# tenpy/cyten

Measured on AMD Instinct MI355X. Metric: block-sparse tdot+SVD GFLOP/s (fp64), higher is better.
Workload: dtype f64

## Files before the change

### cyten_amd/csrc/jacobi_engine.hip

```cpp
#include "jacobi_engine.h"

#include <algorithm>
#include <cmath>
#include <cstdlib>

namespace cyb {
constexpr double kPredictQuad = 16.0;
namespace {

typedef double d4 __attribute__((ext_vector_type(4)));
typedef double d2 __attribute__((ext_vector_type(2)));
#define GLOBAL_AS __attribute__((address_space(1)))
typedef const GLOBAL_AS d2* gc2;
typedef const GLOBAL_AS d2* gcp2;
typedef GLOBAL_AS double* gp;

constexpr int GS = JP + 2;
constexpr int QS = JP + 16;
constexpr int GK = 64;
constexpr int XS = GK + 2;
constexpr int NT = 256;
constexpr int NPAIR = JP / 2;
static_assert(JP == 32, "the wave tiling below assumes 32 x 32 pair problems");

__device__ __forceinline__ double wave_max(double v)
{
#pragma unroll
    for (int o = 32; o > 0; o >>= 1) v = fmax(v, __shfl_xor(v, o));
    return v;
}

__device__ __forceinline__ double block_max(double v, double* red, int tid)
{
    v = wave_max(v);
    __syncthreads();
    if ((tid & 63) == 0) red[tid >> 6] = v;
    __syncthreads();
    return fmax(fmax(red[0], red[1]), fmax(red[2], red[3]));
}

__device__ __forceinline__ double gram_offmax(const double* Gs, double* red, int tid)
{
    double m = 0.0;
#pragma unroll
    for (int e = tid; e < JP * JP; e += NT) {
        const int i = e / JP, j = e % JP;
        if (i < j) {
            const double den = Gs[i * GS + i] * Gs[j * GS + j];
            if (den > 0.0) m = fmax(m, fabs(Gs[i * GS + j]) * rsqrt(den));
        }
    }
    return block_max(m, red, tid);
}

__host__ __device__ __forceinline__ void circle_pair(int n, int r, int k, int& p, int& q)
{
    const int m = n - 1;
    if (k == 0) {
        p = m;
        q = r;
    } else {
        p = r + k;
        if (p >= m) p -= m;
        q = r - k;
        if (q < 0) q += m;
    }
}

__device__ __forceinline__ double fast_rsqrt(double x)
{
    double r = __builtin_amdgcn_rsq(x);
    r = r * (1.5 - 0.5 * x * r * r);
    r = r * (1.5 - 0.5 * x * r * r);
    return r;
}

__device__ __forceinline__ void jacobi_rot(double a, double d, double b, double& c, double& s)
{
    const double delta = d - a;
    const double h2 = delta * delta + 4.0 * b * b;
    c = 1.0;
    s = 0.0;
    if (fabs(b) > 1e-300 && h2 > 1e-300) {
        const double rh = fast_rsqrt(h2);
        const double c2 = 0.5 + 0.5 * fabs(delta) * rh;
        const double rc = fast_rsqrt(c2);
        c = c2 * rc;
        const double sg = ((delta >= 0.0) == (b >= 0.0)) ? 1.0 : -1.0;
        s = sg * fabs(b) * rh * rc;
    }
}

__device__ __forceinline__ int xrow(int i, int P, int Q) { return (i < JB) ? P * JB + i : Q * JB + (i - JB); }

struct JScratch {
    double* gpart;
    double* qout[2];
    int32_t* zout[2];
    int32_t* flag[2];
    unsigned int* cnt;
};

__device__ __forceinline__ void update_role(const JMat* __restrict__ mats, const JWork* __restrict__ work, int round,
                                            int pi, int unit, int U, const JScratch& sc, int buf, bool do_w, bool do_j,
                                            double* smem, int* zflag);

__global__ void __launch_bounds__(NT, 2)
jacobi_gram_kernel(const JMat* __restrict__ mats, const JWork* __restrict__ work, int round, int G, int max_inner,
                   unsigned long long* __restrict__ offmax_bits, JScratch sc, int buf, int n_gram, int prev_round, int UJ)
{
    constexpr int STAGE = 2 * JP * XS > 4 * JP * GS ? 2 * JP * XS : 4 * JP * GS;
    __shared__ __attribute__((aligned(16))) double smem[2 * JP * GS + JP * QS + STAGE + 8];
    __shared__ int perm[JP];
    __shared__ int zrow[JP];
    __shared__ int s_any_null, s_last;
    __shared__ unsigned short sched[(JP - 1) * NPAIR];
    double* Gs = smem;
    double* G2 = Gs + JP * GS;
    double* Qs = G2 + JP * GS;
    double* Xc = Qs + JP * QS;
    double* red = Xc + STAGE;

    const int tid = threadIdx.x;
    const int lane = tid & 63, wave = tid >> 6;
    if ((int)blockIdx.x >= n_gram) {
        const int b = (int)blockIdx.x - n_gram;
        update_role(mats, work, prev_round, b / UJ, b % UJ, UJ, sc, buf ^ 1, false, true, smem, zrow);
        return;
    }
    const int pi = blockIdx.x / G, part = blockIdx.x % G;

    const JWork wk = work[pi];
    const JMat mt = mats[wk.mat];
    if (round >= mt.nb - 1) return;
    int P, Q;
    circle_pair(mt.nb, round, wk.slot, P, Q);
    if (P > Q) {
        const int t = P;
        P = Q;
        Q = t;
    }

    {
        gp W = (gp)mt.W;
        const int ld = mt.lenp;
        d4 acc[2][2];
#pragma unroll
        for (int i = 0; i < 2; ++i)
#pragma unroll
            for (int j = 0; j < 2; ++j) acc[i][j] = d4{0.0, 0.0, 0.0, 0.0};
        const int r = lane & 15, g2 = 2 * (lane >> 4);
        gcp2 s0 = (gcp2)(W + (int64_t)xrow(r, P, Q) * ld + g2);
        gcp2 s1 = (gcp2)(W + (int64_t)xrow(r + 16, P, Q) * ld + g2);
        const int nchunk_all = ld / 8;
        const int c_begin = (int)((int64_t)part * nchunk_all / G), c_end = (int)((int64_t)(part + 1) * nchunk_all / G);
        constexpr int UN = 8;
        d2 x0[UN], x1[UN], n0[UN], n1[UN];
        auto load = [&](d2 (&a0)[UN], d2 (&a1)[UN], int c0) {
#pragma unroll
            for (int u = 0; u < UN; ++u) {
                const int c = min(c0 + 4 * u, c_end - 1);
                a0[u] = s0[c * 4];
                a1[u] = s1[c * 4];
            }
        };
        if (c_begin + wave < c_end) load(x0, x1, c_begin + wave);
        for (int c0 = c_begin + wave; c0 < c_end; c0 += 4 * UN) {
            const bool more = c0 + 4 * UN < c_end;
            if (more) load(n0, n1, c0 + 4 * UN);
#pragma unroll
            for (int u = 0; u < UN; ++u) {
                if (c0 + 4 * u < c_end) {
                    acc[0][0] = __builtin_amdgcn_mfma_f64_16x16x4f64(x0[u].x, x0[u].x, acc[0][0], 0, 0, 0);
                    acc[0][1] = __builtin_amdgcn_mfma_f64_16x16x4f64(x0[u].x, x1[u].x, acc[0][1], 0, 0, 0);
                    acc[1][1] = __builtin_amdgcn_mfma_f64_16x16x4f64(x1[u].x, x1[u].x, acc[1][1], 0, 0, 0);
                    acc[0][0] = __builtin_amdgcn_mfma_f64_16x16x4f64(x0[u].y, x0[u].y, acc[0][0], 0, 0, 0);
                    acc[0][1] = __builtin_amdgcn_mfma_f64_16x16x4f64(x0[u].y, x1[u].y, acc[0][1], 0, 0, 0);
                    acc[1][1] = __builtin_amdgcn_mfma_f64_16x16x4f64(x1[u].y, x1[u].y, acc[1][1], 0, 0, 0);
                }
            }
            if (more) {
#pragma unroll
                for (int u = 0; u < UN; ++u) {
                    x0[u] = n0[u];
                    x1[u] = n1[u];
                }
            }
        }
        double* wpart = Xc + wave * (JP * GS);
#pragma unroll
        for (int i = 0; i < 2; ++i)
#pragma unroll
            for (int j = 0; j < 2; ++j)
#pragma unroll
                for (int r = 0; r < 4; ++r) {
                    if (i == 1 && j == 0)
                        wpart[(16 + (lane & 15)) * GS + (lane >> 4) + 4 * r] = acc[0][1][r];
                    else
                        wpart[(i * 16 + (lane >> 4) + 4 * r) * GS + j * 16 + (lane & 15)] = acc[i][j][r];
                }
    }
    __syncthreads();
    if (G == 1) {
        for (int e = tid; e < JP * JP; e += NT) {
            const int i = e / JP, j = e % JP;
            double s = 0.0;
#pragma unroll
            for (int w = 0; w < 4; ++w) s += Xc[w * (JP * GS) + i * GS + j];
            Gs[i * GS + j] = s;
        }
        __syncthreads();
    } else {
        GLOBAL_AS double* mine = (GLOBAL_AS double*)(sc.gpart + ((size_t)pi * G + part) * (JP * JP));
        for (int e = tid; e < JP * JP; e += NT) {
            const int i = e / JP, j = e % JP;
            double s = 0.0;
#pragma unroll
            for (int w = 0; w < 4; ++w) s += Xc[w * (JP * GS) + i * GS + j];
            __hip_atomic_store((double*)(mine + e), s, __ATOMIC_RELAXED, __HIP_MEMORY_SCOPE_AGENT);
        }
        asm volatile("s_waitcnt vmcnt(0)" ::: "memory");
        __syncthreads();
        if (tid == 0) {
            const unsigned int old = __hip_atomic_fetch_add(sc.cnt + pi, 1u, __ATOMIC_RELAXED, __HIP_MEMORY_SCOPE_AGENT);
            s_last = (old == (unsigned int)(G - 1)) ? 1 : 0;
            if (s_last) __hip_atomic_store(sc.cnt + pi, 0u, __ATOMIC_RELAXED, __HIP_MEMORY_SCOPE_AGENT);
        }
        __syncthreads();
        if (!s_last) return;
        const GLOBAL_AS double* all = (const GLOBAL_AS double*)(sc.gpart + (size_t)pi * G * (JP * JP));
        for (int e = tid; e < JP * JP; e += NT) {
            const int i = e / JP, j = e % JP;
            double s = 0.0;
            for (int g = 0; g < G; ++g)
                s += __hip_atomic_load((double*)(all + (size_t)g * (JP * JP) + i * JP + j), __ATOMIC_RELAXED, __HIP_MEMORY_SCOPE_AGENT);
            Gs[i * GS + j] = s;
        }
        __syncthreads();
    }
    if (tid == 0) s_any_null = 0;
    __syncthreads();
    if (tid < JP) {
        const double thr2 = mt.thr2;
        const double g = Gs[tid * GS + tid];
        const int z = (g > 0.0 && g <= thr2) ? 1 : 0;
        zrow[tid] = z;
        perm[tid] = tid;
        if (z) s_any_null = 1;
    }
    __syncthreads();
    const bool any_null = s_any_null != 0;
    if (any_null) {
        for (int e = tid; e < JP * JP; e += NT) {
            const int i = e / JP, j = e % JP;
            if (zrow[i] || zrow[j]) Gs[i * GS + j] = 0.0;
        }
        __syncthreads();
    }
    double off = gram_offmax(Gs, red, tid);
    if (tid == 0) {
        atomicMax(offmax_bits + wk.mat, (unsigned long long)__double_as_longlong(off));
        sc.flag[buf][pi] = (off <= mt.tol && !any_null) ? 0 : 1;
    }
    if (off <= mt.tol && !any_null) return;

    for (int e = tid; e < JP * QS; e += NT) Qs[e] = ((e / QS) == (e % QS)) ? 1.0 : 0.0;
    for (int e = tid; e < (JP - 1) * NPAIR; e += NT) {
        int p, q;
        circle_pair(JP, e / NPAIR, e % NPAIR, p, q);
        sched[e] = (unsigned short)(p | (q << 8));
    }
    __syncthreads();
    double* Ga = Gs;
    double* Gb = G2;
    for (int sweep = 0; sweep < (off <= mt.tol ? 0 : max_inner); ++sweep) {
        for (int r = 0; r < JP - 1; ++r) {
            const int pr = tid >> 4, pc = tid & 15;
            const unsigned int sr = sched[r * NPAIR + pr], scl = sched[r * NPAIR + pc];
            const int i = sr & 255, j = sr >> 8, k = scl & 255, l = scl >> 8;
            double c2, s2;
            jacobi_rot(Ga[k * GS + k], Ga[l * GS + l], Ga[k * GS + l], c2, s2);
            const int srcl = (lane & 48) | pr;
            const double c1 = __shfl(c2, srcl), s1 = __shfl(s2, srcl);
            {
                const double gik = Ga[i * GS + k], gil = Ga[i * GS + l];
                const double gjk = Ga[j * GS + k], gjl = Ga[j * GS + l];
                const double hik = c1 * gik - s1 * gjk, hil = c1 * gil - s1 * gjl;
                const double hjk = s1 * gik + c1 * gjk, hjl = s1 * gil + c1 * gjl;
                double nik = c2 * hik - s2 * hil, nil = s2 * hik + c2 * hil;
                double njk = c2 * hjk - s2 * hjl, njl = s2 * hjk + c2 * hjl;
                if (pr == pc) {
                    nil = 0.0;
                    njk = 0.0;
                }
                Gb[i * GS + k] = nik;
                Gb[i * GS + l] = nil;
                Gb[j * GS + k] = njk;
                Gb[j * GS + l] = njl;
            }
#pragma unroll
            for (int t = 0; t < 2; ++t) {
                const int row = (tid >> 4) + 16 * t;
                const double qk = Qs[row * QS + k], ql = Qs[row * QS + l];
                Qs[row * QS + k] = c2 * qk - s2 * ql;
                Qs[row * QS + l] = s2 * qk + c2 * ql;
            }
            __syncthreads();
            double* tsw = Ga;
            Ga = Gb;
            Gb = tsw;
        }
        if (sweep + 1 < max_inner) {
            const double off_in = gram_offmax(Ga, red, tid);
            if (off_in <= 0.25 * mt.tol) break;
        }
    }
    __syncthreads();
    if (off > mt.tol && tid < JP) {
        auto key = [&](int i) { return xrow(i, P, Q) < mt.nv ? Ga[i * GS + i] : -1.0e300; };
        const double g = key(tid);
        int rk = 0;
        for (int j = 0; j < JP; ++j) {
            const double gj = key(j);
            rk += (gj > g || (gj == g && j < tid)) ? 1 : 0;
        }
        perm[rk] = tid;
    }
    __syncthreads();
    GLOBAL_AS double* qo = (GLOBAL_AS double*)(sc.qout[buf] + (size_t)pi * (JP * JP));
    for (int e = tid; e < JP * JP; e += NT) {
        const int k = e / JP, r = e % JP;
        qo[e] = Qs[k * QS + perm[r]];
    }
    if (tid < JP) sc.zout[buf][(size_t)pi * JP + tid] = zrow[perm[tid]];
}

__device__ __forceinline__ void update_role(const JMat* __restrict__ mats, const JWork* __restrict__ work, int round,
                                            int pi, int unit, int U, const JScratch& sc, int buf, bool do_w, bool do_j,
                                            double* smem, int* zflag)
{
    double* Qs = smem;
    const int tid = threadIdx.x;
    const int lane = tid & 63, wave = tid >> 6;
    const JWork wk = work[pi];
    const JMat mt = mats[wk.mat];
    if (round >= mt.nb - 1) return;
    if (sc.flag[buf][pi] == 0) return;
    int P, Q;
    circle_pair(mt.nb, round, wk.slot, P, Q);
    if (P > Q) {
        const int t = P;
        P = Q;
        Q = t;
    }
    const int cw = do_w ? mt.lenp / 64 : 0, cj = (do_j && mt.J) ? mt.nvp / 64 : 0;
    const int ct = cw + cj;
    const int c_begin = (int)((int64_t)unit * ct / U), c_end = (int)((int64_t)(unit + 1) * ct / U);
    if (c_begin >= c_end) return;
    const int n = lane & 15, kq = lane >> 4;
    auto chunk_ptr = [&](int c, int k) -> gp {
        const bool in_w = c < cw;
        gp base = (gp)(in_w ? mt.W : mt.J);
        const int ld = in_w ? mt.lenp : mt.nvp;
        const int cc = in_w ? c : c - cw;
        return base + (int64_t)xrow(k, P, Q) * ld + cc * 64 + wave * 16 + n;
    };
    double xb[JP / 4], xn[JP / 4];
#pragma unroll
    for (int kk = 0; kk < JP / 4; ++kk) xb[kk] = *chunk_ptr(c_begin, 4 * kk + kq);
    const GLOBAL_AS double* qo = (const GLOBAL_AS double*)(sc.qout[buf] + (size_t)pi * (JP * JP));
    for (int e = tid; e < JP * JP; e += NT) Qs[(e / JP) * QS + (e % JP)] = qo[e];
    if (tid < JP) zflag[tid] = sc.zout[buf][(size_t)pi * JP + tid];
    __syncthreads();
    const double* ap0 = Qs + (lane >> 4) * QS + (lane & 15);
    const double* ap1 = ap0 + 16;
    int zr[2][4];
#pragma unroll
    for (int i = 0; i < 2; ++i)
#pragma unroll
        for (int r = 0; r < 4; ++r) zr[i][r] = zflag[i * 16 + (lane >> 4) + 4 * r];
    for (int c = c_begin; c < c_end; ++c) {
        if (c + 1 < c_end) {
#pragma unroll
            for (int kk = 0; kk < JP / 4; ++kk) xn[kk] = *chunk_ptr(c + 1, 4 * kk + kq);
        }
        d4 acc[2] = {d4{0.0, 0.0, 0.0, 0.0}, d4{0.0, 0.0, 0.0, 0.0}};
#pragma unroll
        for (int kk = 0; kk < JP / 4; ++kk) {
            const double a0 = ap0[kk * 4 * QS], a1 = ap1[kk * 4 * QS];
            acc[0] = __builtin_amdgcn_mfma_f64_16x16x4f64(a0, xb[kk], acc[0], 0, 0, 0);
            acc[1] = __builtin_amdgcn_mfma_f64_16x16x4f64(a1, xb[kk], acc[1], 0, 0, 0);
        }
        const bool zero_null = c < cw;
#pragma unroll
        for (int i = 0; i < 2; ++i)
#pragma unroll
            for (int r = 0; r < 4; ++r) {
                const int row = i * 16 + (lane >> 4) + 4 * r;
                const double val = (zero_null && zr[i][r]) ? 0.0 : acc[i][r];
                *chunk_ptr(c, row) = val;
            }
#pragma unroll
        for (int kk = 0; kk < JP / 4; ++kk) xb[kk] = xn[kk];
    }
}

__global__ void __launch_bounds__(NT, 3)
jacobi_update_kernel(const JMat* __restrict__ mats, const JWork* __restrict__ work, int round, int U, JScratch sc, int buf,
                     int do_w, int do_j)
{
    __shared__ __attribute__((aligned(16))) double smem[JP * QS];
    __shared__ int zflag[JP];
    update_role(mats, work, round, blockIdx.x / U, blockIdx.x % U, U, sc, buf, do_w != 0, do_j != 0, smem, zflag);
}


struct RPair {
    double* W;
    double* J;
    double tol, thr2;
    int32_t nvp, lenp, nb, nv;
    int32_t mat, slot;
    int32_t pad[2];
};
static_assert(sizeof(RPair) == 64, "RPair is read as one 64-byte descriptor");

struct RScratch {
    double* gpart;
    unsigned int* cnt;
    unsigned int* err;
    int np;
    unsigned long long* stamps;
};

typedef unsigned int u32x4 __attribute__((ext_vector_type(4)));
union Q16 {
    u32x4 u;
    d2 d;
};

constexpr int VS = JP + 2;
constexpr int ROUND_LDS_DOUBLES = 2 * JP * GS + 2 * JP * VS + JP * QS + 4 * JP * GS + 8;
constexpr size_t ROUND_LDS_BYTES = 88 * 1024;
static_assert(ROUND_LDS_DOUBLES * 8 + 1024 <= ROUND_LDS_BYTES, "LDS carve-up of the fused round kernel");
constexpr int RGMAX = 8;
constexpr int RPRE = 6;

__device__ __forceinline__ int ring_next(int p)
{
    if (p == 0) return 0;
    if (p == 1) return 2;
    if (p & 1) return p - 2;
    return p == JP - 2 ? JP - 1 : p + 2;
}

__device__ __forceinline__ void jacobi_rot_bf(double a, double d, double b, double& c, double& s, double thr2 = 0.0)
{
    const double delta = d - a;
    const double b2 = b + b;
    double h2 = fma(b2, b2, delta * delta);
    const bool ok = (fabs(b) > 1e-300) & (h2 > 1e-300) & (b * b > thr2 * a * d);
    h2 = ok ? h2 : 1.0;
    double r = __builtin_amdgcn_rsq(h2);
    double g = h2 * r, h = 0.5 * r;
    double e = fma(-g, h, 0.5);
    g = fma(g, e, g);
    h = fma(h, e, h);
    e = fma(-g, h, 0.5);
    h = fma(h, e, h);
    const double c2 = fma(fabs(delta), h, 0.5);
    double r2 = __builtin_amdgcn_rsq(c2);
    double gc = c2 * r2, hc = 0.5 * r2;
    double ec = fma(-gc, hc, 0.5);
    gc = fma(gc, ec, gc);
    hc = fma(hc, ec, hc);
    ec = fma(-gc, hc, 0.5);
    gc = fma(gc, ec, gc);
    hc = fma(hc, ec, hc);
    const double sabs = (fabs(b) * h) * (4.0 * hc);
    const bool pos = (delta >= 0.0) == (b >= 0.0);
    c = ok ? gc : 1.0;
    s = ok ? (pos ? sabs : -sabs) : 0.0;
}

__global__ void __launch_bounds__(NT, 1)
jacobi_round_kernel(const RPair* __restrict__ pairs, int round, int G, int max_inner,
                    unsigned long long* __restrict__ offmax_bits, RScratch sc)
{
    extern __shared__ __attribute__((aligned(16))) double rsm[];
    double* Gs = rsm;
    double* G2 = Gs + JP * GS;
    double* Va = G2 + JP * GS;
    double* Vb = Va + JP * VS;
    double* Qs = Vb + JP * VS;
    double* Xc = Qs + JP * QS;
    double* red = Xc + 4 * JP * GS;
    int* ibase = reinterpret_cast<int*>(red + 8);
    int* perm = ibase;
    int* zrow = ibase + JP;
    int* zout = ibase + 2 * JP;
    int* flags = ibase + 3 * JP;

    const int tid = threadIdx.x;
    const int lane = tid & 63, wave = tid >> 6;
    const int pi = blockIdx.x / G, part = blockIdx.x % G;
#define ROUND_STAMP(k)                                                                              \
    do {                                                                                            \
        if (sc.stamps && tid == 0) sc.stamps[(size_t)blockIdx.x * 8 + (k)] = wall_clock64();        \
    } while (0)
    ROUND_STAMP(0);
    const RPair mt = pairs[pi];
    if (round >= mt.nb - 1) return;
    int P, Q;
    circle_pair(mt.nb, round, mt.slot, P, Q);
    if (P > Q) {
        const int t = P;
        P = Q;
        Q = t;
    }
    const int cw = mt.lenp / 64, cj = mt.J ? mt.nvp / 64 : 0;
    const int w_begin = (int)((int64_t)part * cw / G), w_end = (int)((int64_t)(part + 1) * cw / G);
    const int j_begin = (int)((int64_t)part * cj / G), j_end = (int)((int64_t)(part + 1) * cj / G);
    const int nW = w_end - w_begin, nJ = j_end - j_begin;
    const int ct = nW + nJ;
    const int un = lane & 15, ukq = lane >> 4;
    auto chunk_ptr = [&](int c, int k) -> gp {
        const bool in_w = c < nW;
        gp base = (gp)(in_w ? mt.W : mt.J);
        const int ld = in_w ? mt.lenp : mt.nvp;
        const int cc = in_w ? w_begin + c : j_begin + (c - nW);
        return base + (int64_t)xrow(k, P, Q) * ld + cc * 64 + wave * 16 + un;
    };

    double xpre[RPRE][JP / 4];
    {
        gp W = (gp)mt.W;
        const int ld = mt.lenp;
        d4 acc00 = d4{0.0, 0.0, 0.0, 0.0}, acc01 = acc00, acc11 = acc00;
        const int r = lane & 15, g2 = 2 * (lane >> 4);
        gcp2 s0 = (gcp2)(W + (int64_t)xrow(r, P, Q) * ld + g2);
        gcp2 s1 = (gcp2)(W + (int64_t)xrow(r + 16, P, Q) * ld + g2);
        const int c_begin = 8 * w_begin, c_end = 8 * w_end;
        constexpr int UN = 8;
        d2 x0[UN], x1[UN], n0[UN], n1[UN];
        auto load = [&](d2 (&a0)[UN], d2 (&a1)[UN], int c0) {
#pragma unroll
            for (int u = 0; u < UN; ++u) {
                const int c = min(c0 + 4 * u, c_end - 1);
                a0[u] = s0[c * 4];
                a1[u] = s1[c * 4];
            }
        };
        if (c_begin + wave < c_end) load(x0, x1, c_begin + wave);
#pragma unroll
        for (int c = 0; c < RPRE; ++c) {
            if (c < ct) {
#pragma unroll
                for (int kk = 0; kk < JP / 4; ++kk) xpre[c][kk] = *chunk_ptr(c, 4 * kk + ukq);
            }
        }
        for (int c0 = c_begin + wave; c0 < c_end; c0 += 4 * UN) {
            const bool more = c0 + 4 * UN < c_end;
            if (more) load(n0, n1, c0 + 4 * UN);
#pragma unroll
            for (int u = 0; u < UN; ++u) {
                if (c0 + 4 * u < c_end) {
                    acc00 = __builtin_amdgcn_mfma_f64_16x16x4f64(x0[u].x, x0[u].x, acc00, 0, 0, 0);
                    acc01 = __builtin_amdgcn_mfma_f64_16x16x4f64(x0[u].x, x1[u].x, acc01, 0, 0, 0);
                    acc11 = __builtin_amdgcn_mfma_f64_16x16x4f64(x1[u].x, x1[u].x, acc11, 0, 0, 0);
                    acc00 = __builtin_amdgcn_mfma_f64_16x16x4f64(x0[u].y, x0[u].y, acc00, 0, 0, 0);
                    acc01 = __builtin_amdgcn_mfma_f64_16x16x4f64(x0[u].y, x1[u].y, acc01, 0, 0, 0);
                    acc11 = __builtin_amdgcn_mfma_f64_16x16x4f64(x1[u].y, x1[u].y, acc11, 0, 0, 0);
                }
            }
            if (more) {
#pragma unroll
                for (int u = 0; u < UN; ++u) {
                    x0[u] = n0[u];
                    x1[u] = n1[u];
                }
            }
        }
        double* wpart = Xc + wave * (JP * GS);
#pragma unroll
        for (int q = 0; q < 4; ++q) {
            const int rr = (lane >> 4) + 4 * q, cc = lane & 15;
            wpart[rr * GS + cc] = acc00[q];
            wpart[rr * GS + 16 + cc] = acc01[q];
            wpart[(16 + cc) * GS + rr] = acc01[q];
            wpart[(16 + rr) * GS + 16 + cc] = acc11[q];
        }
    }
    __syncthreads();
    ROUND_STAMP(1);
    {
        const int gi = tid >> 3, gj = 4 * (tid & 7);
        d2 lo = d2{0.0, 0.0}, hi = d2{0.0, 0.0};
#pragma unroll
        for (int w = 0; w < 4; ++w) {
            const double* src = Xc + w * (JP * GS) + gi * GS + gj;
            lo.x += src[0];
            lo.y += src[1];
            hi.x += src[2];
            hi.y += src[3];
        }
        if (G > 1) {
            const unsigned int pbytes = JP * JP * 8;
            __amdgpu_buffer_rsrc_t rs_all = __builtin_amdgcn_make_buffer_rsrc(sc.gpart + (size_t)pi * G * (JP * JP), 0, pbytes * G, 0x00020000);
            Q16 a, b;
            a.d = lo;
            b.d = hi;
            const unsigned int off = (unsigned int)part * pbytes + (unsigned int)tid * 32u;
            __builtin_amdgcn_raw_buffer_store_b128(a.u, rs_all, off, 0, 16);
            __builtin_amdgcn_raw_buffer_store_b128(b.u, rs_all, off + 16u, 0, 16);
            asm volatile("s_waitcnt vmcnt(0)" ::: "memory");
            __syncthreads();
            if (tid == 0) {
                unsigned int* ticket = sc.cnt + (size_t)round * sc.np + pi;
                __hip_atomic_fetch_add(ticket, 1u, __ATOMIC_RELAXED, __HIP_MEMORY_SCOPE_AGENT);
                int ok = 1;
                const unsigned long long t0 = wall_clock64();
                while (__hip_atomic_load(ticket, __ATOMIC_RELAXED, __HIP_MEMORY_SCOPE_AGENT) < (unsigned int)G) {
                    __builtin_amdgcn_s_sleep(1);
                    if (wall_clock64() - t0 > 100000000ull) {
                        ok = 0;
                        __hip_atomic_store(sc.err, 1u, __ATOMIC_RELAXED, __HIP_MEMORY_SCOPE_AGENT);
                        break;
                    }
                }
                flags[1] = ok;
            }
            __syncthreads();
            if (!flags[1]) return;
            Q16 pa[RGMAX], pb[RGMAX];
#pragma unroll
            for (int g = 0; g < RGMAX; ++g) {
                if (g < G) {
                    pa[g].u = __builtin_amdgcn_raw_buffer_load_b128(rs_all, (unsigned int)g * pbytes + (unsigned int)tid * 32u, 0, 16);
                    pb[g].u = __builtin_amdgcn_raw_buffer_load_b128(rs_all, (unsigned int)g * pbytes + (unsigned int)tid * 32u + 16u, 0, 16);
                }
            }
            lo = d2{0.0, 0.0};
            hi = d2{0.0, 0.0};
#pragma unroll
            for (int g = 0; g < RGMAX; ++g) {
                if (g < G) {
                    lo += pa[g].d;
                    hi += pb[g].d;
                }
            }
        }
        double* dst = Gs + gi * GS + gj;
        dst[0] = lo.x;
        dst[1] = lo.y;
        dst[2] = hi.x;
        dst[3] = hi.y;
    }
    __syncthreads();
    ROUND_STAMP(2);
    if (tid == 0) flags[0] = 0;
    __syncthreads();
    if (tid < JP) {
        const double g = Gs[tid * GS + tid];
        const int z = (g > 0.0 && g <= mt.thr2) ? 1 : 0;
        zrow[tid] = z;
        perm[tid] = tid;
        if (z) flags[0] = 1;
    }
    __syncthreads();
    const bool any_null = flags[0] != 0;
    if (any_null) {
        for (int e = tid; e < JP * JP; e += NT) {
            const int i = e / JP, j = e % JP;
            if (zrow[i] || zrow[j]) Gs[i * GS + j] = 0.0;
        }
        __syncthreads();
    }
    const double off = gram_offmax(Gs, red, tid);
    if (part == 0 && tid == 0) atomicMax(offmax_bits + mt.mat, (unsigned long long)__double_as_longlong(off));
    if (off <= mt.tol && !any_null) return;

    ROUND_STAMP(3);
    for (int e = tid; e < JP * VS; e += NT) Va[e] = ((e / VS) == (e % VS)) ? 1.0 : 0.0;
    __syncthreads();
    double* Ga = Gs;
    double* Gb = G2;
    double* Vc = Va;
    double* Vn = Vb;
    {
        const int pr = tid >> 4, pc = tid & 15;
        const int r0 = 2 * pr, c0 = 2 * pc;
        const int dr0 = ring_next(r0), dr1 = ring_next(r0 + 1), dc0 = ring_next(c0), dc1 = ring_next(c0 + 1);
        for (int sweep = 0; sweep < (off <= mt.tol ? 0 : max_inner); ++sweep) {
            for (int r = 0; r < JP - 1; ++r) {
                const d2 g0 = *reinterpret_cast<const d2*>(Ga + r0 * GS + c0);
                const d2 g1 = *reinterpret_cast<const d2*>(Ga + (r0 + 1) * GS + c0);
                const d2 ac = *reinterpret_cast<const d2*>(Ga + c0 * GS + c0);
                const double dc = Ga[(c0 + 1) * GS + c0 + 1];
                const d2 v0 = *reinterpret_cast<const d2*>(Vc + r0 * VS + c0);
                const d2 v1 = *reinterpret_cast<const d2*>(Vc + (r0 + 1) * VS + c0);
                double c1, s1, c2, s2;
                jacobi_rot_bf(ac.x, dc, ac.y, c2, s2);
                const int rsrc = (lane & 48) | pr;
                c1 = __shfl(c2, rsrc);
                s1 = __shfl(s2, rsrc);
                const double hik = c1 * g0.x - s1 * g1.x, hil = c1 * g0.y - s1 * g1.y;
                const double hjk = s1 * g0.x + c1 * g1.x, hjl = s1 * g0.y + c1 * g1.y;
                double nik = c2 * hik - s2 * hil, nil = s2 * hik + c2 * hil;
                double njk = c2 * hjk - s2 * hjl, njl = s2 * hjk + c2 * hjl;
                if (pr == pc) {
                    nil = 0.0;
                    njk = 0.0;
                }
                Gb[dr0 * GS + dc0] = nik;
                Gb[dr0 * GS + dc1] = nil;
                Gb[dr1 * GS + dc0] = njk;
                Gb[dr1 * GS + dc1] = njl;
                Vn[r0 * VS + dc0] = c2 * v0.x - s2 * v0.y;
                Vn[r0 * VS + dc1] = s2 * v0.x + c2 * v0.y;
                Vn[(r0 + 1) * VS + dc0] = c2 * v1.x - s2 * v1.y;
                Vn[(r0 + 1) * VS + dc1] = s2 * v1.x + c2 * v1.y;
                __syncthreads();
                double* t = Ga;
                Ga = Gb;
                Gb = t;
                t = Vc;
                Vc = Vn;
                Vn = t;
            }
            if (sweep + 1 < max_inner) {
                const double off_in = gram_offmax(Ga, red, tid);
                if (off_in <= 0.25 * mt.tol) break;
            }
        }
    }
    __syncthreads();
    ROUND_STAMP(4);
    if (off > mt.tol && tid < JP) {
        auto key = [&](int i) { return xrow(i, P, Q) < mt.nv ? Ga[i * GS + i] : -1.0e300; };
        const double g = key(tid);
        int rk = 0;
        for (int j = 0; j < JP; ++j) {
            const double gj = key(j);
            rk += (gj > g || (gj == g && j < tid)) ? 1 : 0;
        }
        perm[rk] = tid;
    }
    __syncthreads();
    for (int e = tid; e < JP * JP; e += NT) {
        const int k = e / JP, m = e % JP;
        Qs[k * QS + m] = Vc[k * VS + perm[m]];
    }
    if (tid < JP) zout[tid] = zrow[perm[tid]];
    __syncthreads();
    ROUND_STAMP(5);
    if (ct <= 0) return;
    const double* ap0 = Qs + (lane >> 4) * QS + (lane & 15);
    const double* ap1 = ap0 + 16;
    double a0[JP / 4], a1[JP / 4];
#pragma unroll
    for (int kk = 0; kk < JP / 4; ++kk) {
        a0[kk] = ap0[kk * 4 * QS];
        a1[kk] = ap1[kk * 4 * QS];
    }
    int zr[2][4];
#pragma unroll
    for (int i = 0; i < 2; ++i)
#pragma unroll
        for (int q = 0; q < 4; ++q) zr[i][q] = zout[i * 16 + (lane >> 4) + 4 * q];
    auto apply = [&](int c, const double (&xb)[JP / 4]) {
        d4 acc[2] = {d4{0.0, 0.0, 0.0, 0.0}, d4{0.0, 0.0, 0.0, 0.0}};
#pragma unroll
        for (int kk = 0; kk < JP / 4; ++kk) {
            acc[0] = __builtin_amdgcn_mfma_f64_16x16x4f64(a0[kk], xb[kk], acc[0], 0, 0, 0);
            acc[1] = __builtin_amdgcn_mfma_f64_16x16x4f64(a1[kk], xb[kk], acc[1], 0, 0, 0);
        }
        const bool zero_null = c < nW;
#pragma unroll
        for (int i = 0; i < 2; ++i)
#pragma unroll
            for (int q = 0; q < 4; ++q) {
                const int row = i * 16 + (lane >> 4) + 4 * q;
                *chunk_ptr(c, row) = (zero_null && zr[i][q]) ? 0.0 : acc[i][q];
            }
    };
#pragma unroll
    for (int c = 0; c < RPRE; ++c)
        if (c < ct) apply(c, xpre[c]);
    if (ct > RPRE) {
        double xb[JP / 4], xn[JP / 4];
#pragma unroll
        for (int kk = 0; kk < JP / 4; ++kk) xb[kk] = *chunk_ptr(RPRE, 4 * kk + ukq);
        for (int c = RPRE; c < ct; ++c) {
            if (c + 1 < ct) {
#pragma unroll
                for (int kk = 0; kk < JP / 4; ++kk) xn[kk] = *chunk_ptr(c + 1, 4 * kk + ukq);
            }
            apply(c, xb);
#pragma unroll
            for (int kk = 0; kk < JP / 4; ++kk) xb[kk] = xn[kk];
        }
    }
    __syncthreads();
    ROUND_STAMP(6);
#undef ROUND_STAMP
}


constexpr int CJ = JP / 2;
constexpr int CS = CJ + 1;
__device__ __forceinline__ void hermitian_pivot_solve(const double* Gs, double* work, double* rot, double* Vout, double* Gdiag, int sweeps,
                                                      int lane, double thr2 = 0.0, bool cross = false)
{
    auto pair_of = [cross](int r, int k, int& p, int& q) {
        if (cross) {
            p = k;
            q = CJ / 2 + ((k + r) & (CJ / 2 - 1));
        } else
            circle_pair(CJ, r, k, p, q);
    };
    const int n_steps = cross ? CJ / 2 : CJ - 1;
    double* Hr = work;
    double* Hi = Hr + CJ * CS;
    double* Ur = Hi + CJ * CS;
    double* Ui = Ur + CJ * CS;
    for (int e = lane; e < CJ * CJ; e += 64) {
        const int a = e / CJ, b = e % CJ;
        Hr[a * CS + b] = 0.5 * (Gs[(2 * a) * GS + 2 * b] + Gs[(2 * a + 1) * GS + 2 * b + 1]);
        Hi[a * CS + b] = a == b ? 0.0 : 0.5 * (Gs[(2 * a + 1) * GS + 2 * b] - Gs[(2 * a) * GS + 2 * b + 1]);
        Ur[a * CS + b] = a == b ? 1.0 : 0.0;
        Ui[a * CS + b] = 0.0;
    }
    __builtin_amdgcn_fence(__ATOMIC_RELEASE, "wavefront");
    __builtin_amdgcn_wave_barrier();
    for (int sw = 0; sw < sweeps; ++sw)
        for (int r = 0; r < n_steps; ++r) {
            if (lane < CJ / 2) {
                int p, q;
                pair_of(r, lane, p, q);
                const double gr = Hr[p * CS + q], gi = Hi[p * CS + q];
                const double ab = sqrt(gr * gr + gi * gi);
                double c = 1.0, sn = 0.0, pr = 1.0, pi = 0.0;
                if (ab > 1e-300) {
                    jacobi_rot_bf(Hr[p * CS + p], Hr[q * CS + q], ab, c, sn, thr2);
                    pr = gr / ab;
                    pi = gi / ab;
                }
                rot[lane * 4 + 0] = c;
                rot[lane * 4 + 1] = sn;
                rot[lane * 4 + 2] = pr;
                rot[lane * 4 + 3] = pi;
            }
            __builtin_amdgcn_fence(__ATOMIC_RELEASE, "wavefront");
            __builtin_amdgcn_wave_barrier();
            for (int e = lane; e < (CJ / 2) * CJ; e += 64) {
                const int k = e / CJ, col = e % CJ;
                int p, q;
                pair_of(r, k, p, q);
                const double c = rot[k * 4], sn = rot[k * 4 + 1], fr = rot[k * 4 + 2], fi = rot[k * 4 + 3];
                const double pr_ = Hr[p * CS + col], pi_ = Hi[p * CS + col], qr_ = Hr[q * CS + col], qi_ = Hi[q * CS + col];
                const double tr = fr * qr_ - fi * qi_, ti = fr * qi_ + fi * qr_;
                Hr[p * CS + col] = c * pr_ - sn * tr;
                Hi[p * CS + col] = c * pi_ - sn * ti;
                Hr[q * CS + col] = sn * pr_ + c * tr;
                Hi[q * CS + col] = sn * pi_ + c * ti;
            }
            __builtin_amdgcn_fence(__ATOMIC_RELEASE, "wavefront");
            __builtin_amdgcn_wave_barrier();
            for (int e = lane; e < (CJ / 2) * CJ * 2; e += 64) {
                const int which = e / ((CJ / 2) * CJ), f = e % ((CJ / 2) * CJ);
                const int k = f / CJ, row = f % CJ;
                int p, q;
                pair_of(r, k, p, q);
                double* Xr = which ? Ur : Hr;
                double* Xi = which ? Ui : Hi;
                const double c = rot[k * 4], sn = rot[k * 4 + 1], fr = rot[k * 4 + 2], fi = -rot[k * 4 + 3];
                const double pr_ = Xr[row * CS + p], pi_ = Xi[row * CS + p], qr_ = Xr[row * CS + q], qi_ = Xi[row * CS + q];
                const double tr = fr * qr_ - fi * qi_, ti = fr * qi_ + fi * qr_;
                Xr[row * CS + p] = c * pr_ - sn * tr;
                Xi[row * CS + p] = c * pi_ - sn * ti;
                Xr[row * CS + q] = sn * pr_ + c * tr;
                Xi[row * CS + q] = sn * pi_ + c * ti;
            }
            __builtin_amdgcn_fence(__ATOMIC_RELEASE, "wavefront");
            __builtin_amdgcn_wave_barrier();
        }
    for (int e = lane; e < CJ * CJ; e += 64) {
        const int a = e / CJ, b = e % CJ;
        const double x = Ur[a * CS + b], y = Ui[a * CS + b];
        Vout[(2 * a) * VS + 2 * b] = x;
        Vout[(2 * a) * VS + 2 * b + 1] = -y;
        Vout[(2 * a + 1) * VS + 2 * b] = y;
        Vout[(2 * a + 1) * VS + 2 * b + 1] = x;
    }
    if (lane < CJ) {
        const double lam = Hr[lane * CS + lane];
        Gdiag[(2 * lane) * GS + 2 * lane] = lam;
        Gdiag[(2 * lane + 1) * GS + 2 * lane + 1] = lam;
    }
}

struct SScratch {
    double* gpart;
    unsigned int* ticket;
    unsigned int* ready;
    unsigned int* err;
    const int2* wgmap;
    const int2* wgent;
    unsigned long long* stamps;
    int stamp_round;
    int n_sweeps, n_mats;
    unsigned int* arrive;
    int* nsw;
    unsigned int* readyJ;
    int defer_j;
    int cross_every, cross_min_nb;
};
constexpr int SW_MAX_ENT = 64;

constexpr int SW_UN = 8;
constexpr int SW_PRE = 6;
constexpr int SWEEP_XREG = (4 * JP * GS > JP * GS + 2 * JP * VS) ? 4 * JP * GS : JP * GS + 2 * JP * VS;
constexpr int SWEEP_LDS_DOUBLES = JP * GS + SWEEP_XREG + 2 * JP * QS + 8;
constexpr size_t SWEEP_LDS_BYTES = 88 * 1024;
static_assert((size_t)SWEEP_LDS_DOUBLES * 8 + 1024 <= SWEEP_LDS_BYTES, "LDS request of the sweep kernel");
constexpr int SWEEP_WG_PER_CU = 1;

typedef unsigned int u32x2 __attribute__((ext_vector_type(2)));
union Q8 {
    u32x2 u;
    double d;
};

template <int SLEEP = 1>
__device__ __forceinline__ bool spin_until(const unsigned int* word, unsigned int target, unsigned int* err)
{
    const unsigned long long t0 = wall_clock64();
    unsigned int it = 0;
    while (__hip_atomic_load(word, __ATOMIC_RELAXED, __HIP_MEMORY_SCOPE_AGENT) < target) {
        __builtin_amdgcn_s_sleep(SLEEP);
        if ((++it & 63u) == 0u) {
            if (__hip_atomic_load(err, __ATOMIC_RELAXED, __HIP_MEMORY_SCOPE_AGENT) != 0u) return false;
            if (wall_clock64() - t0 > 100000000ull) {
                __hip_atomic_store(err, 1u, __ATOMIC_RELAXED, __HIP_MEMORY_SCOPE_AGENT);
                return false;
            }
        }
    }
    return true;
}

__device__ __forceinline__ void sweep_update_j(const __amdgpu_buffer_rsrc_t rsJ, const double* Qm, int P, int Q, int nvp, int j_begin,
                                               int nJ, int wave, int lane)
{
    const int un = lane & 15, ukq = lane >> 4;
    const double* ap0 = Qm + (lane >> 4) * QS + (lane & 15);
    const double* ap1 = ap0 + 16;
    double a0[JP / 4], a1[JP / 4];
#pragma unroll
    for (int kk = 0; kk < JP / 4; ++kk) {
        a0[kk] = ap0[kk * 4 * QS];
        a1[kk] = ap1[kk * 4 * QS];
    }
    auto off_of = [&](int c, int k) { return (unsigned int)(((int64_t)xrow(k, P, Q) * nvp + (j_begin + c) * 64 + wave * 16 + un) * 8); };
    auto load = [&](double (&x)[JP / 4], int c) {
#pragma unroll
        for (int kk = 0; kk < JP / 4; ++kk) {
            Q8 q;
            q.u = __builtin_amdgcn_raw_buffer_load_b64(rsJ, off_of(c, 4 * kk + ukq), 0, 16);
            x[kk] = q.d;
        }
    };
    double xb[JP / 4], xn[JP / 4];
    if (nJ > 0) load(xb, 0);
    for (int c = 0; c < nJ; ++c) {
        if (c + 1 < nJ) load(xn, c + 1);
        d4 acc[2] = {d4{0.0, 0.0, 0.0, 0.0}, d4{0.0, 0.0, 0.0, 0.0}};
#pragma unroll
        for (int kk = 0; kk < JP / 4; ++kk) {
            acc[0] = __builtin_amdgcn_mfma_f64_16x16x4f64(a0[kk], xb[kk], acc[0], 0, 0, 0);
            acc[1] = __builtin_amdgcn_mfma_f64_16x16x4f64(a1[kk], xb[kk], acc[1], 0, 0, 0);
        }
#pragma unroll
        for (int i = 0; i < 2; ++i)
#pragma unroll
            for (int q = 0; q < 4; ++q) {
                Q8 v;
                v.d = acc[i][q];
                __builtin_amdgcn_raw_buffer_store_b64(v.u, rsJ, off_of(c, i * 16 + (lane >> 4) + 4 * q), 0, 16);
            }
#pragma unroll
        for (int kk = 0; kk < JP / 4; ++kk) xb[kk] = xn[kk];
    }
}

template <bool CPLX>
__global__ void __launch_bounds__(NT, 1)
jacobi_sweep_kernel(const RPair* __restrict__ pairs, int max_inner, unsigned long long* __restrict__ offmax_bits, SScratch sc)
{
    extern __shared__ __attribute__((aligned(16))) double rsm[];
    double* Gs = rsm;
    double* G2 = Gs + JP * GS;
    double* Va = G2 + JP * GS;
    double* Vb = Va + JP * VS;
    double* Xc = G2;
    double* Qs0 = G2 + SWEEP_XREG;
    double* Qs1 = Qs0 + JP * QS;
    double* red = Qs1 + JP * QS;
    int* ibase = reinterpret_cast<int*>(red + 8);
    int* perm = ibase;
    int* zrow = ibase + JP;
    int* zout = ibase + 2 * JP;
    int* flags = ibase + 3 * JP;
    int* edone = flags + 4;

    const int tid = threadIdx.x;
    const int lane = tid & 63, wave = tid >> 6;
    const int2 went = sc.wgent ? sc.wgent[blockIdx.x] : make_int2((int)blockIdx.x, (int)blockIdx.x + 1);
    int max_rounds = 0;
    for (int e = went.x; e < went.y; ++e) max_rounds = max(max_rounds, pairs[sc.wgmap[e].x].nb - 1);
    const int n_sw = sc.n_sweeps;
    const bool one_entry = went.y - went.x == 1;
    int pendP = -1, pendQ = -1, pend_ground = 0;
    if (n_sw > 1) {
        if (tid < SW_MAX_ENT) edone[tid] = 0;
        __syncthreads();
    }
    for (int sw = 0; sw < n_sw; ++sw) {
    for (int round = 0; round < max_rounds; ++round)
    for (int ent = went.x; ent < went.y; ++ent) {
    const int2 wm = sc.wgmap[ent];
    const int pi = wm.x, part = wm.y;
    const RPair mt = pairs[pi];
    if (round >= mt.nb - 1) continue;
    if (n_sw > 1 && edone[ent - went.x]) continue;
    const int ground = sw * (mt.nb - 1) + round;
    const int G = mt.pad[0];
    unsigned int* ready = sc.ready + mt.pad[1];
    unsigned int* readyJ = sc.readyJ + mt.pad[1];
    unsigned int* ticket = sc.ticket + pi;
    double* Qs = (ground & 1) ? Qs1 : Qs0;
    const unsigned int pbytes = JP * JP * 8;
    const __amdgpu_buffer_rsrc_t rsW = __builtin_amdgcn_make_buffer_rsrc(mt.W, 0, (int)((size_t)mt.nvp * mt.lenp * 8), 0x00020000);
    const __amdgpu_buffer_rsrc_t rsJ =
        __builtin_amdgcn_make_buffer_rsrc(mt.J ? mt.J : mt.W, 0, mt.J ? (int)((size_t)mt.nvp * mt.nvp * 8) : 0, 0x00020000);
    const int cw = mt.lenp / 64, cj = mt.J ? mt.nvp / 64 : 0;
    const int w_begin = (int)((int64_t)part * cw / G), w_end = (int)((int64_t)(part + 1) * cw / G);
    const int j_begin = (int)((int64_t)part * cj / G), j_end = (int)((int64_t)(part + 1) * cj / G);
    const int nW = w_end - w_begin, nJ = j_end - j_begin;
    const bool defer = sc.defer_j && one_entry && G > 1 && nJ > 0 && round < mt.nb - 2;
    const int ct = defer ? nW : nW + nJ;
    const int pre_limit = (sc.defer_j && G > 1) ? min(ct, nW) : ct;
    const int un = lane & 15, ukq = lane >> 4;
#define SWEEP_STAMP(k)                                                                                            \
    do {                                                                                                          \
        if (sc.stamps && tid == 0 && round == sc.stamp_round) sc.stamps[(size_t)blockIdx.x * 8 + (k)] = wall_clock64(); \
    } while (0)

    {
        int P, Q;
        circle_pair(mt.nb, round, mt.slot, P, Q);
        if (P > Q) {
            const int t = P;
            P = Q;
            Q = t;
        }
        SWEEP_STAMP(0);
        __syncthreads();
        if (ground > 0) {
            if (tid == 0) {
                bool ok = spin_until(ready + (size_t)P * G + part, (unsigned int)ground, sc.err);
                ok = ok && spin_until(ready + (size_t)Q * G + part, (unsigned int)ground, sc.err);
                flags[1] = ok ? 1 : 0;
            }
            __syncthreads();
            if (!flags[1]) return;
        }
        SWEEP_STAMP(1);
        auto chunk_off = [&](int c, int k, bool& in_w) -> unsigned int {
            in_w = c < nW;
            const int ld = in_w ? mt.lenp : mt.nvp;
            const int cc = in_w ? w_begin + c : j_begin + (c - nW);
            return (unsigned int)(((int64_t)xrow(k, P, Q) * ld + cc * 64 + wave * 16 + un) * 8);
        };
        auto chunk_load = [&](int c, int k) -> double {
            bool in_w;
            const unsigned int off = chunk_off(c, k, in_w);
            Q8 q;
            q.u = in_w ? __builtin_amdgcn_raw_buffer_load_b64(rsW, off, 0, 16) : __builtin_amdgcn_raw_buffer_load_b64(rsJ, off, 0, 16);
            return q.d;
        };
        double xpre[SW_PRE][JP / 4];
        {
            const int ld = mt.lenp;
            d4 acc00 = d4{0.0, 0.0, 0.0, 0.0}, acc01 = acc00, acc11 = acc00;
            const int r = lane & 15, g2 = 2 * (lane >> 4);
            const unsigned int o0 = (unsigned int)(((int64_t)xrow(r, P, Q) * ld + g2) * 8);
            const unsigned int o1 = (unsigned int)(((int64_t)xrow(r + 16, P, Q) * ld + g2) * 8);
            const int c_begin = 8 * w_begin, c_end = 8 * w_end;
            constexpr int UN = SW_UN;
            d2 x0[UN], x1[UN], n0[UN], n1[UN];
            auto load = [&](d2 (&a0)[UN], d2 (&a1)[UN], int c0) {
#pragma unroll
                for (int u = 0; u < UN; ++u) {
                    const int c = min(c0 + 4 * u, c_end - 1);
                    Q16 qa, qb;
                    qa.u = __builtin_amdgcn_raw_buffer_load_b128(rsW, o0 + (unsigned int)c * 64u, 0, 16);
                    qb.u = __builtin_amdgcn_raw_buffer_load_b128(rsW, o1 + (unsigned int)c * 64u, 0, 16);
                    a0[u] = qa.d;
                    a1[u] = qb.d;
                }
            };
            if (c_begin + wave < c_end) load(x0, x1, c_begin + wave);
#pragma unroll
            for (int c = 0; c < SW_PRE; ++c) {
                if (c < pre_limit) {
#pragma unroll
                    for (int kk = 0; kk < JP / 4; ++kk) xpre[c][kk] = chunk_load(c, 4 * kk + ukq);
                }
            }
            for (int c0 = c_begin + wave; c0 < c_end; c0 += 4 * UN) {
                const bool more = c0 + 4 * UN < c_end;
                if (more) load(n0, n1, c0 + 4 * UN);
#pragma unroll
                for (int u = 0; u < UN; ++u) {
                    if (c0 + 4 * u < c_end) {
                        acc00 = __builtin_amdgcn_mfma_f64_16x16x4f64(x0[u].x, x0[u].x, acc00, 0, 0, 0);
                        acc01 = __builtin_amdgcn_mfma_f64_16x16x4f64(x0[u].x, x1[u].x, acc01, 0, 0, 0);
                        acc11 = __builtin_amdgcn_mfma_f64_16x16x4f64(x1[u].x, x1[u].x, acc11, 0, 0, 0);
                        acc00 = __builtin_amdgcn_mfma_f64_16x16x4f64(x0[u].y, x0[u].y, acc00, 0, 0, 0);
                        acc01 = __builtin_amdgcn_mfma_f64_16x16x4f64(x0[u].y, x1[u].y, acc01, 0, 0, 0);
                        acc11 = __builtin_amdgcn_mfma_f64_16x16x4f64(x1[u].y, x1[u].y, acc11, 0, 0, 0);
                    }
                }
                if (more) {
#pragma unroll
                    for (int u = 0; u < UN; ++u) {
                        x0[u] = n0[u];
                        x1[u] = n1[u];
                    }
                }
            }
            double* wpart = Xc + wave * (JP * GS);
#pragma unroll
            for (int q = 0; q < 4; ++q) {
                const int rr = (lane >> 4) + 4 * q, cc = lane & 15;
                wpart[rr * GS + cc] = acc00[q];
                wpart[rr * GS + 16 + cc] = acc01[q];
                wpart[(16 + cc) * GS + rr] = acc01[q];
                wpart[(16 + rr) * GS + 16 + cc] = acc11[q];
            }
        }
        __syncthreads();
        SWEEP_STAMP(2);
        {
            const int gi = tid >> 3, gj = 4 * (tid & 7);
            d2 lo = d2{0.0, 0.0}, hi = d2{0.0, 0.0};
#pragma unroll
            for (int w = 0; w < 4; ++w) {
                const double* src = Xc + w * (JP * GS) + gi * GS + gj;
                lo.x += src[0];
                lo.y += src[1];
                hi.x += src[2];
                hi.y += src[3];
            }
            if (G > 1) {
                const __amdgpu_buffer_rsrc_t rs_all = __builtin_amdgcn_make_buffer_rsrc(
                    sc.gpart + ((size_t)pi * 2 + (size_t)(ground & 1)) * RGMAX * (JP * JP), 0, (int)(pbytes * G), 0x00020000);
                Q16 a, b;
                a.d = lo;
                b.d = hi;
                const unsigned int off = (unsigned int)part * pbytes + (unsigned int)tid * 32u;
                __builtin_amdgcn_raw_buffer_store_b128(a.u, rs_all, off, 0, 16);
                __builtin_amdgcn_raw_buffer_store_b128(b.u, rs_all, off + 16u, 0, 16);
                asm volatile("s_waitcnt vmcnt(0)" ::: "memory");
                __syncthreads();
                if (tid == 0) __hip_atomic_fetch_add(ticket, 1u, __ATOMIC_RELAXED, __HIP_MEMORY_SCOPE_AGENT);
                if (pendP >= 0) {
                    if (tid == 0) {
                        bool ok = spin_until(readyJ + (size_t)pendP * G + part, (unsigned int)pend_ground, sc.err);
                        ok = ok && spin_until(readyJ + (size_t)pendQ * G + part, (unsigned int)pend_ground, sc.err);
                        flags[1] = ok ? 1 : 0;
                    }
                    __syncthreads();
                    if (!flags[1]) return;
                    sweep_update_j(rsJ, (pend_ground & 1) ? Qs1 : Qs0, pendP, pendQ, mt.nvp, j_begin, nJ, wave, lane);
                    asm volatile("s_waitcnt vmcnt(0)" ::: "memory");
                    __syncthreads();
                    if (tid == 0) {
                        __hip_atomic_store(readyJ + (size_t)pendP * G + part, (unsigned int)(pend_ground + 1), __ATOMIC_RELAXED, __HIP_MEMORY_SCOPE_AGENT);
                        __hip_atomic_store(readyJ + (size_t)pendQ * G + part, (unsigned int)(pend_ground + 1), __ATOMIC_RELAXED, __HIP_MEMORY_SCOPE_AGENT);
                    }
                    pendP = -1;
                }
                if (tid == 0) flags[1] = spin_until(ticket, (unsigned int)G * (unsigned int)(ground + 1), sc.err) ? 1 : 0;
                __syncthreads();
                if (!flags[1]) return;
                lo = d2{0.0, 0.0};
                hi = d2{0.0, 0.0};
                for (int g0 = 0; g0 < G; g0 += 4) {
                    Q16 pa[4], pb[4];
#pragma unroll
                    for (int g = 0; g < 4; ++g) {
                        if (g0 + g < G) {
                            pa[g].u = __builtin_amdgcn_raw_buffer_load_b128(rs_all, (unsigned int)(g0 + g) * pbytes + (unsigned int)tid * 32u, 0, 16);
                            pb[g].u = __builtin_amdgcn_raw_buffer_load_b128(rs_all, (unsigned int)(g0 + g) * pbytes + (unsigned int)tid * 32u + 16u, 0, 16);
                        }
                    }
#pragma unroll
                    for (int g = 0; g < 4; ++g) {
                        if (g0 + g < G) {
                            lo += pa[g].d;
                            hi += pb[g].d;
                        }
                    }
                }
            }
            double* dst = Gs + gi * GS + gj;
            dst[0] = lo.x;
            dst[1] = lo.y;
            dst[2] = hi.x;
            dst[3] = hi.y;
        }
        __syncthreads();
        SWEEP_STAMP(3);
        if (tid == 0) flags[0] = 0;
        __syncthreads();
        if (tid < JP) {
            double g = Gs[tid * GS + tid];
            if constexpr (CPLX) g = fmax(g, Gs[(tid ^ 1) * GS + (tid ^ 1)]);
            const int z = (g > 0.0 && g <= mt.thr2) ? 1 : 0;
            zrow[tid] = z;
            perm[tid] = tid;
            if (z) flags[0] = 1;
        }
        __syncthreads();
        const bool any_null = flags[0] != 0;
        if (any_null) {
            for (int e = tid; e < JP * JP; e += NT) {
                const int i = e / JP, j = e % JP;
                if (zrow[i] || zrow[j]) Gs[i * GS + j] = 0.0;
            }
            __syncthreads();
        }
        const double off = gram_offmax(Gs, red, tid);
        if (part == 0 && tid == 0) atomicMax(offmax_bits + (size_t)sw * sc.n_mats + mt.mat, (unsigned long long)__double_as_longlong(off));
        const bool skip = off <= mt.tol && !any_null;
        if (!skip) {
            double* Ga = Gs;
            double* Gb = G2;
            double* Vc = Va;
            double* Vn = Vb;
            bool pos_is_interleaved = false;
            const int cross_k = sc.cross_every > 0 ? sc.cross_every : max(4, (mt.nb + 2) / 4);
            const bool cross = sc.cross_every != 0 && !any_null && mt.nb >= sc.cross_min_nb && (round % cross_k) != 0;
            if constexpr (CPLX) {
                if (tid < 64) hermitian_pivot_solve(Gs, G2, Vb, Va, Gs, max_inner, tid, 0.25 * mt.tol * mt.tol, cross);
                __syncthreads();
            } else {
            auto cpos = [](int i) { return i < JB ? 2 * i : 2 * (i - JB) + 1; };
            pos_is_interleaved = cross;
            if (cross) {
                for (int e = tid; e < JP * JP; e += NT) {
                    const int i = e / JP, j = e % JP;
                    Gb[cpos(i) * GS + cpos(j)] = Ga[i * GS + j];
                }
                for (int e = tid; e < JP * VS; e += NT) Va[e] = (cpos(e / VS) == (e % VS)) ? 1.0 : 0.0;
                double* t = Ga;
                Ga = Gb;
                Gb = t;
            } else
                for (int e = tid; e < JP * VS; e += NT) Va[e] = ((e / VS) == (e % VS)) ? 1.0 : 0.0;
            __syncthreads();
            {
                const int pr = tid >> 4, pc = tid & 15;
                const int r0 = 2 * pr, c0 = 2 * pc;
                const int dr0 = cross ? r0 : ring_next(r0), dr1 = cross ? ((r0 + 3) & (JP - 1)) : ring_next(r0 + 1);
                const int dc0 = cross ? c0 : ring_next(c0), dc1 = cross ? ((c0 + 3) & (JP - 1)) : ring_next(c0 + 1);
                const int n_steps = cross ? JB : JP - 1;
                for (int sweep = 0; sweep < (off <= mt.tol ? 0 : max_inner); ++sweep) {
                    for (int r = 0; r < n_steps; ++r) {
                        const d2 g0 = *reinterpret_cast<const d2*>(Ga + r0 * GS + c0);
                        const d2 g1 = *reinterpret_cast<const d2*>(Ga + (r0 + 1) * GS + c0);
                        const d2 ac = *reinterpret_cast<const d2*>(Ga + c0 * GS + c0);
                        const double dc = Ga[(c0 + 1) * GS + c0 + 1];
                        const d2 v0 = *reinterpret_cast<const d2*>(Vc + r0 * VS + c0);
                        const d2 v1 = *reinterpret_cast<const d2*>(Vc + (r0 + 1) * VS + c0);
                        double c1, s1, c2, s2;
                        jacobi_rot_bf(ac.x, dc, ac.y, c2, s2, 0.25 * mt.tol * mt.tol);
                        const int rsrc = (lane & 48) | pr;
                        c1 = __shfl(c2, rsrc);
                        s1 = __shfl(s2, rsrc);
                        const double hik = c1 * g0.x - s1 * g1.x, hil = c1 * g0.y - s1 * g1.y;
                        const double hjk = s1 * g0.x + c1 * g1.x, hjl = s1 * g0.y + c1 * g1.y;
                        double nik = c2 * hik - s2 * hil, nil = s2 * hik + c2 * hil;
                        double njk = c2 * hjk - s2 * hjl, njl = s2 * hjk + c2 * hjl;
                        if (pr == pc) {
                            nil = 0.0;
                            njk = 0.0;
                        }
                        Gb[dr0 * GS + dc0] = nik;
                        Gb[dr0 * GS + dc1] = nil;
                        Gb[dr1 * GS + dc0] = njk;
                        Gb[dr1 * GS + dc1] = njl;
                        Vn[r0 * VS + dc0] = c2 * v0.x - s2 * v0.y;
                        Vn[r0 * VS + dc1] = s2 * v0.x + c2 * v0.y;
                        Vn[(r0 + 1) * VS + dc0] = c2 * v1.x - s2 * v1.y;
                        Vn[(r0 + 1) * VS + dc1] = s2 * v1.x + c2 * v1.y;
                        __syncthreads();
                        double* t = Ga;
                        Ga = Gb;
                        Gb = t;
                        t = Vc;
                        Vc = Vn;
                        Vn = t;
                    }
                    if (sweep + 1 < max_inner) {
                        const double off_in = gram_offmax(Ga, red, tid);
                        if (off_in <= 0.25 * mt.tol) break;
                    }
                }
            }
            }
            __syncthreads();
            SWEEP_STAMP(4);
            if (off > mt.tol && tid < 64) {
                const int li = lane & (JP - 1);
                const int li_idx = pos_is_interleaved ? ((li & 1) ? JB + (li >> 1) : (li >> 1)) : li;
                const double g = xrow(li_idx, P, Q) < mt.nv ? Ga[li * GS + li] : -1.0e300;
                const int glo = __double2loint(g), ghi = __double2hiint(g);
                int rk = 0;
#pragma unroll
                for (int j = 0; j < JP; ++j) {
                    const double gj = __hiloint2double(__builtin_amdgcn_readlane(ghi, j), __builtin_amdgcn_readlane(glo, j));
                    rk += (gj > g || (gj == g && j < li)) ? 1 : 0;
                }
                if (lane < JP) perm[rk] = lane;
            }
            __syncthreads();
            for (int e = tid; e < JP * JP; e += NT) {
                const int k = e / JP, m = e % JP;
                Qs[k * QS + m] = Vc[k * VS + perm[m]];
            }
            if (tid < JP) {
                const int pp = perm[tid];
                zout[tid] = zrow[pos_is_interleaved ? ((pp & 1) ? JB + (pp >> 1) : (pp >> 1)) : pp];
            }
            __syncthreads();
            SWEEP_STAMP(5);
            if (ct > nW) {
                if (tid == 0) {
                    bool ok = spin_until(readyJ + (size_t)P * G + part, (unsigned int)ground, sc.err);
                    ok = ok && spin_until(readyJ + (size_t)Q * G + part, (unsigned int)ground, sc.err);
                    flags[1] = ok ? 1 : 0;
                }
                __syncthreads();
                if (!flags[1]) return;
#pragma unroll
                for (int c = 0; c < SW_PRE; ++c) {
                    if (c >= pre_limit && c < ct) {
#pragma unroll
                        for (int kk = 0; kk < JP / 4; ++kk) xpre[c][kk] = chunk_load(c, 4 * kk + ukq);
                    }
                }
            }
            if (ct > 0) {
                const double* ap0 = Qs + (lane >> 4) * QS + (lane & 15);
                const double* ap1 = ap0 + 16;
                double a0[JP / 4], a1[JP / 4];
#pragma unroll
                for (int kk = 0; kk < JP / 4; ++kk) {
                    a0[kk] = ap0[kk * 4 * QS];
                    a1[kk] = ap1[kk * 4 * QS];
                }
                int zr[2][4];
#pragma unroll
                for (int i = 0; i < 2; ++i)
#pragma unroll
                    for (int q = 0; q < 4; ++q) zr[i][q] = zout[i * 16 + (lane >> 4) + 4 * q];
                auto apply = [&](int c, const double (&xb)[JP / 4]) {
                    d4 acc[2] = {d4{0.0, 0.0, 0.0, 0.0}, d4{0.0, 0.0, 0.0, 0.0}};
#pragma unroll
                    for (int kk = 0; kk < JP / 4; ++kk) {
                        acc[0] = __builtin_amdgcn_mfma_f64_16x16x4f64(a0[kk], xb[kk], acc[0], 0, 0, 0);
                        acc[1] = __builtin_amdgcn_mfma_f64_16x16x4f64(a1[kk], xb[kk], acc[1], 0, 0, 0);
                    }
                    const bool zero_null = c < nW;
#pragma unroll
                    for (int i = 0; i < 2; ++i)
#pragma unroll
                        for (int q = 0; q < 4; ++q) {
                            const int row = i * 16 + (lane >> 4) + 4 * q;
                            bool in_w;
                            const unsigned int o = chunk_off(c, row, in_w);
                            Q8 v;
                            v.d = (zero_null && zr[i][q]) ? 0.0 : acc[i][q];
                            if (in_w) __builtin_amdgcn_raw_buffer_store_b64(v.u, rsW, o, 0, 16);
                            else __builtin_amdgcn_raw_buffer_store_b64(v.u, rsJ, o, 0, 16);
                        }
                };
#pragma unroll
                for (int c = 0; c < SW_PRE; ++c)
                    if (c < ct) apply(c, xpre[c]);
                if (ct > SW_PRE) {
                    double xb[JP / 4], xn[JP / 4];
#pragma unroll
                    for (int kk = 0; kk < JP / 4; ++kk) xb[kk] = chunk_load(SW_PRE, 4 * kk + ukq);
                    for (int c = SW_PRE; c < ct; ++c) {
                        if (c + 1 < ct) {
#pragma unroll
                            for (int kk = 0; kk < JP / 4; ++kk) xn[kk] = chunk_load(c + 1, 4 * kk + ukq);
                        }
                        apply(c, xb);
#pragma unroll
                        for (int kk = 0; kk < JP / 4; ++kk) xb[kk] = xn[kk];
                    }
                }
            }
        }
        if (defer && !skip) {
            pendP = P;
            pendQ = Q;
            pend_ground = ground;
        }
        asm volatile("s_waitcnt vmcnt(0)" ::: "memory");
        __syncthreads();
        if (tid == 0) {
            if (skip && nJ > 0) {
                (void)spin_until(readyJ + (size_t)P * G + part, (unsigned int)ground, sc.err);
                (void)spin_until(readyJ + (size_t)Q * G + part, (unsigned int)ground, sc.err);
            }
            __hip_atomic_store(ready + (size_t)P * G + part, (unsigned int)(ground + 1), __ATOMIC_RELAXED, __HIP_MEMORY_SCOPE_AGENT);
            __hip_atomic_store(ready + (size_t)Q * G + part, (unsigned int)(ground + 1), __ATOMIC_RELAXED, __HIP_MEMORY_SCOPE_AGENT);
            if (!(defer && !skip)) {
                __hip_atomic_store(readyJ + (size_t)P * G + part, (unsigned int)(ground + 1), __ATOMIC_RELAXED, __HIP_MEMORY_SCOPE_AGENT);
                __hip_atomic_store(readyJ + (size_t)Q * G + part, (unsigned int)(ground + 1), __ATOMIC_RELAXED, __HIP_MEMORY_SCOPE_AGENT);
            }
            if (n_sw > 1 && round == mt.nb - 2) __hip_atomic_fetch_add(sc.arrive + mt.mat, 1u, __ATOMIC_RELAXED, __HIP_MEMORY_SCOPE_AGENT);
        }
        SWEEP_STAMP(6);
    }
    }
    if (n_sw == 1) break;
    __syncthreads();
    if (tid == 0) {
        int all = 1, ok = 1;
        for (int ent = went.x; ent < went.y && ok; ++ent) {
            if (edone[ent - went.x]) continue;
            const int2 wm = sc.wgmap[ent];
            const RPair mt = pairs[wm.x];
            const unsigned int entries = (unsigned int)(mt.nb / 2) * (unsigned int)mt.pad[0];
            if (!spin_until<32>(sc.arrive + mt.mat, entries * (unsigned int)(sw + 1), sc.err)) {
                ok = 0;
                break;
            }
            const double off = __longlong_as_double((long long)__hip_atomic_load(offmax_bits + (size_t)sw * sc.n_mats + mt.mat, __ATOMIC_RELAXED, __HIP_MEMORY_SCOPE_AGENT));
            const double prev = sw ? __longlong_as_double((long long)__hip_atomic_load(offmax_bits + (size_t)(sw - 1) * sc.n_mats + mt.mat,
                                                                                      __ATOMIC_RELAXED, __HIP_MEMORY_SCOPE_AGENT))
                                   : 1e300;
            const bool stagnated = sw + 1 >= 6 && off <= 64.0 * mt.tol && off >= 0.5 * prev;
            const bool predicted = off <= 0.1 * sqrt(mt.tol) && prev < 1.0 && off <= prev * sqrt(prev) && off <= kPredictQuad * prev * prev;
            if (off <= mt.tol || stagnated || predicted) {
                edone[ent - went.x] = 1;
                if (mt.slot == 0 && wm.y == 0) sc.nsw[mt.mat] = sw + 1;
            } else all = 0;
        }
        flags[1] = ok;
        flags[2] = all;
    }
    __syncthreads();
    if (!flags[1] || flags[2]) return;
    }
#undef SWEEP_STAMP
}

}

int jacobi_orthogonalise(cyb_ctx_t ctx, const std::vector<JMat>& h_mats, int max_sweeps,
                         std::vector<int32_t>& sweeps_out, bool cplx)
{
    const int n = (int)h_mats.size();
    sweeps_out.assign((size_t)n, 0);
    if (n == 0) return CYB_OK;
    hipStream_t st = ctx->stream;

    std::vector<int> active;
    for (int i = 0; i < n; ++i) {
        if (h_mats[(size_t)i].nv <= 1) sweeps_out[(size_t)i] = 0;
        else active.push_back(i);
    }
    static const bool one_launch_ok = getenv("CYB_JACOBI_PERSWEEP") == nullptr && getenv("CYB_JACOBI_TRACE") == nullptr &&
                                      getenv("CYB_JACOBI_STAMPS") == nullptr && getenv("CYB_JACOBI_NOPREDICT") == nullptr;
    static const bool one_launch_all = getenv("CYB_JACOBI_ONELAUNCH") != nullptr;
    int nb_max_all = 0;
    for (int i = 0; i < n; ++i) nb_max_all = std::max(nb_max_all, h_mats[(size_t)i].nb);
    const int n_sw_dev = (one_launch_ok && (one_launch_all || nb_max_all <= 16)) ? max_sweeps : 1;
    const size_t w_off = (size_t)n * (size_t)n_sw_dev;
    const size_t b_off = (sizeof(unsigned long long) * w_off + 2 * sizeof(unsigned int) * (size_t)n + 15) / 16 * 16;
    std::vector<unsigned long long> h_off(b_off / 8 + 2);
    bool one_launch_done = false;
    std::vector<int> cached_order, cached_G;
    uint64_t cached_at = 0;
    void* cached_img = nullptr;
    size_t cached_map_off = 0;
    std::vector<double> prev_off((size_t)n, 1e300);
    int status = CYB_OK;
    for (int sweep = 1; sweep <= max_sweeps && !active.empty(); ++sweep) {
        std::vector<int> order = active;
        std::stable_sort(order.begin(), order.end(),
                         [&](int a, int b) { return h_mats[(size_t)a].nb > h_mats[(size_t)b].nb; });
        std::vector<JWork> wl;
        int max_nb = 0;
        for (int m : order) {
            const int nb = h_mats[(size_t)m].nb;
            max_nb = std::max(max_nb, nb);
            for (int k = 0; k < nb / 2; ++k) wl.push_back(JWork{m, k});
        }
        const JMat* d_mats = nullptr;
        void* d_wl = nullptr;
        static const bool legacy = getenv("CYB_JACOBI_LEGACY") != nullptr;
        static const int fused_max = getenv("CYB_JACOBI_FUSED_MAX") ? atoi(getenv("CYB_JACOBI_FUSED_MAX")) : 64;
        static const int inner_env = getenv("CYB_JACOBI_INNER") ? atoi(getenv("CYB_JACOBI_INNER")) : 0;
        const int max_inner = inner_env > 0 ? inner_env : (max_nb <= 8 ? 3 : 1);
        constexpr int kGmax = RGMAX;
        const size_t np = wl.size();
        const size_t b_cnt = (sizeof(unsigned int) * np * (size_t)std::max(max_nb - 1, 1) + 15) / 16 * 16;
        const size_t b_gpart = sizeof(double) * np * kGmax * JP * JP, b_q = sizeof(double) * np * JP * JP;
        const size_t b_z = sizeof(int32_t) * np * JP, b_f = (sizeof(int32_t) * np + 15) / 16 * 16, b_c = (sizeof(unsigned int) * np + 15) / 16 * 16;
        size_t n_ready = 0;
        for (int m : order) n_ready += (size_t)h_mats[(size_t)m].nb * RGMAX;
        const size_t b_ready = (sizeof(unsigned int) * (2 * n_ready + np) + 15) / 16 * 16;
        void* wsp = nullptr;
        status = ctx->workspace(b_off + 16 + b_cnt + b_ready + 2 * b_gpart + 2 * (b_q + b_z + b_f) + b_c + 1024, &wsp, 2);
        if (status != CYB_OK) break;
        char* bp = static_cast<char*>(wsp);
        RScratch rs;
        unsigned long long* d_off = reinterpret_cast<unsigned long long*>(bp);
        rs.err = reinterpret_cast<unsigned int*>(bp + b_off);
        rs.cnt = reinterpret_cast<unsigned int*>(bp + b_off + 16);
        unsigned int* d_ready = reinterpret_cast<unsigned int*>(bp + b_off + 16 + b_cnt);
        bp += b_off + 16 + b_cnt + b_ready;
        rs.gpart = reinterpret_cast<double*>(bp);
        bp += 2 * b_gpart;
        rs.np = (int)np;
        rs.stamps = nullptr;
        JScratch sc;
        sc.gpart = rs.gpart;
        for (int h = 0; h < 2; ++h) {
            sc.qout[h] = reinterpret_cast<double*>(bp);
            bp += b_q;
        }
        for (int h = 0; h < 2; ++h) {
            sc.zout[h] = reinterpret_cast<int32_t*>(bp);
            bp += b_z;
        }
        for (int h = 0; h < 2; ++h) {
            sc.flag[h] = reinterpret_cast<int32_t*>(bp);
            bp += b_f;
        }
        sc.cnt = reinterpret_cast<unsigned int*>(bp);
        if (hipMemsetAsync(wsp, 0, b_off + 16 + b_cnt + b_ready, st) != hipSuccess) {
            status = CYB_ERR_HIP;
            break;
        }
        std::vector<RPair> rp(np);
        for (size_t k = 0; k < np; ++k) {
            const JMat& jm = h_mats[(size_t)wl[k].mat];
            RPair& q = rp[k];
            q.W = jm.W;
            q.J = jm.J;
            q.tol = jm.tol;
            q.thr2 = jm.thr2;
            q.nvp = jm.nvp;
            q.lenp = jm.lenp;
            q.nb = jm.nb;
            q.nv = jm.nv;
            q.mat = wl[k].mat;
            q.slot = wl[k].slot;
            q.pad[0] = q.pad[1] = 0;
        }
        void* d_rp = nullptr;
        static const bool want_stamps = getenv("CYB_JACOBI_STAMPS") != nullptr;
        static unsigned long long* d_stamps = nullptr;
        if (want_stamps) {
            if (!d_stamps && hipMalloc(reinterpret_cast<void**>(&d_stamps), sizeof(unsigned long long) * 8 * 2048) != hipSuccess) d_stamps = nullptr;
            rs.stamps = d_stamps;
        }
        static bool attr_set = false;
        if (!attr_set) {
            if (hipFuncSetAttribute(reinterpret_cast<const void*>(jacobi_round_kernel), hipFuncAttributeMaxDynamicSharedMemorySize,
                                    (int)ROUND_LDS_BYTES) != hipSuccess) {
                set_error("jacobi: cannot reserve %zu bytes of LDS for the round kernel", ROUND_LDS_BYTES);
                status = CYB_ERR_HIP;
                break;
            }
            attr_set = true;
        }
        bool any_j = false;
        for (int m : order) any_j = any_j || h_mats[(size_t)m].J != nullptr;
        static const bool defer_j = getenv("CYB_JACOBI_NODEFER") == nullptr;
        static const int g_env = getenv("CYB_JACOBI_G") ? atoi(getenv("CYB_JACOBI_G")) : 0;
        static const int u_max = getenv("CYB_JACOBI_UMAX") ? atoi(getenv("CYB_JACOBI_UMAX")) : 16;
        static const bool no_sweep = getenv("CYB_JACOBI_NOSWEEP") != nullptr;
        bool did_sweep = false;
        bool big_ok = true;
        for (int m : order)
            big_ok = big_ok && (size_t)h_mats[(size_t)m].nvp * (size_t)std::max(h_mats[(size_t)m].lenp, h_mats[(size_t)m].nvp) * 8 < ((size_t)1 << 31);
        const size_t sweep_slots = (size_t)SWEEP_WG_PER_CU * (size_t)ctx->n_cu;
        static const bool no_share = getenv("CYB_JACOBI_NOSHARE") != nullptr;
        if (!legacy && !no_sweep && big_ok && (np <= sweep_slots || !no_share)) {
            std::vector<int> Gm((size_t)n, 1);
            auto chain = [&](int m) {
                const JMat& jm = h_mats[(size_t)m];
                const double per_round = 8.0 + 22.0 * (double)(jm.lenp + ((jm.J || jm.rec_j) ? jm.nvp : 0)) / 2240.0 / (double)Gm[(size_t)m]
                                         + (Gm[(size_t)m] > 1 ? 4.0 : 0.0);
                return per_round * (double)(jm.nb - 1);
            };
            size_t used = np;
            while (true) {
                int best = -1;
                double worst = 0.0;
                for (int m : order) {
                    const JMat& jm = h_mats[(size_t)m];
                    const int cw_ = jm.lenp / 64;
                    if (Gm[(size_t)m] >= RGMAX || Gm[(size_t)m] >= cw_ || used + (size_t)jm.nb / 2 > sweep_slots) continue;
                    const double c = chain(m);
                    if (c > worst) {
                        worst = c;
                        best = m;
                    }
                }
                if (best < 0) break;
                ++Gm[(size_t)best];
                used += (size_t)h_mats[(size_t)best].nb / 2;
            }
            if (g_env > 0)
                for (int m : order) Gm[(size_t)m] = std::max(1, std::min({g_env, RGMAX, h_mats[(size_t)m].lenp / 64}));
            size_t total = 0;
            for (int m : order) total += (size_t)h_mats[(size_t)m].nb / 2 * (size_t)Gm[(size_t)m];
            if (total <= sweep_slots || (!no_share && total == np)) {
                std::vector<int> flag_base((size_t)n, 0);
                int fb = (int)np;
                for (int m : order) {
                    flag_base[(size_t)m] = fb;
                    fb += h_mats[(size_t)m].nb * Gm[(size_t)m];
                }
                std::vector<int2> wgmap;
                for (size_t k = 0; k < np; ++k) {
                    rp[k].pad[0] = Gm[(size_t)wl[k].mat];
                    rp[k].pad[1] = flag_base[(size_t)wl[k].mat];
                    for (int g = 0; g < Gm[(size_t)wl[k].mat]; ++g) wgmap.push_back(make_int2((int)k, g));
                }
                std::vector<int2> wgent;
                if (wgmap.size() > sweep_slots) {
                    std::vector<size_t> ent_before;
                    size_t acc = 0;
                    for (int m : order) {
                        ent_before.push_back(acc);
                        acc += (size_t)h_mats[(size_t)m].nb / 2;
                    }
                    ent_before.push_back(acc);
                    size_t best_i = 0, best_m = 0;
                    double best_cost = 1e300;
                    for (size_t i = 0; i <= order.size(); ++i) {
                        const size_t D = ent_before[i], S = acc - D;
                        if (D > sweep_slots || (S > 0 && D >= sweep_slots)) break;
                        const size_t m = S ? (S + (sweep_slots - D) - 1) / (sweep_slots - D) : 1;
                        const double own = (double)(h_mats[(size_t)order[0]].nb - 1);
                        const double shared = i < order.size() ? (double)m * (double)(h_mats[(size_t)order[i]].nb - 1) : 0.0;
                        const double cost = std::max(own, shared);
                        if (cost < best_cost) {
                            best_cost = cost;
                            best_i = i;
                            best_m = m;
                        }
                    }
                    const size_t D = ent_before[best_i];
                    for (size_t e = 0; e < D; ++e) wgent.push_back(make_int2((int)e, (int)e + 1));
                    for (size_t e = D; e < wgmap.size(); e += best_m)
                        wgent.push_back(make_int2((int)e, (int)std::min(e + best_m, wgmap.size())));
                }
                const size_t n_wg = wgent.empty() ? wgmap.size() : wgent.size();
                std::vector<int> g_now;
                for (int m : order) g_now.push_back(Gm[(size_t)m]);
                const size_t map_off = (sizeof(RPair) * np + 255) / 256 * 256;
                const size_t ent_off = (map_off + sizeof(int2) * wgmap.size() + 255) / 256 * 256;
                if (!(cached_img && order == cached_order && g_now == cached_G && ctx->n_uploads - cached_at < (uint64_t)cyb_ctx_s::kSlots / 2 - 1)) {
                    std::vector<char> img(ent_off + sizeof(int2) * wgent.size());
                    memcpy(img.data(), rp.data(), sizeof(RPair) * np);
                    memcpy(img.data() + map_off, wgmap.data(), sizeof(int2) * wgmap.size());
                    if (!wgent.empty()) memcpy(img.data() + ent_off, wgent.data(), sizeof(int2) * wgent.size());
                    status = ctx->upload(img.data(), img.size(), &cached_img);
                    if (status != CYB_OK) break;
                    cached_order = order;
                    cached_G = g_now;
                    cached_at = ctx->n_uploads;
                    cached_map_off = map_off;
                }
                void* d_rp2 = cached_img;
                void* d_map = static_cast<char*>(cached_img) + cached_map_off;
                static bool attr2_set = false;
                if (!attr2_set) {
                    if (hipFuncSetAttribute(reinterpret_cast<const void*>(jacobi_sweep_kernel<false>), hipFuncAttributeMaxDynamicSharedMemorySize,
                                            (int)SWEEP_LDS_BYTES) != hipSuccess ||
                        hipFuncSetAttribute(reinterpret_cast<const void*>(jacobi_sweep_kernel<true>), hipFuncAttributeMaxDynamicSharedMemorySize,
                                            (int)SWEEP_LDS_BYTES) != hipSuccess) {
                        set_error("jacobi: cannot reserve %zu bytes of LDS for the sweep kernel", SWEEP_LDS_BYTES);
                        status = CYB_ERR_HIP;
                        break;
                    }
                    attr2_set = true;
                }
                SScratch ss;
                ss.gpart = rs.gpart;
                ss.ticket = d_ready;
                ss.ready = d_ready;
                ss.readyJ = d_ready + n_ready;
                static const bool no_defer_j = getenv("CYB_JACOBI_NODEFERJ") != nullptr;
                ss.defer_j = no_defer_j ? 0 : 1;
                static const int cross_env = getenv("CYB_JACOBI_CROSS") ? atoi(getenv("CYB_JACOBI_CROSS")) : -1;
                static const bool cross_small = getenv("CYB_JACOBI_CROSS_SMALL") != nullptr;
                ss.cross_every = (max_inner == 1 || cross_small) ? cross_env : 0;
                static const int cross_min_nb = getenv("CYB_JACOBI_CROSS_MINNB") ? atoi(getenv("CYB_JACOBI_CROSS_MINNB")) : 0;
                ss.cross_min_nb = cross_min_nb;
                ss.err = rs.err;
                ss.wgmap = static_cast<const int2*>(d_map);
                ss.wgent = wgent.empty() ? nullptr : reinterpret_cast<const int2*>(static_cast<char*>(cached_img) + ent_off);
                ss.stamps = wgent.empty() ? rs.stamps : nullptr;
                ss.stamp_round = std::min(3, max_nb - 2);
                size_t max_ent = 1;
                for (const int2& we : wgent) max_ent = std::max(max_ent, (size_t)(we.y - we.x));
                const bool one_launch = n_sw_dev > 1 && sweep == 1 && max_ent <= (size_t)SW_MAX_ENT;
                ss.n_sweeps = one_launch ? n_sw_dev : 1;
                ss.n_mats = n;
                ss.arrive = reinterpret_cast<unsigned int*>(d_off + w_off);
                ss.nsw = reinterpret_cast<int*>(ss.arrive + n);
                one_launch_done = one_launch;
                if (cplx)
                    hipLaunchKernelGGL(jacobi_sweep_kernel<true>, dim3((unsigned)n_wg), dim3(NT), SWEEP_LDS_BYTES, st,
                                       static_cast<const RPair*>(d_rp2), max_inner, d_off, ss);
                else
                    hipLaunchKernelGGL(jacobi_sweep_kernel<false>, dim3((unsigned)n_wg), dim3(NT), SWEEP_LDS_BYTES, st,
                                       static_cast<const RPair*>(d_rp2), max_inner, d_off, ss);
                if (ss.stamps && wgmap.size() <= 2048) {
                    std::vector<unsigned long long> hs(8 * wgmap.size());
                    if (hipMemcpyAsync(hs.data(), rs.stamps, sizeof(unsigned long long) * hs.size(), hipMemcpyDeviceToHost, st) == hipSuccess &&
                        hipStreamSynchronize(st) == hipSuccess) {
                        double acc[6] = {0, 0, 0, 0, 0, 0};
                        int cntw = 0;
                        const int mbig = order.front();
                        for (size_t b = 0; b < wgmap.size(); ++b) {
                            if (wl[(size_t)wgmap[b].x].mat != mbig) continue;
                            for (int k = 0; k < 6; ++k) acc[k] += (double)(hs[8 * b + k + 1] - hs[8 * b + k]) * 0.01;
                            ++cntw;
                        }
                        if (cntw)
                            fprintf(stderr, "[jacobi sweep stamps] sweep %d round %d, largest matrix (G=%d, %d workgroups of %zu): wait %.2f load+gram %.2f "
                                            "exch %.2f defl+eig %.2f sort %.2f upd+publish %.2f us\n",
                                    sweep, ss.stamp_round, Gm[(size_t)mbig], cntw, wgmap.size(), acc[0] / cntw, acc[1] / cntw,
                                    acc[2] / cntw, acc[3] / cntw, acc[4] / cntw, acc[5] / cntw);
                    }
                }
                did_sweep = true;
            }
        }
        if (!did_sweep && cplx) {
            set_error("block-Jacobi on embedded complex rows needs the persistent sweep kernel (list too large for one launch)");
            status = CYB_ERR_UNSUPPORTED;
            break;
        }
        if (!did_sweep) {
        cached_img = nullptr;
        {
            void* d_mats_v = nullptr;
            status = ctx->upload(h_mats.data(), sizeof(JMat) * (size_t)n, &d_mats_v);
            if (status == CYB_OK) status = ctx->upload(wl.data(), sizeof(JWork) * wl.size(), &d_wl);
            if (status == CYB_OK) status = ctx->upload(rp.data(), sizeof(RPair) * np, &d_rp);
            if (status != CYB_OK) break;
            d_mats = static_cast<const JMat*>(d_mats_v);
            if (hipMemsetAsync(sc.cnt, 0, b_c, st) != hipSuccess) {
                status = CYB_ERR_HIP;
                break;
            }
        }
        int pend_round = -1;
        size_t pend_cnt = 0;
        auto flush_pending = [&]() {
            if (pend_round < 0) return;
            const int U = (int)std::min<size_t>(16, std::max<size_t>(1, (size_t)(3 * ctx->n_cu) / pend_cnt));
            hipLaunchKernelGGL(jacobi_update_kernel, dim3((unsigned)(pend_cnt * U)), dim3(NT), 0, st, d_mats,
                               static_cast<const JWork*>(d_wl), pend_round, U, sc, pend_round & 1, 0, 1);
            pend_round = -1;
        };
        for (int r = 0; r < max_nb - 1; ++r) {
            size_t cnt = 0;
            for (int m : order) {
                if (h_mats[(size_t)m].nb - 1 > r) cnt += (size_t)h_mats[(size_t)m].nb / 2;
                else break;
            }
            if (cnt == 0) break;
            const bool fused = !legacy && cnt <= (size_t)fused_max && cnt <= (size_t)ctx->n_cu;
            if (fused) {
                flush_pending();
                int G = (int)std::min<size_t>(kGmax, (size_t)ctx->n_cu / cnt);
                if (g_env > 0 && (size_t)g_env * cnt <= (size_t)ctx->n_cu) G = std::min(g_env, kGmax);
                G = std::max(G, 1);
                hipLaunchKernelGGL(jacobi_round_kernel, dim3((unsigned)(cnt * G)), dim3(NT), ROUND_LDS_BYTES, st,
                                   static_cast<const RPair*>(d_rp), r, G, max_inner, d_off, rs);
                if (rs.stamps && r == max_nb / 2 && cnt * (size_t)G <= 2048) {
                    std::vector<unsigned long long> hs(8 * cnt * G);
                    if (hipMemcpyAsync(hs.data(), rs.stamps, sizeof(unsigned long long) * hs.size(), hipMemcpyDeviceToHost, st) == hipSuccess &&
                        hipStreamSynchronize(st) == hipSuccess) {
                        double acc[6] = {0, 0, 0, 0, 0, 0}, tot = 0, mx = 0;
                        for (size_t b = 0; b < cnt * G; ++b) {
                            for (int k = 0; k < 6; ++k) acc[k] += (double)(hs[8 * b + k + 1] - hs[8 * b + k]) * 0.01;
                            const double t = (double)(hs[8 * b + 6] - hs[8 * b]) * 0.01;
                            tot += t;
                            mx = std::max(mx, t);
                        }
                        const double nb_ = (double)(cnt * G);
                        fprintf(stderr, "[jacobi stamps] sweep %d round %d: %zu pairs x G=%d | gram %.2f exch %.2f defl %.2f eig %.2f sort %.2f upd %.2f | wg mean %.2f max %.2f us\n",
                                sweep, r, cnt, G, acc[0] / nb_, acc[1] / nb_, acc[2] / nb_, acc[3] / nb_, acc[4] / nb_, acc[5] / nb_, tot / nb_, mx);
                    }
                }
                continue;
            }
            const int slots = 2 * ctx->n_cu;
            int G = g_env > 0 ? g_env : ((size_t)2 * cnt <= (size_t)slots ? 2 : 1);
            G = std::min(G, kGmax);
            const int U = (int)std::min<size_t>((size_t)u_max, std::max<size_t>(1, (size_t)(3 * ctx->n_cu) / cnt));
            const int buf = r & 1;
            const int n_gram = (int)(cnt * G);
            int UJ = 1;
            size_t n_jwg = 0;
            if (pend_round >= 0) {
                const long long free_slots = (long long)slots - (long long)n_gram;
                UJ = (int)std::max<long long>(1, std::min<long long>(8, free_slots / (long long)pend_cnt));
                n_jwg = pend_cnt * (size_t)UJ;
            }
            hipLaunchKernelGGL(jacobi_gram_kernel, dim3((unsigned)(n_gram + n_jwg)), dim3(NT), 0, st, d_mats,
                               static_cast<const JWork*>(d_wl), r, G, max_inner, d_off, sc, buf, n_gram, pend_round, UJ);
            const bool defer = defer_j && any_j;
            hipLaunchKernelGGL(jacobi_update_kernel, dim3((unsigned)(cnt * U)), dim3(NT), 0, st, d_mats,
                               static_cast<const JWork*>(d_wl), r, U, sc, buf, 1, defer ? 0 : 1);
            pend_round = defer ? r : -1;
            pend_cnt = cnt;
        }
        flush_pending();
        }
        if (hipGetLastError() != hipSuccess) {
            set_error("jacobi round kernels: launch failed");
            status = CYB_ERR_HIP;
            break;
        }
        unsigned int h_err = 0;
        if (ctx->d2h(h_off.data(), d_off, b_off + 16) != CYB_OK) {
            set_error("jacobi: reading the convergence flags failed: %s", hipGetErrorString(hipGetLastError()));
            status = CYB_ERR_HIP;
            break;
        }
        memcpy(&h_err, reinterpret_cast<const char*>(h_off.data()) + b_off, sizeof(unsigned int));
        if (h_err) {
            set_error("jacobi round kernel: a workgroup waited more than a second for the Gram partials of its pair "
                      "(partner workgroup not resident?)");
            status = CYB_ERR_HIP;
            break;
        }
        std::vector<int> still;
        if (one_launch_done) {
            const int* h_nsw = reinterpret_cast<const int*>(reinterpret_cast<const unsigned int*>(h_off.data() + w_off) + n);
            for (int m : active) {
                if (h_nsw[m] > 0) sweeps_out[(size_t)m] = h_nsw[m];
                else still.push_back(m);
            }
            active.swap(still);
            break;
        }
        static const bool trace = getenv("CYB_JACOBI_TRACE") != nullptr;
        for (int m : active) {
            double off;
            memcpy(&off, &h_off[(size_t)m], sizeof(double));
            if (trace)
                fprintf(stderr, "[jacobi] sweep %2d mat %3d (nv=%d len=%d) off=%.3e tol=%.3e\n", sweep, m,
                        h_mats[(size_t)m].nv, h_mats[(size_t)m].len, off, h_mats[(size_t)m].tol);
            const double tol = h_mats[(size_t)m].tol;
            const bool stagnated = sweep >= 6 && off <= 64.0 * tol && off >= 0.5 * prev_off[(size_t)m];
            static const bool no_predict = getenv("CYB_JACOBI_NOPREDICT") != nullptr;
            const double prev = prev_off[(size_t)m];
            const bool predicted = !no_predict && off <= 0.1 * std::sqrt(tol) && prev < 1.0 && off <= prev * std::sqrt(prev) &&
                                   off <= kPredictQuad * prev * prev;
            if (off <= tol || stagnated || predicted) sweeps_out[(size_t)m] = sweep;
            else still.push_back(m);
            prev_off[(size_t)m] = off;
        }
        active.swap(still);
    }
    if (status != CYB_OK) return status;
    if (!active.empty()) {
        for (int m : active) sweeps_out[(size_t)m] = -1;
        set_error("block-Jacobi did not converge within %d sweeps for %zu matrices", max_sweeps, active.size());
        return CYB_ERR_NOCONV;
    }
    return CYB_OK;
}

}
```

### cyten_amd/csrc/scaling.hip

```cpp
#include "common.h"

#include <algorithm>
#include <cmath>

namespace cyb {
namespace {

#define GLOBAL_AS __attribute__((address_space(1)))
typedef const GLOBAL_AS double* gcp;
typedef GLOBAL_AS double* gp;

struct AmaxDesc {
    const double* A;
    int64_t lda;
    int32_t m, n;
    double* out;
};

__global__ void __launch_bounds__(256) matrix_amax_kernel(const AmaxDesc* __restrict__ descs)
{
    __shared__ double red[4];
    const AmaxDesc d = descs[blockIdx.y];
    gcp A = (gcp)d.A;
    double mx = 0.0;
    bool bad = false;
    if (d.lda == d.n) {
        const int64_t tot = (int64_t)d.m * d.n;
        for (int64_t e = (int64_t)blockIdx.x * 256 + threadIdx.x; e < tot; e += (int64_t)gridDim.x * 256) {
            const double v = A[e];
            bad = bad || !(fabs(v) <= 1.7e308);
            mx = fmax(mx, fabs(v));
        }
    } else {
        for (int r = blockIdx.x; r < d.m; r += gridDim.x) {
            gcp row = A + (int64_t)r * d.lda;
            for (int c = threadIdx.x; c < d.n; c += 256) {
                const double v = row[c];
                bad = bad || !(fabs(v) <= 1.7e308);
                mx = fmax(mx, fabs(v));
            }
        }
    }
    if (bad) mx = __builtin_nan("");
#pragma unroll
    for (int o = 32; o > 0; o >>= 1) {
        const double other = __shfl_xor(mx, o);
        mx = (mx != mx || other != other) ? __builtin_nan("") : fmax(mx, other);
    }
    if ((threadIdx.x & 63) == 0) red[threadIdx.x >> 6] = mx;
    __syncthreads();
    if (threadIdx.x == 0) {
        double r = red[0];
        for (int w = 1; w < 4; ++w) r = (r != r || red[w] != red[w]) ? __builtin_nan("") : fmax(r, red[w]);
        ((gp)d.out)[blockIdx.x] = r;
    }
}

struct ScaleDesc {
    const double* src;
    int64_t lds;
    double* dst;
    int64_t ldd;
    int32_t rows, cols;
    double s;
};

__global__ void __launch_bounds__(256) scale_copy_kernel(const ScaleDesc* __restrict__ descs)
{
    const ScaleDesc d = descs[blockIdx.y];
    gcp src = (gcp)d.src;
    gp dst = (gp)d.dst;
    const int64_t tot = (int64_t)d.rows * d.cols;
    for (int64_t e = (int64_t)blockIdx.x * 256 + threadIdx.x; e < tot; e += (int64_t)gridDim.x * 256) {
        const int64_t r = e / d.cols, c = e % d.cols;
        dst[r * d.ldd + c] = src[r * d.lds + c] * d.s;
    }
}

}

int matrix_amax(cyb_ctx_t ctx, const std::vector<MatRef>& mats, std::vector<double>& amax)
{
    const size_t n = mats.size();
    amax.assign(n, 0.0);
    if (n == 0) return CYB_OK;
    constexpr int kParts = 32;
    void* d_out = nullptr;
    CYB_TRY(ctx->workspace(sizeof(double) * n * kParts, &d_out, 2));
    std::vector<AmaxDesc> ds(n);
    for (size_t i = 0; i < n; ++i)
        ds[i] = AmaxDesc{mats[i].A, mats[i].lda, (int32_t)mats[i].m, (int32_t)mats[i].n, static_cast<double*>(d_out) + i * kParts};
    void* d_ds = nullptr;
    CYB_TRY(ctx->upload(ds.data(), sizeof(AmaxDesc) * n, &d_ds));
    hipLaunchKernelGGL(matrix_amax_kernel, dim3(kParts, (unsigned)n), dim3(256), 0, ctx->stream, static_cast<const AmaxDesc*>(d_ds));
    CYB_HIP(hipGetLastError());
    std::vector<double> parts(n * kParts);
    CYB_TRY(ctx->d2h(parts.data(), d_out, sizeof(double) * parts.size()));
    for (size_t i = 0; i < n; ++i) {
        double r = 0.0;
        for (int p = 0; p < kParts; ++p) {
            const double v = parts[i * kParts + p];
            r = (r != r || v != v) ? std::nan("") : std::max(r, v);
        }
        amax[i] = r;
    }
    return CYB_OK;
}

double range_scale(double amax)
{
    if (!(amax > 0.0) || !(amax <= 1.7e308)) return 1.0;
    if (amax <= 1e90 && amax >= 1e-90) return 1.0;
    int e = 0;
    (void)std::frexp(amax, &e);
    return std::ldexp(1.0, -e);
}

int scale_copy_batched(cyb_ctx_t ctx, const std::vector<ScaleJob>& jobs)
{
    if (jobs.empty()) return CYB_OK;
    std::vector<ScaleDesc> ds(jobs.size());
    for (size_t i = 0; i < jobs.size(); ++i)
        ds[i] = ScaleDesc{jobs[i].src, jobs[i].lds, jobs[i].dst, jobs[i].ldd, (int32_t)jobs[i].rows, (int32_t)jobs[i].cols, jobs[i].s};
    void* d_ds = nullptr;
    CYB_TRY(ctx->upload(ds.data(), sizeof(ScaleDesc) * ds.size(), &d_ds));
    hipLaunchKernelGGL(scale_copy_kernel, dim3(64, (unsigned)ds.size()), dim3(256), 0, ctx->stream, static_cast<const ScaleDesc*>(d_ds));
    CYB_HIP(hipGetLastError());
    return CYB_OK;
}

}
```

### cyten_amd/csrc/svd_jacobi.hip

```cpp
#include "blocked_qr.h"
#include "jacobi_engine.h"

#include <algorithm>
#include <cmath>
#include <cstdlib>

namespace cyb {
namespace {

#define GLOBAL_AS __attribute__((address_space(1)))
typedef GLOBAL_AS double* gp;
typedef const GLOBAL_AS double* gcp;

struct PrepDesc {
    const double* A;
    int64_t lda;
    int32_t m, n;
    double* W;
    double* J;
    int32_t nvp, lenp;
    int32_t transpose;
    int32_t pad;
    const double* shift;
};

__global__ void __launch_bounds__(256) prep_kernel(const PrepDesc* __restrict__ descs)
{
    __shared__ double tile[32][33];
    const PrepDesc d = descs[blockIdx.y];
    gcp A = (gcp)d.A;
    gp W = (gp)d.W;
    const int tx = threadIdx.x & 31, ty = threadIdx.x >> 5;
    const int tiles_n = (d.n + 31) / 32, tiles_m = (d.m + 31) / 32;
    const double shift = d.shift ? *(gcp)d.shift : 0.0;
    for (int t = blockIdx.x; t < tiles_m * tiles_n; t += gridDim.x) {
        const int ti = t / tiles_n, tj = t % tiles_n;
        const int i0 = ti * 32, j0 = tj * 32;
        if (d.transpose) {
#pragma unroll
            for (int r = 0; r < 4; ++r) {
                const int i = i0 + ty + 8 * r, j = j0 + tx;
                tile[ty + 8 * r][tx] = (i < d.m && j < d.n) ? A[(int64_t)i * d.lda + j] : 0.0;
            }
            __syncthreads();
#pragma unroll
            for (int r = 0; r < 4; ++r) {
                const int j = j0 + ty + 8 * r, i = i0 + tx;
                if (j < d.n && i < d.m) W[(int64_t)j * d.lenp + i] = tile[tx][ty + 8 * r];
            }
            __syncthreads();
        } else {
#pragma unroll
            for (int r = 0; r < 4; ++r) {
                const int i = i0 + ty + 8 * r, j = j0 + tx;
                if (i < d.m && j < d.n) {
                    double v = A[(int64_t)i * d.lda + j];
                    if (i == j) v += shift;
                    W[(int64_t)i * d.lenp + j] = v;
                }
            }
        }
    }
    if (d.J) {
        gp J = (gp)d.J;
        for (int i = blockIdx.x * 256 + threadIdx.x; i < d.nvp; i += gridDim.x * 256) J[(int64_t)i * d.nvp + i] = 1.0;
    }
}

struct NormDesc {
    const double* A;
    int64_t lda;
    int32_t m, n;
    double* out;
};
__global__ void __launch_bounds__(256) fro_shift_kernel(const NormDesc* __restrict__ descs)
{
    __shared__ double red[4];
    const NormDesc d = descs[blockIdx.x];
    gcp A = (gcp)d.A;
    double s = 0.0;
    const int64_t tot = (int64_t)d.m * d.n;
    for (int64_t e = threadIdx.x; e < tot; e += 256) {
        const double v = A[(e / d.n) * d.lda + (e % d.n)];
        s += v * v;
    }
#pragma unroll
    for (int o = 32; o > 0; o >>= 1) s += __shfl_xor(s, o);
    if ((threadIdx.x & 63) == 0) red[threadIdx.x >> 6] = s;
    __syncthreads();
    if (threadIdx.x == 0) {
        const double f = sqrt(red[0] + red[1] + red[2] + red[3]);
        *(gp)d.out = (f > 0.0) ? 2.0 * f : 1.0;
    }
}

struct PostDesc {
    const double* W;
    const double* J;
    int32_t nvp, lenp, nv, len;
    int32_t transposed;
    int32_t mode;
    double* sig;
    int32_t* rank;
    double* S;
    double* U;
    int64_t ldu;
    double* Vh;
    int64_t ldvh;
    const double* shift;
    double* scratch;
    int32_t* n_null;
    double null_scale;
    int32_t cplx = 0;
    int32_t pad_ = 0;
    const double* sig_lq = nullptr;
};

__global__ void __launch_bounds__(256) row_norm_kernel(const PostDesc* __restrict__ descs)
{
    const PostDesc d = descs[blockIdx.y];
    gcp W = (gcp)d.W;
    const int lane = threadIdx.x & 63;
    for (int j = blockIdx.x * 4 + (threadIdx.x >> 6); j < d.nv; j += gridDim.x * 4) {
        double s = 0.0;
        for (int c = lane; c < d.len; c += 64) {
            const double v = W[(int64_t)j * d.lenp + c];
            s += v * v;
        }
#pragma unroll
        for (int o = 32; o > 0; o >>= 1) s += __shfl_xor(s, o);
        if (lane == 0) {
            const double o = d.sig_lq ? ((gcp)d.sig_lq)[j] : 0.0;
            ((gp)d.sig)[j] = (o > 0.0 && s > 0.0) ? o : sqrt(s);
        }
    }
}

__global__ void __launch_bounds__(256) rank_kernel(const PostDesc* __restrict__ descs)
{
    constexpr int CH = 2048;
    __shared__ double keys[CH];
    const PostDesc d = descs[blockIdx.y];
    gcp sig = (gcp)d.sig;
    const double shift = d.shift ? *(gcp)d.shift : 0.0;
    const int msk = d.cplx ? ~1 : ~0;
    const int per = (d.nv + (int)gridDim.x * 256 - 1) / ((int)gridDim.x * 256);
    for (int it = 0; it < per; ++it) {
        const int j = (it * (int)gridDim.x + (int)blockIdx.x) * 256 + (int)threadIdx.x;
        const bool mine = j < d.nv;
        const double sj = mine ? sig[j & msk] : 0.0;
        int r = 0;
        for (int k0 = 0; k0 < d.nv; k0 += CH) {
            const int kn = min(CH, d.nv - k0);
            __syncthreads();
            for (int k = threadIdx.x; k < kn; k += 256) keys[k] = sig[(k0 + k) & msk];
            __syncthreads();
            if (mine) {
                if (d.mode == 0) {
                    for (int k = 0; k < kn; ++k) {
                        const double sk = keys[k];
                        r += (sk > sj || (sk == sj && k0 + k < j)) ? 1 : 0;
                    }
                } else {
                    for (int k = 0; k < kn; ++k) {
                        const double sk = keys[k];
                        r += (sk < sj || (sk == sj && k0 + k < j)) ? 1 : 0;
                    }
                }
            }
        }
        if (mine) {
            d.rank[j] = r;
            d.S[r] = (d.mode == 0) ? sj : sj - shift;
        }
    }
}

__global__ void __launch_bounds__(256) write_factors_kernel(const PostDesc* __restrict__ descs)
{
    __shared__ double tile[32][33];
    __shared__ int rk[32];
    __shared__ double sc[32];
    const PostDesc d = descs[blockIdx.y];
    gcp W = (gcp)d.W;
    gcp J = (gcp)d.J;
    const int tx = threadIdx.x & 31, ty = threadIdx.x >> 5;
    double smax = 0.0;
    if (d.mode == 0) smax = ((gcp)d.S)[0];
    const double thresh = fmax(smax * 1e-280, 1e-300);

    const bool col_from_W = (d.mode == 1) || d.transposed;
    gcp csrc = col_from_W ? W : J;
    const int csrc_ld = col_from_W ? d.lenp : d.nvp;
    const int c_rows = col_from_W ? d.len : d.nv;
    gcp rsrc = col_from_W ? J : W;
    const int rsrc_ld = col_from_W ? d.nvp : d.lenp;
    const int r_cols = col_from_W ? d.nv : d.len;

    const int tj = (d.nv + 31) / 32;
    if (d.U) {
        const int ti_n = (c_rows + 31) / 32;
        for (int t = blockIdx.x; t < tj * ti_n; t += gridDim.x) {
            const int j0 = (t / ti_n) * 32, i0 = (t % ti_n) * 32;
            __syncthreads();
            if (threadIdx.x < 32) {
                const int j = j0 + threadIdx.x;
                double s = 1.0;
                int r = 0;
                if (j < d.nv) {
                    r = d.rank[j];
                    if (col_from_W) {
                        const double sj = ((gcp)d.sig)[j];
                        s = (d.mode == 0 && sj <= thresh) ? d.null_scale : 1.0 / sj;
                    }
                }
                rk[threadIdx.x] = r;
                sc[threadIdx.x] = s;
            }
            __syncthreads();
#pragma unroll
            for (int q = 0; q < 4; ++q) {
                const int j = j0 + ty + 8 * q, i = i0 + tx;
                tile[ty + 8 * q][tx] = (j < d.nv && i < c_rows) ? csrc[(int64_t)j * csrc_ld + i] * sc[ty + 8 * q] : 0.0;
            }
            __syncthreads();
#pragma unroll
            for (int q = 0; q < 4; ++q) {
                const int i = i0 + ty + 8 * q, j = j0 + tx;
                if (i < c_rows && j < d.nv) ((gp)d.U)[(int64_t)i * d.ldu + rk[tx]] = tile[tx][ty + 8 * q];
            }
        }
    }
    if (d.mode == 0 && d.Vh) {
        for (int j = blockIdx.x; j < d.nv; j += gridDim.x) {
            const int r = d.rank[j];
            double s = 1.0;
            if (!col_from_W) {
                const double sj = ((gcp)d.sig)[j];
                s = (sj <= thresh) ? d.null_scale : 1.0 / sj;
            }
            for (int c = threadIdx.x; c < r_cols; c += 256)
                ((gp)d.Vh)[(int64_t)r * d.ldvh + c] = rsrc[(int64_t)j * rsrc_ld + c] * s;
        }
    }
    if (d.mode == 0 && blockIdx.x == 0) {
        __syncthreads();
        int cnt = 0;
        for (int j = threadIdx.x; j < d.nv; j += 256) cnt += (((gcp)d.sig)[j] <= thresh) ? 1 : 0;
#pragma unroll
        for (int o = 32; o > 0; o >>= 1) cnt += __shfl_xor(cnt, o);
        if ((threadIdx.x & 63) == 0) rk[threadIdx.x >> 6] = cnt;
        __syncthreads();
        if (threadIdx.x == 0) *d.n_null = rk[0] + rk[1] + rk[2] + rk[3];
    }
}

__global__ void __launch_bounds__(256) complete_null_kernel(const PostDesc* __restrict__ descs)
{
    __shared__ double red[4];
    __shared__ int redi[4];
    __shared__ int s_pick;
    const PostDesc d = descs[blockIdx.x];
    if (d.mode != 0 || *d.n_null == 0) return;
    const int tid = threadIdx.x;
    gp F = (gp)(d.transposed ? d.U : d.Vh);
    if (!F) return;
    const int64_t es = d.transposed ? d.ldu : 1;
    const int64_t vs = d.transposed ? 1 : d.ldvh;
    gp v = (gp)d.scratch;
    gp resid = v + d.lenp;
    const int n_null = *d.n_null;
    const int first_null = d.nv - n_null;
    for (int i = tid; i < d.len; i += 256) {
        double s = 1.0;
        for (int q = 0; q < first_null; ++q) {
            const double f = F[(int64_t)i * es + q * vs];
            s -= f * f;
        }
        resid[i] = s;
    }
    __syncthreads();
    for (int r = first_null; r < d.nv; ++r) {
        double best = -1.0;
        int bi = 0;
        for (int i = tid; i < d.len; i += 256)
            if (resid[i] > best) {
                best = resid[i];
                bi = i;
            }
#pragma unroll
        for (int o = 32; o > 0; o >>= 1) {
            const double ob = __shfl_xor(best, o);
            const int oi = __shfl_xor(bi, o);
            if (ob > best || (ob == best && oi < bi)) {
                best = ob;
                bi = oi;
            }
        }
        if ((tid & 63) == 0) {
            red[tid >> 6] = best;
            redi[tid >> 6] = bi;
        }
        __syncthreads();
        if (tid == 0) {
            int p = 0;
            for (int w = 1; w < 4; ++w)
                if (red[w] > red[p] || (red[w] == red[p] && redi[w] < redi[p])) p = w;
            s_pick = redi[p];
        }
        __syncthreads();
        const int cand = s_pick;
        for (int i = tid; i < d.len; i += 256) v[i] = (i == cand) ? 1.0 : 0.0;
        __syncthreads();
        for (int pass = 0; pass < 2; ++pass) {
            for (int q = 0; q < r; ++q) {
                double s = 0.0;
                for (int i = tid; i < d.len; i += 256) s += F[(int64_t)i * es + q * vs] * v[i];
#pragma unroll
                for (int o = 32; o > 0; o >>= 1) s += __shfl_xor(s, o);
                __syncthreads();
                if ((tid & 63) == 0) red[tid >> 6] = s;
                __syncthreads();
                const double dot = red[0] + red[1] + red[2] + red[3];
                for (int i = tid; i < d.len; i += 256) v[i] -= dot * F[(int64_t)i * es + q * vs];
                __syncthreads();
            }
        }
        double s = 0.0;
        for (int i = tid; i < d.len; i += 256) s += v[i] * v[i];
#pragma unroll
        for (int o = 32; o > 0; o >>= 1) s += __shfl_xor(s, o);
        __syncthreads();
        if ((tid & 63) == 0) red[tid >> 6] = s;
        __syncthreads();
        const double nrm2 = red[0] + red[1] + red[2] + red[3];
        const double inv = (nrm2 > 0.0) ? 1.0 / sqrt(nrm2) : 0.0;
        for (int i = tid; i < d.len; i += 256) {
            const double f = v[i] * inv;
            F[(int64_t)i * es + r * vs] = f;
            resid[i] = (i == cand) ? -1.0 : resid[i] - f * f;
        }
        __syncthreads();
    }
}

inline int round_up(int x, int m) { return (x + m - 1) / m * m; }

struct Layout {
    std::vector<JMat> mats;
    std::vector<PrepDesc> prep;
    std::vector<PostDesc> post;
    size_t bytes = 0;
};

}

static inline int row_blocks(int nv, int nvp)
{
    const int nb = 2 * ((nv + 2 * cyb::JB - 1) / (2 * cyb::JB));
    return std::min(std::max(nb, 4), nvp / cyb::JB);
}

static int run_jacobi(cyb_ctx_t ctx, int mode, int64_t nmat, const cyb_svd_desc* sd, const cyb_eigh_desc* ed,
                      int32_t* info, bool cplx = false)
{
    if (nmat == 0) return CYB_OK;
    hipStream_t st = ctx->stream;
    std::vector<JMat> mats((size_t)nmat);
    std::vector<PrepDesc> prep((size_t)nmat);
    std::vector<PostDesc> post((size_t)nmat);
    std::vector<NormDesc> nd;
    size_t off = 0;
    auto take = [&](size_t bytes) {
        const size_t o = off;
        off += (bytes + 255) / 256 * 256;
        return o;
    };
    struct Offs {
        size_t W, J, sig, rank, shift, scratch, nnull;
    };
    std::vector<Offs> offs((size_t)nmat);
    for (int64_t b = 0; b < nmat; ++b) {
        int m, n;
        if (mode == 0) {
            CYB_REQUIRE(sd[b].m >= 0 && sd[b].n >= 0 && sd[b].m < (1 << 30) && sd[b].n < (1 << 30),
                        "svd block %lld: bad shape", (long long)b);
            m = (int)sd[b].m;
            n = (int)sd[b].n;
            CYB_REQUIRE(m == 0 || n == 0 || (sd[b].A && sd[b].S), "svd block %lld: NULL pointer", (long long)b);
            CYB_REQUIRE(sd[b].lda >= n, "svd block %lld: lda < n", (long long)b);
        } else {
            CYB_REQUIRE(ed[b].n >= 0 && ed[b].n < (1 << 30), "eigh block %lld: bad shape", (long long)b);
            m = n = (int)ed[b].n;
            CYB_REQUIRE(n == 0 || (ed[b].A && ed[b].W), "eigh block %lld: NULL pointer", (long long)b);
            CYB_REQUIRE(ed[b].lda >= n, "eigh block %lld: lda < n", (long long)b);
        }
        const int nv = std::min(m, n), len = std::max(m, n);
        const int nvp = std::max(round_up(nv, 64), 64), lenp = std::max(round_up(len, 64), 64);
        const bool need_J = (mode == 0);
        Offs& o = offs[(size_t)b];
        o.W = take(sizeof(double) * (size_t)nvp * lenp);
        o.J = need_J ? take(sizeof(double) * (size_t)nvp * nvp) : 0;
        o.sig = take(sizeof(double) * (size_t)nvp);
        o.rank = take(sizeof(int32_t) * (size_t)nvp);
        o.shift = take(sizeof(double));
        o.scratch = take(sizeof(double) * (size_t)lenp * 2);
        o.nnull = take(sizeof(int32_t));
        JMat& jm = mats[(size_t)b];
        jm.nvp = nvp;
        jm.lenp = lenp;
        jm.nb = row_blocks(nv, nvp);
        jm.nv = nv;
        jm.len = len;
        jm.rec_j = 0;
        jm.tol = 2.220446049250313e-16 * std::max(16.0, 4.0 * std::sqrt((double)len));
        jm.thr2 = 0.0;
    }
    void* ws = nullptr;
    CYB_TRY(ctx->workspace(off, &ws));
    char* base = static_cast<char*>(ws);
    CYB_HIP(hipMemsetAsync(ws, 0, off, st));
    for (int64_t b = 0; b < nmat; ++b) {
        const Offs& o = offs[(size_t)b];
        JMat& jm = mats[(size_t)b];
        jm.W = reinterpret_cast<double*>(base + o.W);
        jm.J = (mode == 0) ? reinterpret_cast<double*>(base + o.J) : nullptr;
        PrepDesc& p = prep[(size_t)b];
        PostDesc& q = post[(size_t)b];
        if (mode == 0) {
            p.A = sd[b].A;
            p.lda = sd[b].lda;
            p.m = (int)sd[b].m;
            p.n = (int)sd[b].n;
            p.transpose = (sd[b].m >= sd[b].n) ? 1 : 0;
            p.shift = nullptr;
            q.U = sd[b].U;
            q.ldu = sd[b].ldu;
            q.Vh = sd[b].Vh;
            q.ldvh = sd[b].ldvh;
            q.S = sd[b].S;
            q.shift = nullptr;
        } else {
            p.A = ed[b].A;
            p.lda = ed[b].lda;
            p.m = p.n = (int)ed[b].n;
            p.transpose = 0;
            p.shift = reinterpret_cast<double*>(base + o.shift);
            q.U = ed[b].V;
            q.ldu = ed[b].ldv;
            q.Vh = nullptr;
            q.ldvh = 0;
            q.S = ed[b].W;
            q.shift = p.shift;
            nd.push_back(NormDesc{ed[b].A, ed[b].lda, (int)ed[b].n, (int)ed[b].n, reinterpret_cast<double*>(base + o.shift)});
        }
        p.W = jm.W;
        p.J = jm.J;
        p.nvp = jm.nvp;
        p.lenp = jm.lenp;
        p.pad = 0;
        q.W = jm.W;
        q.J = jm.J;
        q.nvp = jm.nvp;
        q.lenp = jm.lenp;
        q.nv = jm.nv;
        q.len = jm.len;
        q.transposed = p.transpose;
        q.mode = mode;
        q.sig = reinterpret_cast<double*>(base + o.sig);
        q.rank = reinterpret_cast<int32_t*>(base + o.rank);
        q.scratch = reinterpret_cast<double*>(base + o.scratch);
        q.n_null = reinterpret_cast<int32_t*>(base + o.nnull);
        q.null_scale = 0.0;
        q.cplx = cplx ? 1 : 0;
    }
    void* d_prep = nullptr;
    CYB_TRY(ctx->upload(prep.data(), sizeof(PrepDesc) * prep.size(), &d_prep));
    if (mode == 1) {
        void* d_nd = nullptr;
        CYB_TRY(ctx->upload(nd.data(), sizeof(NormDesc) * nd.size(), &d_nd));
        hipLaunchKernelGGL(fro_shift_kernel, dim3((unsigned)nmat), dim3(256), 0, st, static_cast<const NormDesc*>(d_nd));
    }
    hipLaunchKernelGGL(prep_kernel, dim3(64, (unsigned)nmat), dim3(256), 0, st, static_cast<const PrepDesc*>(d_prep));
    CYB_HIP(hipGetLastError());
    std::vector<int32_t> sweeps;
    const int jst = jacobi_orthogonalise(ctx, mats, 40, sweeps, cplx);
    if (info)
        for (int64_t b = 0; b < nmat; ++b) info[b] = sweeps[(size_t)b];
    if (jst != CYB_OK && jst != CYB_ERR_NOCONV) return jst;
    void* d_post = nullptr;
    CYB_TRY(ctx->upload(post.data(), sizeof(PostDesc) * post.size(), &d_post));
    const PostDesc* dp = static_cast<const PostDesc*>(d_post);
    hipLaunchKernelGGL(row_norm_kernel, dim3(helper_grid_x((size_t)nmat), (unsigned)nmat), dim3(256), 0, st, dp);
    hipLaunchKernelGGL(rank_kernel, dim3(8, (unsigned)nmat), dim3(256), 0, st, dp);
    hipLaunchKernelGGL(write_factors_kernel, dim3(helper_grid_x((size_t)nmat), (unsigned)nmat), dim3(256), 0, st, dp);
    if (mode == 0) hipLaunchKernelGGL(complete_null_kernel, dim3((unsigned)nmat), dim3(256), 0, st, dp);
    CYB_HIP(hipGetLastError());
    if (info) CYB_HIP(hipStreamSynchronize(st));
    return jst;
}


namespace {

struct RowsDesc {
    double* W;
    const double* sig;
    const int32_t* idx;
    double* buf;
    int32_t kp, k, cnt, pad;
    const int32_t* col;
};
__global__ void __launch_bounds__(256) gather_rows_kernel(const RowsDesc* __restrict__ descs)
{
    const RowsDesc d = descs[blockIdx.y];
    gcp W = (gcp)d.W;
    gp buf = (gp)d.buf;
    const int lane = threadIdx.x & 63;
    for (int c = blockIdx.x * 4 + (threadIdx.x >> 6); c < d.cnt; c += gridDim.x * 4) {
        const int j = d.idx[c];
        const double inv = 1.0 / ((gcp)d.sig)[j];
        for (int i = lane; i < d.k; i += 64) buf[(int64_t)c * d.k + i] = W[(int64_t)j * d.kp + i] * inv;
    }
}
__global__ void __launch_bounds__(256) scatter_rows_kernel(const RowsDesc* __restrict__ descs)
{
    const RowsDesc d = descs[blockIdx.y];
    gp W = (gp)d.W;
    gcp buf = (gcp)d.buf;
    const int lane = threadIdx.x & 63;
    for (int c = blockIdx.x * 4 + (threadIdx.x >> 6); c < d.cnt; c += gridDim.x * 4) {
        const int j = d.idx[c];
        const int cc = d.col ? d.col[c] : c;
        for (int i = lane; i < d.k; i += 64) W[(int64_t)j * d.kp + i] = buf[(int64_t)cc * d.k + i];
    }
}

struct JcqDesc {
    const double* J;
    const int32_t* rank;
    double* Cq;
    int64_t L;
    int32_t kp, k;
};
__global__ void __launch_bounds__(256) j_to_cq_kernel(const JcqDesc* __restrict__ descs)
{
    const JcqDesc d = descs[blockIdx.y];
    gcp J = (gcp)d.J;
    gp Cq = (gp)d.Cq;
    const int lane = threadIdx.x & 63;
    for (int j = blockIdx.x * 4 + (threadIdx.x >> 6); j < d.k; j += gridDim.x * 4) {
        const int r = d.rank[j];
        for (int i = lane; i < d.k; i += 64) Cq[(int64_t)r * d.L + i] = J[(int64_t)j * d.kp + i];
    }
}


struct RowMoveDesc {
    const double* src;
    double* dst;
    const int32_t* idx;
    int64_t lds, ldd;
    int32_t cnt, ncols;
    int32_t mode, pad;
};
__global__ void __launch_bounds__(256) row_move_kernel(const RowMoveDesc* __restrict__ descs)
{
    const RowMoveDesc d = descs[blockIdx.y];
    gcp src = (gcp)d.src;
    gp dst = (gp)d.dst;
    const int lane = threadIdx.x & 63;
    for (int g = blockIdx.x * 4 + (threadIdx.x >> 6); g < d.cnt; g += gridDim.x * 4) {
        const int j = d.idx[g];
        if (d.mode == 0) {
            for (int c = lane; c < d.ncols; c += 64) dst[(int64_t)g * d.ldd + c] = src[(int64_t)j * d.lds + c];
        } else if (d.mode == 1) {
            for (int c = lane; c < d.ncols; c += 64) dst[(int64_t)j * d.ldd + c] = src[(int64_t)g * d.lds + c];
        } else {
            for (int c = lane; c < d.ncols; c += 64) dst[(int64_t)j * d.ldd + c] = 0.0;
        }
    }
}
__global__ void __launch_bounds__(256) j_scatter_kernel(const RowMoveDesc* __restrict__ descs)
{
    const RowMoveDesc d = descs[blockIdx.y];
    gcp src = (gcp)d.src;
    gp dst = (gp)d.dst;
    const int lane = threadIdx.x & 63;
    for (int g = blockIdx.x * 4 + (threadIdx.x >> 6); g < d.cnt; g += gridDim.x * 4) {
        const int j = d.idx[g];
        for (int h = lane; h < d.cnt; h += 64) dst[(int64_t)j * d.ldd + d.idx[h]] = src[(int64_t)g * d.lds + h];
    }
}

struct PairDesc {
    double* W;
    int64_t ld;
    int32_t nv, len;
};
__global__ void __launch_bounds__(256) embed_pairs_kernel(const PairDesc* __restrict__ descs)
{
    const PairDesc d = descs[blockIdx.y];
    gp W = (gp)d.W;
    const int lane = threadIdx.x & 63;
    for (int a = blockIdx.x * 4 + (threadIdx.x >> 6); a < d.nv / 2; a += gridDim.x * 4) {
        gp e = W + (int64_t)(2 * a) * d.ld, o = e + d.ld;
        for (int j = lane; j < d.len / 2; j += 64) {
            const double x = 0.5 * (e[2 * j] + o[2 * j + 1]), y = 0.5 * (o[2 * j] - e[2 * j + 1]);
            e[2 * j] = x;
            e[2 * j + 1] = -y;
            o[2 * j] = y;
            o[2 * j + 1] = x;
        }
    }
}

struct LqDesc {
    double* Wq;
    double* Jc;
    double* Wc;
    double* Cq2;
    double* sig2;
    double* bad;
    double thr2;
    int32_t rp, kp, k, r0;
    int32_t cplx, jrec;
    double* Ws;
    double* G;
    double* dev;
    double* sigo;
    const int32_t* idx;
};
constexpr double JREC_BOUND = 2e-11;
constexpr int JREC_NB = 128;
__global__ void __launch_bounds__(256) lq_pack_kernel(const LqDesc* __restrict__ descs)
{
    const LqDesc d = descs[blockIdx.y];
    gcp Jc = (gcp)d.Jc;
    gp C = (gp)d.Cq2;
    const int lane = threadIdx.x & 63;
    for (int i = blockIdx.x * 4 + (threadIdx.x >> 6); i < d.k; i += gridDim.x * 4) {
        for (int c = lane; c < d.k; c += 64) {
            double v;
            if (i < d.r0) {
                if (c < d.r0 && d.jrec) continue;
                v = c < d.r0 ? Jc[(int64_t)i * d.rp + c] : 0.0;
            } else v = c == i ? 1.0 : 0.0;
            C[(int64_t)i * d.k + c] = v;
        }
    }
}
__global__ void __launch_bounds__(256) lq_rows_kernel(const LqDesc* __restrict__ descs)
{
    const LqDesc d = descs[blockIdx.y];
    gcp Wq = (gcp)d.Wq;
    gp Jc = (gp)d.Jc;
    const int lane = threadIdx.x & 63;
    for (int i = blockIdx.x * 4 + (threadIdx.x >> 6); i < d.r0; i += gridDim.x * 4) {
        double s = 0.0;
        for (int c = lane; c < d.r0; c += 64) {
            const double v = Wq[(int64_t)i * d.rp + c];
            s += v * v;
        }
#pragma unroll
        for (int o = 32; o > 0; o >>= 1) s += __shfl_xor(s, o);
        const double sg = sqrt(s);
        if (lane == 0) {
            ((gp)d.sig2)[i] = sg;
            if (!(sg > 0.0)) *(gp)d.bad = 1.0;
            if (d.jrec && !(sg * sg > d.thr2)) *(gp)d.bad = 1.0;
        }
        const double inv = sg > 0.0 ? 1.0 / sg : 0.0;
        for (int c = lane; c < d.r0; c += 64) Jc[(int64_t)i * d.rp + c] = Wq[(int64_t)i * d.rp + c] * inv;
        if (d.jrec) {
            gp Ws = (gp)d.Ws;
            const double inv2 = inv * inv;
            for (int c = lane; c < d.r0; c += 64) Ws[(int64_t)i * d.r0 + c] = Wq[(int64_t)i * d.rp + c] * inv2;
        }
    }
}
__global__ void __launch_bounds__(256) jrec_check_kernel(const LqDesc* __restrict__ descs)
{
    const LqDesc d = descs[blockIdx.y];
    if (!d.jrec) return;
    gcp G = (gcp)d.G;
    const int lane = threadIdx.x & 63;
    double mx = 0.0;
    bool nan = false;
    for (int i = blockIdx.x * 4 + (threadIdx.x >> 6); i < d.r0; i += gridDim.x * 4) {
        for (int c = i / JREC_NB * JREC_NB + lane; c < d.r0; c += 64) {
            const double v = fabs(G[(int64_t)i * d.r0 + c] - (c == i ? 1.0 : 0.0));
            nan = nan || !(v == v);
            mx = fmax(mx, v);
        }
    }
#pragma unroll
    for (int o = 32; o > 0; o >>= 1) mx = fmax(mx, __shfl_xor(mx, o));
    nan = __any(nan);
    if (lane == 0) {
        if (nan) mx = __builtin_huge_val();
        atomicMax((unsigned long long*)d.dev, (unsigned long long)__double_as_longlong(mx));
        if (!(mx <= JREC_BOUND)) *(gp)d.bad = 1.0;
    }
}
__global__ void __launch_bounds__(256) lq_check_kernel(const LqDesc* __restrict__ descs)
{
    const LqDesc d = descs[blockIdx.y];
    gcp Jc = (gcp)d.Jc;
    const int lane = threadIdx.x & 63;
    const int wid = blockIdx.x * 4 + (threadIdx.x >> 6), nw = gridDim.x * 4;
    for (int i0 = 0; i0 < d.r0; i0 += 64) {
        bool fl = false;
        if (i0 + lane < d.r0) {
            const double sg = ((gcp)d.sig2)[i0 + lane];
            fl = !(sg * sg > d.thr2);
        }
        unsigned long long msk = __ballot(fl);
        while (msk) {
            const int i = i0 + __ffsll((long long)msk) - 1;
            msk &= msk - 1;
            double worst = 0.0;
            for (int j = wid; j < d.r0; j += nw) {
                if (j == i) continue;
                double t = 0.0;
                for (int c = lane; c < d.r0; c += 64) t = fma(Jc[(int64_t)i * d.rp + c], Jc[(int64_t)j * d.rp + c], t);
#pragma unroll
                for (int o = 32; o > 0; o >>= 1) t += __shfl_xor(t, o);
                worst = fmax(worst, fabs(t));
            }
            if (lane == 0 && !(worst <= 1e-12)) *(gp)d.bad = 1.0;
        }
    }
}
__global__ void __launch_bounds__(256) lq_unpack_kernel(const LqDesc* __restrict__ descs)
{
    const LqDesc d = descs[blockIdx.y];
    gcp C = (gcp)d.Cq2;
    gp Wc = (gp)d.Wc;
    const int lane = threadIdx.x & 63;
    for (int i = blockIdx.x * 4 + (threadIdx.x >> 6); i < d.r0; i += gridDim.x * 4) {
        const double sg = ((gcp)d.sig2)[i];
        const double sm = d.cplx ? fmax(sg, ((gcp)d.sig2)[i ^ 1]) : sg;
        double f = sm * sm > d.thr2 ? sg : 0.0;
        double n2 = 0.0;
        for (int c = lane; c < d.k; c += 64) n2 = fma(C[(int64_t)i * d.k + c], C[(int64_t)i * d.k + c], n2);
#pragma unroll
        for (int o = 32; o > 0; o >>= 1) n2 += __shfl_xor(n2, o);
        if (lane == 0) ((gp)d.sigo)[d.idx[i]] = n2 > 0.0 ? f : 0.0;
        f = n2 > 0.0 ? f / sqrt(n2) : 0.0;
        for (int c = lane; c < d.kp; c += 64) Wc[(int64_t)i * d.kp + c] = c < d.k ? f * C[(int64_t)i * d.k + c] : 0.0;
    }
}

static int launch_row_moves(cyb_ctx_t ctx, const std::vector<RowMoveDesc>& v, bool jscatter = false)
{
    if (v.empty()) return CYB_OK;
    void* d = nullptr;
    CYB_TRY(ctx->upload(v.data(), sizeof(RowMoveDesc) * v.size(), &d));
    if (jscatter)
        hipLaunchKernelGGL(j_scatter_kernel, dim3(64, (unsigned)v.size()), dim3(256), 0, ctx->stream, static_cast<const RowMoveDesc*>(d));
    else
        hipLaunchKernelGGL(row_move_kernel, dim3(helper_grid_x(v.size()), (unsigned)v.size()), dim3(256), 0, ctx->stream, static_cast<const RowMoveDesc*>(d));
    CYB_HIP(hipGetLastError());
    return CYB_OK;
}

}

static int run_svd_qr(cyb_ctx_t ctx, int64_t nmat, const cyb_svd_desc* sd, int32_t* info, int flags, int32_t* rank_out)
{
    if (nmat == 0) return CYB_OK;
    const bool cplx = (flags & CYB_SVD_EMBEDDED_COMPLEX) != 0;
    hipStream_t st = ctx->stream;
    auto al = [](size_t b) { return (b + 255) / 256 * 256; };
    struct Lay {
        int m, n, k, L, kp;
        bool tall;
        size_t Ac, aux, W, J, sig, rank, thr, nnull, Cq, Fc, aux2, Cn, idx, Wc, Jc;
        size_t bad, Wq, aux3, Cq2, sig2;
        size_t stop;
        size_t ctl;
        int n_fac = -1;
        size_t sigo;
        size_t dev;
        bool lq = false;
        bool jrec = false;
        int r0 = 0;
        std::vector<int32_t> good0;
    };
    std::vector<Lay> lay((size_t)nmat);
    size_t off = 0;
    size_t sig_begin = off;
    for (int64_t b = 0; b < nmat; ++b) {
        Lay& l = lay[(size_t)b];
        l.m = (int)sd[b].m;
        l.n = (int)sd[b].n;
        l.k = std::min(l.m, l.n);
        l.L = std::max(l.m, l.n);
        l.kp = round_up(l.k, 64);
        l.tall = l.m >= l.n;
        l.sig = off;
        off += sizeof(double) * (size_t)l.kp;
    }
    for (int64_t b = 0; b < nmat; ++b) {
        lay[(size_t)b].thr = off;
        off += sizeof(double);
    }
    for (int64_t b = 0; b < nmat; ++b) {
        lay[(size_t)b].bad = off;
        off += sizeof(double);
    }
    for (int64_t b = 0; b < nmat; ++b) {
        lay[(size_t)b].dev = off;
        off += sizeof(double);
    }
    for (int64_t b = 0; b < nmat; ++b) {
        lay[(size_t)b].ctl = off;
        off += 2 * sizeof(double);
    }
    const size_t sig_bytes = off - sig_begin;
    off = al(off);
    for (int64_t b = 0; b < nmat; ++b) {
        Lay& l = lay[(size_t)b];
        auto take = [&](size_t bytes) {
            const size_t o = off;
            off += al(bytes);
            return o;
        };
        l.Ac = take(sizeof(double) * (size_t)l.L * l.k);
        l.aux = take(bqr_aux_bytes(l.L, l.k, l.L, l.k));
        l.stop = take(sizeof(double) * (size_t)std::max(1, (l.k + cyb::NBK - 1) / cyb::NBK * cyb::bqr_strip_slots(l.L)));
        l.W = take(sizeof(double) * (size_t)l.kp * l.kp);
        l.J = take(sizeof(double) * (size_t)l.kp * l.kp);
        l.rank = take(sizeof(int32_t) * (size_t)l.kp);
        l.nnull = take(sizeof(int32_t));
        l.Cq = take(sizeof(double) * (size_t)l.L * l.k);
        l.Fc = take(sizeof(double) * (size_t)l.k * l.k);
        l.aux2 = take(bqr_aux_bytes(l.k, l.k, l.k, l.k));
        l.Cn = take(sizeof(double) * (size_t)l.k * l.k);
        l.Wc = take(sizeof(double) * (size_t)l.kp * l.kp);
        l.Jc = take(sizeof(double) * (size_t)l.kp * l.kp);
        l.Wq = take(sizeof(double) * (size_t)l.kp * l.kp);
        l.aux3 = take(bqr_aux_bytes(l.k, l.k, l.kp, l.k));
        l.Cq2 = take(sizeof(double) * (size_t)l.k * l.k);
        l.sig2 = take(sizeof(double) * (size_t)l.kp);
        l.sigo = take(sizeof(double) * (size_t)l.kp);
    }
    const size_t idx_begin = off;
    for (int64_t b = 0; b < nmat; ++b) {
        lay[(size_t)b].idx = off;
        off += sizeof(int32_t) * (size_t)lay[(size_t)b].k;
    }
    off = al(off);
    void* ws = nullptr;
    CYB_TRY(ctx->workspace(off, &ws, 0));
    char* base = static_cast<char*>(ws);
    CYB_HIP(hipMemsetAsync(ws, 0, off, st));
    auto dp = [&](size_t o) { return reinterpret_cast<double*>(base + o); };

    std::vector<BqrMat> qm((size_t)nmat);
    std::vector<XposeDesc> x_in, x_r;
    std::vector<EyeDesc> eyeJ;
    std::vector<JMat> jm((size_t)nmat);
    for (int64_t b = 0; b < nmat; ++b) {
        const Lay& l = lay[(size_t)b];
        BqrMat& q = qm[(size_t)b];
        q.Ac = dp(l.Ac);
        q.ld = l.L;
        q.m = l.L;
        q.n = l.k;
        q.k = l.k;
        bqr_carve(q, base + l.aux, l.k);
        q.v_zeroed = 1;
        q.reflect_always = cplx ? 1 : 0;
        q.ctl = dp(l.ctl);
        q.parts = dp(l.stop);
        q.stop_rel2 = ((double)l.L * 2.220446049250313e-16) * ((double)l.L * 2.220446049250313e-16);
        if (l.tall)
            x_in.push_back(XposeDesc{sd[b].A, q.Ac, sd[b].lda, l.L, l.n, l.m, 0, 0, 0, 0});
        else
            x_in.push_back(XposeDesc{sd[b].A, q.Ac, sd[b].lda, l.L, l.m, l.n, 0, 0, 1, 0});
        x_r.push_back(XposeDesc{q.Ac, dp(l.W), l.L, l.kp, l.k, l.k, 1, l.k, 0, 0});
        eyeJ.push_back(EyeDesc{dp(l.J), l.kp, l.kp, l.kp, 0, 0});
        JMat& j = jm[(size_t)b];
        j.W = dp(l.W);
        j.J = dp(l.J);
        j.nvp = l.kp;
        j.lenp = l.kp;
        j.nb = row_blocks(l.k, l.kp);
        j.nv = l.k;
        j.len = l.k;
        j.rec_j = 0;
        j.tol = 2.220446049250313e-16 * std::max(16.0, 4.0 * std::sqrt((double)l.k));
        j.thr2 = 0.0;
    }
    CYB_TRY(xpose_batched(ctx, x_in));
    CYB_TRY(bqr_factor(ctx, qm));
    CYB_TRY(xpose_batched(ctx, x_r));
    CYB_TRY(eye_cols_batched(ctx, eyeJ));
    std::vector<PostDesc> post((size_t)nmat);
    for (int64_t b = 0; b < nmat; ++b) {
        const Lay& l = lay[(size_t)b];
        PostDesc& q = post[(size_t)b];
        q.W = dp(l.W);
        q.J = dp(l.J);
        q.nvp = l.kp;
        q.lenp = l.kp;
        q.nv = l.k;
        q.len = l.k;
        q.transposed = l.tall ? 0 : 1;
        q.mode = 0;
        q.sig = dp(l.sig);
        q.rank = reinterpret_cast<int32_t*>(base + l.rank);
        q.S = sd[b].S;
        q.U = l.tall ? nullptr : sd[b].U;
        q.ldu = sd[b].ldu;
        q.Vh = l.tall ? sd[b].Vh : nullptr;
        q.ldvh = sd[b].ldvh;
        q.shift = nullptr;
        q.scratch = nullptr;
        q.n_null = reinterpret_cast<int32_t*>(base + l.nnull);
        q.null_scale = 1.0;
        q.cplx = cplx ? 1 : 0;
    }
    void* d_post = nullptr;
    const PostDesc* dpost = nullptr;
    std::vector<double> h_sig(sig_bytes / sizeof(double));
    auto sig_of = [&](const Lay& l) { return h_sig.data() + (l.sig - sig_begin) / sizeof(double); };
    CYB_TRY(ctx->upload(post.data(), sizeof(PostDesc) * post.size(), &d_post));
    dpost = static_cast<const PostDesc*>(d_post);
    hipLaunchKernelGGL(row_norm_kernel, dim3(helper_grid_x((size_t)nmat), (unsigned)nmat), dim3(256), 0, st, dpost);
    CYB_HIP(hipGetLastError());
    CYB_TRY(ctx->d2h(h_sig.data(), base + sig_begin, sig_bytes));
    {
        std::vector<int32_t> idx_all;
        std::vector<size_t> idx_off((size_t)nmat, 0);
        for (int64_t b = 0; b < nmat; ++b) {
            Lay& l = lay[(size_t)b];
            const double* sg = sig_of(l);
            const double stopped = h_sig[(l.ctl - sig_begin) / sizeof(double)];
            l.n_fac = stopped != 0.0 ? (int)stopped - 1 : -1;
            double fro2 = 0.0;
            for (int j = 0; j < l.k; ++j) fro2 += sg[j] * sg[j];
            const double sc = (double)l.L * 2.220446049250313e-16;
            const double thr2 = fro2 * sc * sc;
            jm[(size_t)b].thr2 = thr2;
            std::vector<int32_t> nul;
            for (int j = 0; j < l.k; ++j) {
                const double v = cplx ? std::max(sg[j & ~1], sg[std::min(j | 1, l.k - 1)]) : sg[j];
                (v * v > thr2 ? l.good0 : nul).push_back(j);
            }
            l.r0 = (int)l.good0.size();
            idx_off[(size_t)b] = idx_all.size();
            idx_all.insert(idx_all.end(), l.good0.begin(), l.good0.end());
            idx_all.insert(idx_all.end(), nul.begin(), nul.end());
        }
        static const bool no_lq = getenv("CYB_SVD_NOLQ") != nullptr;
        static const bool lq_always = getenv("CYB_SVD_LQ_ALWAYS") != nullptr;
        static const int lq_skip_k = getenv("CYB_SVD_LQ_SKIP_K") ? atoi(getenv("CYB_SVD_LQ_SKIP_K")) : 128;
        static const double lq_skip_ratio = getenv("CYB_SVD_LQ_SKIP_RATIO") ? atof(getenv("CYB_SVD_LQ_SKIP_RATIO")) : 1e4;
        for (int64_t b = 0; b < nmat; ++b) {
            Lay& l = lay[(size_t)b];
            bool skip = false;
            if (!lq_always && l.r0 == l.k && l.k >= lq_skip_k) {
                const double* sg = sig_of(l);
                double lo = 1e300, hi = 0.0;
                for (int j = 0; j < l.k; ++j) {
                    lo = std::min(lo, sg[j]);
                    hi = std::max(hi, sg[j]);
                }
                skip = hi <= lq_skip_ratio * lo;
            }
            l.lq = !no_lq && l.r0 >= 2 && !skip;
        }
        static const bool no_jrec = getenv("CYB_SVD_NOJREC") != nullptr;
        static const double jrec_ratio = getenv("CYB_SVD_JREC_RATIO") ? atof(getenv("CYB_SVD_JREC_RATIO")) : 1e1;
        static const int jrec_min = getenv("CYB_SVD_JREC_MIN") ? atoi(getenv("CYB_SVD_JREC_MIN")) : 256;
        for (int64_t b = 0; b < nmat; ++b) {
            Lay& l = lay[(size_t)b];
            if (!l.lq || no_jrec || cplx || l.r0 < jrec_min) continue;
            const double* sg = sig_of(l);
            double lo = 1e300, hi = 0.0;
            for (int32_t j : l.good0) {
                lo = std::min(lo, sg[j]);
                hi = std::max(hi, sg[j]);
            }
            l.jrec = hi <= jrec_ratio * lo;
        }
        void* d_idx_v = nullptr;
        CYB_TRY(ctx->upload(idx_all.data(), sizeof(int32_t) * idx_all.size(), &d_idx_v));
        CYB_HIP(hipMemcpyAsync(base + idx_begin, d_idx_v, sizeof(int32_t) * idx_all.size(), hipMemcpyDeviceToDevice, st));
    }
    const std::vector<JMat> jm0 = jm;
    std::vector<BqrMat> qm3;
    std::vector<int> qm3_of((size_t)nmat, -1);
    std::vector<int32_t> sweeps;
    auto iterate = [&](bool allow_lq, int& jst) -> int {
        jm = jm0;
        qm3.clear();
        std::fill(qm3_of.begin(), qm3_of.end(), -1);
        std::vector<RowMoveDesc> gat, zer;
        std::vector<EyeDesc> eyeJc;
        std::vector<XposeDesc> x_r2;
        std::vector<LqDesc> lqd;
        std::vector<int> jrec_blocks;
        std::vector<BqrTarget> tg3;
        for (int64_t b = 0; b < nmat; ++b) {
            Lay& l = lay[(size_t)b];
            l.lq = l.lq && allow_lq;
            if (l.r0 == l.k && !l.lq) continue;
            const int32_t* didx = reinterpret_cast<const int32_t*>(base + l.idx);
            const int rp = std::max(round_up(l.r0, 64), 64);
            gat.push_back(RowMoveDesc{dp(l.W), dp(l.Wc), didx, l.kp, l.kp, l.r0, l.kp, 0, 0});
            if (l.r0 < l.k) zer.push_back(RowMoveDesc{nullptr, dp(l.W), didx + l.r0, 0, l.kp, l.k - l.r0, l.kp, 2, 0});
            const bool jrec = l.lq && l.jrec && allow_lq;
            if (!jrec) eyeJc.push_back(EyeDesc{dp(l.Jc), rp, rp, rp, 0, 0});
            JMat& j = jm[(size_t)b];
            j.W = dp(l.Wc);
            j.J = dp(l.Jc);
            j.nvp = rp;
            j.nb = row_blocks(l.r0, rp);
            j.nv = l.r0;
            if (l.lq) {
                BqrMat q;
                q.Ac = dp(l.Wc);
                q.ld = l.kp;
                q.m = l.k;
                q.n = l.r0;
                q.k = l.r0;
                bqr_carve(q, base + l.aux3, l.k);
                q.v_zeroed = allow_lq ? 1 : 0;
                q.reflect_always = cplx ? 1 : 0;
                x_r2.push_back(XposeDesc{dp(l.Wc), dp(l.Wq), l.kp, rp, l.r0, l.r0, 1, l.r0, 0, 0});
                j.W = dp(l.Wq);
                j.lenp = rp;
                j.len = l.r0;
                const double thr2 = j.thr2;
                j.thr2 = 0.0;
                lqd.push_back(LqDesc{dp(l.Wq), dp(l.Jc), dp(l.Wc), dp(l.Cq2), dp(l.sig2), dp(l.bad), thr2, rp, l.kp, l.k, l.r0, cplx ? 1 : 0,
                                     jrec ? 1 : 0, dp(l.Fc), dp(l.Fc), dp(l.dev), dp(l.sigo), didx});
                if (jrec) {
                    j.J = nullptr;
                    j.rec_j = 1;
                    x_r2.push_back(XposeDesc{dp(l.Wc), dp(l.Cn), l.kp, l.r0, l.r0, l.r0, 1, l.r0, 0, 0});
                    jrec_blocks.push_back((int)b);
                }
                tg3.push_back(BqrTarget{(int)qm3.size(), dp(l.Cq2), l.k, l.k});
                qm3_of[(size_t)b] = (int)qm3.size();
                qm3.push_back(q);
            }
        }
        CYB_TRY(launch_row_moves(ctx, gat));
        CYB_TRY(launch_row_moves(ctx, zer));
        CYB_TRY(eye_cols_batched(ctx, eyeJc));
        if (!qm3.empty()) {
            CYB_TRY(bqr_factor(ctx, qm3));
            CYB_TRY(xpose_batched(ctx, x_r2));
        }
        if (cplx) {
            std::vector<PairDesc> prs;
            for (const JMat& j : jm)
                if (j.nv >= 2) prs.push_back(PairDesc{const_cast<double*>(j.W), j.lenp, j.nv & ~1, j.len & ~1});
            if (!prs.empty()) {
                void* d = nullptr;
                CYB_TRY(ctx->upload(prs.data(), sizeof(PairDesc) * prs.size(), &d));
                hipLaunchKernelGGL(embed_pairs_kernel, dim3(64, (unsigned)prs.size()), dim3(256), 0, st, static_cast<const PairDesc*>(d));
                CYB_HIP(hipGetLastError());
            }
        }
        jst = jacobi_orthogonalise(ctx, jm, 40, sweeps, cplx);
        if (jst != CYB_OK && jst != CYB_ERR_NOCONV) return jst;
        if (!qm3.empty()) {
            void* d = nullptr;
            CYB_TRY(ctx->upload(lqd.data(), sizeof(LqDesc) * lqd.size(), &d));
            const LqDesc* dl = static_cast<const LqDesc*>(d);
            hipLaunchKernelGGL(lq_pack_kernel, dim3(64, (unsigned)lqd.size()), dim3(256), 0, st, dl);
            hipLaunchKernelGGL(lq_rows_kernel, dim3(64, (unsigned)lqd.size()), dim3(256), 0, st, dl);
            if (!jrec_blocks.empty()) {
                int64_t tiles = 0;
                for (int b : jrec_blocks) tiles += (int64_t)((lay[(size_t)b].r0 + 127) / 128) * ((lay[(size_t)b].r0 + 127) / 128);
                const int nbc = tiles >= 2 * (int64_t)ctx->n_cu ? 128 : 64;
                GemmBatch g_rec, g_chk;
                for (int b : jrec_blocks) {
                    const Lay& l = lay[(size_t)b];
                    const int64_t r0 = l.r0, k = l.k;
                    for (int64_t c0 = 0; c0 < r0; c0 += nbc)
                        g_rec.add(dp(l.Cq2) + c0, r0, std::min<int64_t>(nbc, r0 - c0), k, dp(l.Fc) + c0, r0, 1, dp(l.Cn) + c0 * r0 + c0, 1, r0,
                                  r0 - c0, 1.0, 0.0);
                    for (int64_t i0 = 0; i0 < r0; i0 += JREC_NB)
                        g_chk.add(dp(l.Fc) + i0 * r0 + i0, std::min<int64_t>(JREC_NB, r0 - i0), r0 - i0, r0, dp(l.Cq2) + i0 * k, k, 1,
                                  dp(l.Cq2) + i0 * k, 1, k, r0, 1.0, 0.0);
                }
                CYB_TRY(g_rec.launch(ctx));
                CYB_TRY(g_chk.launch(ctx));
                CYB_TRY(ctx->upload(lqd.data(), sizeof(LqDesc) * lqd.size(), &d));
                dl = static_cast<const LqDesc*>(d);
                hipLaunchKernelGGL(jrec_check_kernel, dim3(16, (unsigned)lqd.size()), dim3(256), 0, st, dl);
            }
            hipLaunchKernelGGL(lq_check_kernel, dim3(helper_grid_x(lqd.size()), (unsigned)lqd.size()), dim3(256), 0, st, dl);
            CYB_HIP(hipGetLastError());
            CYB_TRY(bqr_apply_q(ctx, qm3, tg3));
            CYB_TRY(ctx->upload(lqd.data(), sizeof(LqDesc) * lqd.size(), &d));
            hipLaunchKernelGGL(lq_unpack_kernel, dim3(64, (unsigned)lqd.size()), dim3(256), 0, st, static_cast<const LqDesc*>(d));
            CYB_HIP(hipGetLastError());
        }
        return CYB_OK;
    };
    int jst = CYB_OK;
    CYB_TRY(iterate(true, jst));
    if (!qm3.empty()) {
        std::vector<double> bad((size_t)nmat * 2, 0.0);
        CYB_TRY(ctx->d2h(bad.data(), base + lay[0].bad, sizeof(double) * (size_t)nmat * 2));
        const std::vector<double> jdev(bad.begin() + nmat, bad.end());
        bad.resize((size_t)nmat);
        static const bool force_redo = getenv("CYB_SVD_LQ_FORCE_REDO") != nullptr;
        static const bool force_jredo = getenv("CYB_SVD_JREC_FORCE_REDO") != nullptr;
        bool redo = jst == CYB_ERR_NOCONV || force_redo;
        for (double v : bad) redo = redo || v != 0.0;
        for (const Lay& l : lay) redo = redo || (force_jredo && l.lq && l.jrec);
        static const bool trace_redo = getenv("CYB_SVD_TRACE_REDO") != nullptr;
        if (trace_redo)
            for (int64_t b = 0; b < nmat; ++b) {
                const Lay& l = lay[(size_t)b];
                const char* route = !l.lq ? "no LQ step" : !l.jrec ? "excluded" : redo ? "recovered then redone" : "recovered";
                fprintf(stderr, "[cyb] svd jrec: block %lld (%d x %d, r0 %d): %s (deviation %.2e, flagged %d)\n", (long long)b, l.m, l.n, l.r0,
                        route, jdev[(size_t)b], (int)(bad[(size_t)b] != 0.0));
            }
        if (redo && trace_redo) {
            int nb = 0;
            for (double v : bad) nb += v != 0.0;
            fprintf(stderr, "[cyb] svd: plain iteration after the LQ one (%d of %lld blocks flagged, noconv %d)\n", nb, (long long)nmat,
                    (int)(jst == CYB_ERR_NOCONV));
        }
        if (redo) CYB_TRY(iterate(false, jst));
    } else if (getenv("CYB_SVD_TRACE_REDO") != nullptr) {
        for (int64_t b = 0; b < nmat; ++b)
            fprintf(stderr, "[cyb] svd jrec: block %lld (%d x %d, r0 %d): no LQ step (deviation %.2e, flagged 0)\n", (long long)b,
                    lay[(size_t)b].m, lay[(size_t)b].n, lay[(size_t)b].r0, 0.0);
    }
    if (info)
        for (int64_t b = 0; b < nmat; ++b) info[b] = sweeps[(size_t)b];
    if (jst != CYB_OK && jst != CYB_ERR_NOCONV) return jst;
    {
        std::vector<RowMoveDesc> sw, sj;
        for (int64_t b = 0; b < nmat; ++b) {
            const Lay& l = lay[(size_t)b];
            if ((l.r0 == l.k && !l.lq) || l.r0 == 0) continue;
            const int32_t* didx = reinterpret_cast<const int32_t*>(base + l.idx);
            const int rp = std::max(round_up(l.r0, 64), 64);
            sw.push_back(RowMoveDesc{dp(l.Wc), dp(l.W), didx, l.kp, l.kp, l.r0, l.kp, 1, 0});
            sj.push_back(RowMoveDesc{dp(l.Jc), dp(l.J), didx, rp, l.kp, l.r0, l.r0, 0, 0});
        }
        CYB_TRY(launch_row_moves(ctx, sw));
        CYB_TRY(launch_row_moves(ctx, sj, true));
    }
    for (int64_t b = 0; b < nmat; ++b) post[(size_t)b].sig_lq = lay[(size_t)b].lq ? dp(lay[(size_t)b].sigo) : nullptr;
    CYB_TRY(ctx->upload(post.data(), sizeof(PostDesc) * post.size(), &d_post));
    dpost = static_cast<const PostDesc*>(d_post);
    hipLaunchKernelGGL(row_norm_kernel, dim3(helper_grid_x((size_t)nmat), (unsigned)nmat), dim3(256), 0, st, dpost);
    CYB_HIP(hipGetLastError());
    CYB_TRY(ctx->d2h(h_sig.data(), base + sig_begin, sig_bytes));
    {
        std::vector<int32_t> idx_all;
        struct Comp {
            int64_t b;
            size_t good_off, null_off;
            int r, q;
        };
        std::vector<Comp> comps;
        for (int64_t b = 0; b < nmat; ++b) {
            const Lay& l = lay[(size_t)b];
            const double* sg = sig_of(l);
            std::vector<int32_t> good, nul;
            for (int j = 0; j < l.k; ++j) {
                const double v = cplx ? std::max(sg[j & ~1], sg[std::min(j | 1, l.k - 1)]) : sg[j];
                (v > 0.0 ? good : nul).push_back(j);
            }
            if (rank_out) rank_out[b] = (int32_t)good.size();
            Comp c{b, idx_all.size(), 0, (int)good.size(), (int)nul.size()};
            idx_all.insert(idx_all.end(), good.begin(), good.end());
            c.null_off = idx_all.size();
            idx_all.insert(idx_all.end(), nul.begin(), nul.end());
            if (nul.empty() || (flags & CYB_SVD_SKIP_NULL_VECTORS)) continue;
            comps.push_back(c);
        }
        if (!comps.empty()) {
            void* d_idx_v = nullptr;
            CYB_TRY(ctx->upload(idx_all.data(), sizeof(int32_t) * idx_all.size(), &d_idx_v));
            CYB_HIP(hipMemcpyAsync(base + idx_begin, d_idx_v, sizeof(int32_t) * idx_all.size(), hipMemcpyDeviceToDevice, st));
            std::vector<RowsDesc> gath, scat;
            std::vector<int32_t> cols_all;
            std::vector<std::pair<size_t, size_t>> lq_scat;
            std::vector<BqrMat> qm2;
            std::vector<BqrTarget> tg2;
            std::vector<EyeDesc> eyes;
            for (const Comp& c : comps) {
                const Lay& l = lay[(size_t)c.b];
                if (l.lq) {
                    const size_t c0 = cols_all.size();
                    int t = 0;
                    size_t g = 0;
                    const int32_t* nulp = idx_all.data() + c.null_off;
                    for (int qn = 0; qn < c.q; ++qn) {
                        const int32_t j = nulp[qn];
                        while (g < l.good0.size() && l.good0[g] < j) ++g;
                        if (g < l.good0.size() && l.good0[g] == j) cols_all.push_back((int32_t)g);
                        else cols_all.push_back((int32_t)(l.r0 + t++));
                    }
                    lq_scat.push_back({scat.size(), c0});
                    scat.push_back(RowsDesc{dp(l.W), dp(l.sig), reinterpret_cast<const int32_t*>(base + l.idx) + c.r, dp(l.Cq2), l.kp,
                                            l.k, c.q, 0, nullptr});
                    continue;
                }
                if (c.r > 0) {
                    gath.push_back(RowsDesc{dp(l.W), dp(l.sig), reinterpret_cast<const int32_t*>(base + l.idx), dp(l.Fc), l.kp, l.k, c.r, 0, nullptr});
                    BqrMat q;
                    q.Ac = dp(l.Fc);
                    q.ld = l.k;
                    q.m = l.k;
                    q.n = c.r;
                    q.k = std::min(l.k, c.r);
                    bqr_carve(q, base + l.aux2, c.q);
                    tg2.push_back(BqrTarget{(int)qm2.size(), dp(l.Cn), l.k, c.q});
                    qm2.push_back(q);
                }
                eyes.push_back(EyeDesc{dp(l.Cn), l.k, l.k, c.q, c.r, 0});
                scat.push_back(RowsDesc{dp(l.W), dp(l.sig), reinterpret_cast<const int32_t*>(base + l.idx) + c.r, dp(l.Cn), l.kp, l.k, c.q, 0, nullptr});
            }
            if (!gath.empty()) {
                void* d = nullptr;
                CYB_TRY(ctx->upload(gath.data(), sizeof(RowsDesc) * gath.size(), &d));
                hipLaunchKernelGGL(gather_rows_kernel, dim3(64, (unsigned)gath.size()), dim3(256), 0, st,
                                   static_cast<const RowsDesc*>(d));
                CYB_HIP(hipGetLastError());
                CYB_TRY(bqr_factor(ctx, qm2));
            }
            CYB_TRY(eye_cols_batched(ctx, eyes));
            if (!tg2.empty()) CYB_TRY(bqr_apply_q(ctx, qm2, tg2));
            void* d = nullptr;
            if (!cols_all.empty()) {
                void* d_cols = nullptr;
                CYB_TRY(ctx->upload(cols_all.data(), sizeof(int32_t) * cols_all.size(), &d_cols));
                for (const auto& pr : lq_scat) scat[pr.first].col = static_cast<const int32_t*>(d_cols) + pr.second;
            }
            CYB_TRY(ctx->upload(scat.data(), sizeof(RowsDesc) * scat.size(), &d));
            hipLaunchKernelGGL(scatter_rows_kernel, dim3(64, (unsigned)scat.size()), dim3(256), 0, st,
                               static_cast<const RowsDesc*>(d));
            CYB_HIP(hipGetLastError());
        }
    }
    CYB_TRY(ctx->upload(post.data(), sizeof(PostDesc) * post.size(), &d_post));
    dpost = static_cast<const PostDesc*>(d_post);
    hipLaunchKernelGGL(rank_kernel, dim3(8, (unsigned)nmat), dim3(256), 0, st, dpost);
    hipLaunchKernelGGL(write_factors_kernel, dim3(helper_grid_x((size_t)nmat), (unsigned)nmat), dim3(256), 0, st, dpost);
    CYB_HIP(hipGetLastError());
    std::vector<JcqDesc> jc;
    std::vector<BqrTarget> tg;
    std::vector<XposeDesc> x_out;
    for (int64_t b = 0; b < nmat; ++b) {
        const Lay& l = lay[(size_t)b];
        jc.push_back(JcqDesc{dp(l.J), reinterpret_cast<const int32_t*>(base + l.rank), dp(l.Cq), l.L, l.kp, l.k});
        tg.push_back(BqrTarget{(int)b, dp(l.Cq), l.L, l.k, l.n_fac >= 0 ? l.n_fac : (l.k + cyb::NBK - 1) / cyb::NBK});
        if (l.tall)
            x_out.push_back(XposeDesc{dp(l.Cq), sd[b].U, l.L, sd[b].ldu, l.m, l.k, 0, 0, 0, 0});
        else
            x_out.push_back(XposeDesc{dp(l.Cq), sd[b].Vh, l.L, sd[b].ldvh, l.k, l.n, 0, 0, 1, 0});
    }
    {
        void* d = nullptr;
        CYB_TRY(ctx->upload(jc.data(), sizeof(JcqDesc) * jc.size(), &d));
        hipLaunchKernelGGL(j_to_cq_kernel, dim3(helper_grid_x((size_t)nmat), (unsigned)nmat), dim3(256), 0, st, static_cast<const JcqDesc*>(d));
        CYB_HIP(hipGetLastError());
    }
    CYB_TRY(bqr_apply_q(ctx, qm, tg));
    CYB_TRY(xpose_batched(ctx, x_out));
    if (info) CYB_HIP(hipStreamSynchronize(st));
    return jst;
}

}

namespace cyb {
bool svd_small_fits(int64_t m, int64_t n);
int svd_small_batched(cyb_ctx_t ctx, const cyb_svd_desc* descs, int64_t n, int32_t* sweeps_out);
int eigh_small_batched(cyb_ctx_t ctx, const cyb_eigh_desc* descs, int64_t n, int32_t* sweeps_out);
}

extern "C" {

static int svd_batched_impl(cyb_ctx_t ctx, const cyb_svd_desc* descs, int64_t n, int32_t* info, int flags = 0,
                            int32_t* rank_out = nullptr)
{
    CYB_REQUIRE(ctx, "cyb_svd_batched_f64: ctx is NULL");
    CYB_REQUIRE(n >= 0 && (n == 0 || descs), "cyb_svd_batched_f64: bad descriptor list");
    std::vector<cyb_svd_desc> nz;
    std::vector<int64_t> idx;
    for (int64_t b = 0; b < n; ++b) {
        if (info) info[b] = 0;
        if (rank_out) rank_out[b] = (int32_t)std::min(descs[b].m, descs[b].n);
        if (descs[b].m > 0 && descs[b].n > 0) {
            CYB_REQUIRE(descs[b].U && descs[b].Vh, "svd block %lld: U / Vh is NULL", (long long)b);
            nz.push_back(descs[b]);
            idx.push_back(b);
        }
    }
    static const bool no_qr = getenv("CYB_SVD_NOQR") != nullptr;
    static const bool no_small = getenv("CYB_SVD_NOSMALL") != nullptr;
    size_t n_fit = 0;
    for (const auto& d : nz) n_fit += cyb::svd_small_fits(d.m, d.n) ? 1 : 0;
    const bool embedded = (flags & CYB_SVD_EMBEDDED_COMPLEX) != 0;
    const bool use_small = !embedded && !no_small && (n_fit == nz.size() || n_fit >= 16);
    std::vector<cyb_svd_desc> tiny, small, large;
    std::vector<int64_t> idx_t, idx_s, idx_l;
    static const bool no_merge = getenv("CYB_SVD_NOMERGE") != nullptr;
    bool any_large = false;
    for (const auto& d : nz) any_large = any_large || (!no_qr && std::min(d.m, d.n) >= 48 && !(use_small && cyb::svd_small_fits(d.m, d.n)));
    (void)any_large;
    const int64_t large_min = embedded ? 1 : no_merge ? 48 : 2;
    for (size_t k = 0; k < nz.size(); ++k) {
        if (use_small && cyb::svd_small_fits(nz[k].m, nz[k].n)) {
            CYB_REQUIRE(nz[k].S, "svd block %lld: S is NULL", (long long)idx[k]);
            tiny.push_back(nz[k]);
            idx_t.push_back(idx[k]);
        } else if (!no_qr && std::min(nz[k].m, nz[k].n) >= large_min) {
            large.push_back(nz[k]);
            idx_l.push_back(idx[k]);
        } else {
            small.push_back(nz[k]);
            idx_s.push_back(idx[k]);
        }
    }
    std::vector<int32_t> inf_t(tiny.size()), inf_s(small.size()), inf_l(large.size());
    const int st_t = cyb::svd_small_batched(ctx, tiny.data(), (int64_t)tiny.size(), inf_t.data());
    if (st_t != CYB_OK && st_t != CYB_ERR_NOCONV) return st_t;
    if (info)
        for (size_t k = 0; k < tiny.size(); ++k) info[idx_t[k]] = inf_t[k];
    if (small.empty() && large.empty()) return st_t;
    std::vector<int32_t> rank_l(large.size());
    const int st_l = cyb::run_svd_qr(ctx, (int64_t)large.size(), large.data(), info ? inf_l.data() : nullptr, flags,
                                     rank_out ? rank_l.data() : nullptr);
    if (rank_out)
        for (size_t k = 0; k < large.size(); ++k) rank_out[idx_l[k]] = rank_l[k];
    if (st_l != CYB_OK && st_l != CYB_ERR_NOCONV) return st_l;
    const int st_s = cyb::run_jacobi(ctx, 0, (int64_t)small.size(), small.data(), nullptr, info ? inf_s.data() : nullptr);
    if (info) {
        for (size_t k = 0; k < small.size(); ++k) info[idx_s[k]] = inf_s[k];
        for (size_t k = 0; k < large.size(); ++k) info[idx_l[k]] = inf_l[k];
    }
    return st_s != CYB_OK ? st_s : (st_l != CYB_OK ? st_l : st_t);
}

static int eigh_batched_impl(cyb_ctx_t ctx, const cyb_eigh_desc* descs, int64_t n, int32_t* info, int flags = 0)
{
    CYB_REQUIRE(ctx, "cyb_eigh_batched_f64: ctx is NULL");
    CYB_REQUIRE(n >= 0 && (n == 0 || descs), "cyb_eigh_batched_f64: bad descriptor list");
    std::vector<cyb_eigh_desc> nz;
    std::vector<int64_t> idx;
    for (int64_t b = 0; b < n; ++b) {
        if (info) info[b] = 0;
        if (descs[b].n > 0) {
            nz.push_back(descs[b]);
            idx.push_back(b);
        }
    }
    std::vector<int32_t> inf(nz.size());
    static const bool no_small = getenv("CYB_SVD_NOSMALL") != nullptr;
    const bool embedded = (flags & CYB_EIGH_EMBEDDED_COMPLEX) != 0;
    bool all_small = !no_small && !nz.empty() && !embedded;
    for (const auto& d : nz) all_small = all_small && d.n <= 64;
    const int st = all_small ? cyb::eigh_small_batched(ctx, nz.data(), (int64_t)nz.size(), inf.data())
                             : cyb::run_jacobi(ctx, 1, (int64_t)nz.size(), nullptr, nz.data(), info ? inf.data() : nullptr, embedded);
    if (info)
        for (size_t k = 0; k < nz.size(); ++k) info[idx[k]] = inf[k];
    return st;
}

static int svd_batched_ranged(cyb_ctx_t ctx, const cyb_svd_desc* descs, int64_t n, int32_t* info, int flags, int32_t* rank)
{
    std::vector<cyb::MatRef> refs;
    std::vector<int64_t> which;
    for (int64_t b = 0; b < n; ++b)
        if (descs[b].m > 0 && descs[b].n > 0 && descs[b].A) {
            refs.push_back(cyb::MatRef{descs[b].A, descs[b].lda, descs[b].m, descs[b].n});
            which.push_back(b);
        }
    std::vector<double> amax;
    CYB_TRY(cyb::matrix_amax(ctx, refs, amax));
    std::vector<cyb_svd_desc> mod;
    std::vector<void*> temps;
    std::vector<cyb::ScaleJob> pre, post;
    for (size_t k = 0; k < refs.size(); ++k) {
        const double sc = cyb::range_scale(amax[k]);
        if (sc == 1.0) continue;
        if (mod.empty()) mod.assign(descs, descs + n);
        cyb_svd_desc& d = mod[(size_t)which[k]];
        void* t = nullptr;
        CYB_HIP(hipMalloc(&t, sizeof(double) * (size_t)d.m * (size_t)d.n));
        temps.push_back(t);
        pre.push_back(cyb::ScaleJob{d.A, d.lda, static_cast<double*>(t), d.n, d.m, d.n, sc});
        d.A = static_cast<const double*>(t);
        d.lda = d.n;
        post.push_back(cyb::ScaleJob{d.S, 1, d.S, 1, std::min(d.m, d.n), 1, 1.0 / sc});
    }
    if (mod.empty()) return svd_batched_impl(ctx, descs, n, info, flags, rank);
    int st = cyb::scale_copy_batched(ctx, pre);
    if (st == CYB_OK) st = svd_batched_impl(ctx, mod.data(), n, info, flags, rank);
    if (st == CYB_OK || st == CYB_ERR_NOCONV) {
        const int st2 = cyb::scale_copy_batched(ctx, post);
        if (st2 != CYB_OK) st = st2;
    }
    (void)hipStreamSynchronize(ctx->stream);
    for (void* t : temps) (void)hipFree(t);
    return st;
}

int cyb_svd_batched_f64(cyb_ctx_t ctx, const cyb_svd_desc* descs, int64_t n, int32_t* info)
{
    CYB_REQUIRE(ctx, "cyb_svd_batched_f64: ctx is NULL");
    CYB_REQUIRE(n >= 0 && (n == 0 || descs), "cyb_svd_batched_f64: bad descriptor list");
    return svd_batched_ranged(ctx, descs, n, info, 0, nullptr);
}

int cyb_svd_batched_ex_f64(cyb_ctx_t ctx, const cyb_svd_desc* descs, int64_t n, int32_t* info, int32_t flags, int32_t* rank)
{
    CYB_REQUIRE(ctx, "cyb_svd_batched_ex_f64: ctx is NULL");
    CYB_REQUIRE(n >= 0 && (n == 0 || descs), "cyb_svd_batched_ex_f64: bad descriptor list");
    CYB_REQUIRE((flags & ~(CYB_SVD_SKIP_NULL_VECTORS | CYB_SVD_EMBEDDED_COMPLEX)) == 0, "cyb_svd_batched_ex_f64: unknown flag bits 0x%x", flags);
    if (flags & CYB_SVD_EMBEDDED_COMPLEX)
        for (int64_t b = 0; b < n; ++b)
            CYB_REQUIRE(descs[b].m % 2 == 0 && descs[b].n % 2 == 0, "svd block %lld: an embedded complex block has even extents", (long long)b);
    const int st = svd_batched_ranged(ctx, descs, n, info, flags, rank);
    if (rank && !info) CYB_HIP(hipStreamSynchronize(ctx->stream));
    return st;
}

static int eigh_batched_ranged(cyb_ctx_t ctx, const cyb_eigh_desc* descs, int64_t n, int32_t* info, int flags)
{
    std::vector<cyb::MatRef> refs;
    std::vector<int64_t> which;
    for (int64_t b = 0; b < n; ++b)
        if (descs[b].n > 0 && descs[b].A) {
            refs.push_back(cyb::MatRef{descs[b].A, descs[b].lda, descs[b].n, descs[b].n});
            which.push_back(b);
        }
    std::vector<double> amax;
    CYB_TRY(cyb::matrix_amax(ctx, refs, amax));
    std::vector<cyb_eigh_desc> mod;
    std::vector<void*> temps;
    std::vector<cyb::ScaleJob> pre, post;
    for (size_t k = 0; k < refs.size(); ++k) {
        const double sc = cyb::range_scale(amax[k]);
        if (sc == 1.0) continue;
        if (mod.empty()) mod.assign(descs, descs + n);
        cyb_eigh_desc& d = mod[(size_t)which[k]];
        void* t = nullptr;
        CYB_HIP(hipMalloc(&t, sizeof(double) * (size_t)d.n * (size_t)d.n));
        temps.push_back(t);
        pre.push_back(cyb::ScaleJob{d.A, d.lda, static_cast<double*>(t), d.n, d.n, d.n, sc});
        d.A = static_cast<const double*>(t);
        d.lda = d.n;
        post.push_back(cyb::ScaleJob{d.W, 1, d.W, 1, d.n, 1, 1.0 / sc});
    }
    if (mod.empty()) return eigh_batched_impl(ctx, descs, n, info, flags);
    int st = cyb::scale_copy_batched(ctx, pre);
    if (st == CYB_OK) st = eigh_batched_impl(ctx, mod.data(), n, info, flags);
    if (st == CYB_OK || st == CYB_ERR_NOCONV) {
        const int st2 = cyb::scale_copy_batched(ctx, post);
        if (st2 != CYB_OK) st = st2;
    }
    (void)hipStreamSynchronize(ctx->stream);
    for (void* t : temps) (void)hipFree(t);
    return st;
}

int cyb_eigh_batched_f64(cyb_ctx_t ctx, const cyb_eigh_desc* descs, int64_t n, int32_t* info)
{
    CYB_REQUIRE(ctx, "cyb_eigh_batched_f64: ctx is NULL");
    CYB_REQUIRE(n >= 0 && (n == 0 || descs), "cyb_eigh_batched_f64: bad descriptor list");
    return eigh_batched_ranged(ctx, descs, n, info, 0);
}

int cyb_eigh_batched_ex_f64(cyb_ctx_t ctx, const cyb_eigh_desc* descs, int64_t n, int32_t* info, int32_t flags)
{
    CYB_REQUIRE(ctx, "cyb_eigh_batched_ex_f64: ctx is NULL");
    CYB_REQUIRE(n >= 0 && (n == 0 || descs), "cyb_eigh_batched_ex_f64: bad descriptor list");
    CYB_REQUIRE((flags & ~CYB_EIGH_EMBEDDED_COMPLEX) == 0, "cyb_eigh_batched_ex_f64: unknown flag bits 0x%x", flags);
    if (flags & CYB_EIGH_EMBEDDED_COMPLEX)
        for (int64_t b = 0; b < n; ++b)
            CYB_REQUIRE(descs[b].n % 2 == 0, "eigh block %lld: an embedded complex block has an even extent", (long long)b);
    return eigh_batched_ranged(ctx, descs, n, info, flags);
}

}
```

### cyten_amd/csrc/truncation.hip

```cpp
#include "common.h"

#include <algorithm>
#include <vector>

namespace {

constexpr int NT = 1024;
constexpr int NMAX = 8192;
constexpr int NBIG = 65536;

struct SDesc {
    const double* S;
    int64_t n, offset;
    double w;
};

struct Opts {
    int64_t chi_max, chi_min;
    double degeneracy_tol, trunc_cut, svd_min;
    int32_t has_svd_min, minimize_error;
};

__device__ __forceinline__ bool key_less(double ka, int ia, double kb, int ib) { return ka < kb || (ka == kb && ia < ib); }

__device__ int block_any(bool v, int* scratch)
{
    const unsigned long long b = __ballot(v);
    __syncthreads();
    if ((threadIdx.x & 63) == 0) scratch[threadIdx.x >> 6] = b != 0;
    __syncthreads();
    int r = 0;
    for (int q = 0; q < NT / 64; ++q) r |= scratch[q];
    return r;
}

template <typename T>
__device__ T block_excl_scan(T v, T* wave_tot, T* total)
{
    const int lane = threadIdx.x & 63, wave = threadIdx.x >> 6;
    T inc = v;
#pragma unroll
    for (int o = 1; o < 64; o <<= 1) {
        const T up = __shfl_up(inc, o);
        if (lane >= o) inc += up;
    }
    __syncthreads();
    if (lane == 63) wave_tot[wave] = inc;
    __syncthreads();
    T base = 0, all = 0;
    for (int w = 0; w < NT / 64; ++w) {
        if (w < wave) base += wave_tot[w];
        all += wave_tot[w];
    }
    if (total) *total = all;
    return base + inc - v;
}

template <bool BIG>
__global__ void __launch_bounds__(NT) truncate_select_kernel(const SDesc* __restrict__ descs, int n_sectors, int n, int n2, Opts o,
                                                             double* __restrict__ s_all,
                                                             int64_t* __restrict__ keep_idx, uint8_t* __restrict__ mask_out,
                                                             double* __restrict__ result,
                                                             double* __restrict__ gkey, int* __restrict__ gidx,
                                                             unsigned char* __restrict__ ggood)
{
    __shared__ double lkey[NMAX];
    __shared__ int lidx[NMAX];
    __shared__ unsigned char lgood[BIG ? 1 : NMAX];
    double* key = BIG ? gkey : lkey;
    int* idx = BIG ? gidx : lidx;
    unsigned char* good = BIG ? ggood : lgood;
    __shared__ int scratch[NT / 64];
    __shared__ double dtot[NT / 64];
    __shared__ int s_cut;
    const int tid = threadIdx.x;
    for (int s = 0; s < n_sectors; ++s) {
        const SDesc d = descs[s];
        for (int64_t e = tid; e < d.n; e += NT) {
            const double v = d.S[e];
            s_all[d.offset + e] = v;
            key[d.offset + e] = d.w * (v * v);
            idx[d.offset + e] = (int)(d.offset + e);
        }
    }
    for (int e = n + tid; e < n2; e += NT) {
        key[e] = __builtin_huge_val();
        idx[e] = e;
    }
    __syncthreads();
    auto cmpx = [&](double* kk, int* ii, int e, int p, bool up) {
        const double ka = kk[e], kb = kk[p];
        const int ia = ii[e], ib = ii[p];
        const bool swap = up ? key_less(kb, ib, ka, ia) : key_less(ka, ia, kb, ib);
        if (swap) {
            kk[e] = kb, kk[p] = ka;
            ii[e] = ib, ii[p] = ia;
        }
    };
    if (!BIG) {
        for (int k = 2; k <= n2; k <<= 1) {
            for (int j = k >> 1; j > 0; j >>= 1) {
                for (int t = tid; t < n2 / 2; t += NT) {
                    const int e = ((t & ~(j - 1)) << 1) | (t & (j - 1));
                    cmpx(key, idx, e, e + j, (e & k) == 0);
                }
                __syncthreads();
            }
        }
    } else {
        auto chunk_steps = [&](int base, int k, int jmax) {
            for (int e = tid; e < NMAX; e += NT) {
                lkey[e] = gkey[base + e];
                lidx[e] = gidx[base + e];
            }
            __syncthreads();
            for (int kk = (jmax == 0 ? 2 : k); kk <= k; kk <<= 1) {
                for (int j = min(kk >> 1, NMAX >> 1); j > 0; j >>= 1) {
                    for (int t = tid; t < NMAX / 2; t += NT) {
                        const int e = ((t & ~(j - 1)) << 1) | (t & (j - 1));
                        cmpx(lkey, lidx, e, e + j, ((base + e) & kk) == 0);
                    }
                    __syncthreads();
                }
            }
            for (int e = tid; e < NMAX; e += NT) {
                gkey[base + e] = lkey[e];
                gidx[base + e] = lidx[e];
            }
            __syncthreads();
        };
        for (int base = 0; base < n2; base += NMAX) chunk_steps(base, NMAX, 0);
        for (int k = 2 * NMAX; k <= n2; k <<= 1) {
            for (int j = k >> 1; j >= NMAX; j >>= 1) {
                for (int t = tid; t < n2 / 2; t += NT) {
                    const int e = ((t & ~(j - 1)) << 1) | (t & (j - 1));
                    cmpx(gkey, gidx, e, e + j, (e & k) == 0);
                }
                __syncthreads();
            }
            for (int base = 0; base < n2; base += NMAX) chunk_steps(base, k, 1);
        }
    }
    for (int e = tid; e < n; e += NT) good[e] = 1;
    __syncthreads();
    auto combine = [&](auto g2) {
        bool any = false;
        for (int e = tid; e < n; e += NT) any |= good[e] && g2(e);
        if (block_any(any, scratch)) {
            for (int e = tid; e < n; e += NT) good[e] = good[e] && g2(e);
        }
        __syncthreads();
    };
    if (o.chi_max >= 0 && o.chi_max < n) combine([&](int e) { return e >= n - (int)o.chi_max; });
    if (o.chi_min > 1) combine([&](int e) { return e < n - (int)o.chi_min + 1; });
    if (o.degeneracy_tol > 0.0)
        combine([&](int e) {
            if (e == 0) return true;
            const double a = s_all[idx[e]], b = s_all[idx[e - 1]];
            return log(a <= 1e-100 ? 1e-100 : a) - log(b <= 1e-100 ? 1e-100 : b) >= o.degeneracy_tol;
        });
    if (o.has_svd_min) combine([&](int e) { return s_all[idx[e]] >= o.svd_min; });
    {
        const int chunk = (n + NT - 1) / NT;
        const int b0 = min(tid * chunk, n), b1 = min(b0 + chunk, n);
        double run = 0.0;
        for (int e = b0; e < b1; ++e) {
            run += key[e];
            key[e] = run;
        }
        const double base = block_excl_scan<double>(run, dtot, nullptr);
        for (int e = b0; e < b1; ++e) key[e] += base;
        __syncthreads();
    }
    {
        const double tc2 = o.trunc_cut * o.trunc_cut;
        combine([&](int e) { return key[e] > tc2; });
    }
    {
        int best = o.minimize_error ? n : -1;
        for (int e = tid; e < n; e += NT)
            if (good[e]) best = o.minimize_error ? min(best, e) : max(best, e);
        for (int off = 32; off > 0; off >>= 1) {
            const int other = __shfl_xor(best, off);
            best = o.minimize_error ? min(best, other) : max(best, other);
        }
        if ((tid & 63) == 0) scratch[tid >> 6] = best;
        __syncthreads();
        if (tid == 0) {
            int b = scratch[0];
            for (int q = 1; q < NT / 64; ++q) b = o.minimize_error ? min(b, scratch[q]) : max(b, scratch[q]);
            s_cut = b;
            const double total = key[n - 1];
            const double err = b > 0 ? key[b - 1] : 0.0;
            result[0] = err;
            result[1] = total - err;
        }
        __syncthreads();
    }
    const int cut = s_cut;
    for (int e = tid; e < n; e += NT) good[idx[e]] = 0;
    __syncthreads();
    for (int e = cut + tid; e < n; e += NT) good[idx[e]] = 1;
    __syncthreads();
    for (int e = tid; e < n; e += NT) mask_out[e] = good[e];
    int64_t* counts = reinterpret_cast<int64_t*>(result + 2);
    for (int s = 0; s < n_sectors; ++s) {
        const SDesc d = descs[s];
        const int ns = (int)d.n, o0 = (int)d.offset;
        const int chunk = (ns + NT - 1) / NT;
        const int b0 = min(tid * chunk, ns), b1 = min(b0 + chunk, ns);
        int cnt = 0;
        for (int e = b0; e < b1; ++e) cnt += good[o0 + e];
        int kept = 0;
        int w = block_excl_scan<int>(cnt, scratch, &kept);
        if (tid == 0) counts[s] = kept;
        for (int e = b0; e < b1; ++e)
            if (good[o0 + e]) keep_idx[o0 + w++] = e;
        __syncthreads();
    }
}

}

extern "C" int cyb_truncate_select_f64(cyb_ctx_t ctx, const cyb_vec_desc* descs, int64_t n_sectors, const cyb_trunc_opts* opts,
                                       int64_t* keep_idx_dev, uint8_t* mask_dev, double* result_dev)
{
    return cyb_truncate_select_weighted_f64(ctx, descs, n_sectors, nullptr, opts, keep_idx_dev, mask_dev, result_dev);
}

extern "C" int cyb_truncate_select_weighted_f64(cyb_ctx_t ctx, const cyb_vec_desc* descs, int64_t n_sectors, const double* sector_weights,
                                                const cyb_trunc_opts* opts, int64_t* keep_idx_dev, uint8_t* mask_dev, double* result_dev)
{
    CYB_REQUIRE(ctx && opts && result_dev, "cyb_truncate_select_f64: NULL argument");
    CYB_REQUIRE(n_sectors >= 0 && (n_sectors == 0 || descs), "cyb_truncate_select_f64: bad sector list");
    std::vector<SDesc> hd((size_t)n_sectors);
    int64_t n = 0;
    for (int64_t s = 0; s < n_sectors; ++s) {
        CYB_REQUIRE(descs[s].n >= 0 && (descs[s].n == 0 || descs[s].x), "cyb_truncate_select_f64: sector %lld is malformed", (long long)s);
        const double w = sector_weights ? sector_weights[s] : 1.0;
        CYB_REQUIRE(w > 0.0 && w < 1e300, "cyb_truncate_select_weighted_f64: weight of sector %lld is not a positive finite number", (long long)s);
        hd[(size_t)s] = SDesc{descs[s].x, descs[s].n, n, w};
        n += descs[s].n;
    }
    CYB_REQUIRE(n >= 1, "cyb_truncate_select_f64: no singular values");
    CYB_REQUIRE(keep_idx_dev && mask_dev, "cyb_truncate_select_f64: NULL output");
    if (n > NBIG) {
        cyb::set_error("cyb_truncate_select_f64: %lld values exceed the %d one workgroup sorts", (long long)n, NBIG);
        return CYB_ERR_UNSUPPORTED;
    }
    CYB_REQUIRE(opts->chi_min >= 1, "cyb_truncate_select_f64: chi_min must be >= 1");
    int n2 = 2;
    while (n2 < n) n2 <<= 1;
    void *d_descs = nullptr, *ws = nullptr;
    CYB_TRY(ctx->upload(hd.data(), sizeof(SDesc) * hd.size(), &d_descs));
    const bool big = n > NMAX;
    if (big) n2 = std::max(n2, 2 * NMAX);
    const size_t off_key = (sizeof(double) * (size_t)n + 255) & ~(size_t)255;
    const size_t off_idx = off_key + sizeof(double) * (size_t)n2, off_good = off_idx + sizeof(int) * (size_t)n2;
    CYB_TRY(ctx->workspace(big ? off_good + (size_t)n2 : sizeof(double) * (size_t)n, &ws, 2));
    Opts o{opts->chi_max, opts->chi_min, opts->degeneracy_tol, opts->trunc_cut, opts->svd_min, opts->has_svd_min,
           opts->minimize_error};
    char* w8 = static_cast<char*>(ws);
    if (big)
        hipLaunchKernelGGL(truncate_select_kernel<true>, dim3(1), dim3(NT), 0, ctx->stream, static_cast<const SDesc*>(d_descs),
                           (int)n_sectors, (int)n, n2, o, static_cast<double*>(ws), keep_idx_dev, mask_dev, result_dev,
                           reinterpret_cast<double*>(w8 + off_key), reinterpret_cast<int*>(w8 + off_idx),
                           reinterpret_cast<unsigned char*>(w8 + off_good));
    else
        hipLaunchKernelGGL(truncate_select_kernel<false>, dim3(1), dim3(NT), 0, ctx->stream, static_cast<const SDesc*>(d_descs),
                           (int)n_sectors, (int)n, n2, o, static_cast<double*>(ws), keep_idx_dev, mask_dev, result_dev,
                           (double*)nullptr, (int*)nullptr, (unsigned char*)nullptr);
    CYB_HIP(hipGetLastError());
    return CYB_OK;
}
```

Baseline: 5469.

## Parallelize amax, rank and truncation sorting; drop J scatter and buffers

Spreads the matrix amax reduction over a number of workgroups proportional to matrix size, with an unrolled load loop. The rank kernel now splits the key comparisons across four waves per 64-element column and uses a wider launch grid. Truncation replaces the single-workgroup bitonic sort with a parallel counting-rank kernel for the small case. The separate J scatter kernel and several buffers are removed by having j_to_cq read through an inverse index map. Finer sweep timing stamps are also added for debugging. The main risks are the extra kernel launches and the reshaped buffer layout.

```diff
diff --git a/cyten_amd/csrc/jacobi_engine.hip b/cyten_amd/csrc/jacobi_engine.hip
--- a/cyten_amd/csrc/jacobi_engine.hip
+++ b/cyten_amd/csrc/jacobi_engine.hip
@@ -1054,7 +1054,7 @@
     const int un = lane & 15, ukq = lane >> 4;
 #define SWEEP_STAMP(k)                                                                                            \
     do {                                                                                                          \
-        if (sc.stamps && tid == 0 && round == sc.stamp_round) sc.stamps[(size_t)blockIdx.x * 8 + (k)] = wall_clock64(); \
+        if (sc.stamps && tid == 0 && round == sc.stamp_round) sc.stamps[(size_t)blockIdx.x * 16 + (k)] = wall_clock64(); \
     } while (0)
 
     {
@@ -1243,8 +1243,10 @@
             }
             __syncthreads();
         }
+        SWEEP_STAMP(8);
         const double off = gram_offmax(Gs, red, tid);
         if (part == 0 && tid == 0) atomicMax(offmax_bits + (size_t)sw * sc.n_mats + mt.mat, (unsigned long long)__double_as_longlong(off));
+        SWEEP_STAMP(9);
         const bool skip = off <= mt.tol && !any_null;
         if (!skip) {
             double* Ga = Gs;
@@ -1272,6 +1274,7 @@
             } else
                 for (int e = tid; e < JP * VS; e += NT) Va[e] = ((e / VS) == (e % VS)) ? 1.0 : 0.0;
             __syncthreads();
+            SWEEP_STAMP(10);
             {
                 const int pr = tid >> 4, pc = tid & 15;
                 const int r0 = 2 * pr, c0 = 2 * pc;
@@ -1338,6 +1341,7 @@
                 if (lane < JP) perm[rk] = lane;
             }
             __syncthreads();
+            SWEEP_STAMP(11);
             for (int e = tid; e < JP * JP; e += NT) {
                 const int k = e / JP, m = e % JP;
                 Qs[k * QS + m] = Vc[k * VS + perm[m]];
@@ -1583,7 +1587,7 @@
         static const bool want_stamps = getenv("CYB_JACOBI_STAMPS") != nullptr;
         static unsigned long long* d_stamps = nullptr;
         if (want_stamps) {
-            if (!d_stamps && hipMalloc(reinterpret_cast<void**>(&d_stamps), sizeof(unsigned long long) * 8 * 2048) != hipSuccess) d_stamps = nullptr;
+            if (!d_stamps && hipMalloc(reinterpret_cast<void**>(&d_stamps), sizeof(unsigned long long) * 16 * 2048) != hipSuccess) d_stamps = nullptr;
             rs.stamps = d_stamps;
         }
         static bool attr_set = false;
@@ -1736,6 +1740,7 @@
                 ss.arrive = reinterpret_cast<unsigned int*>(d_off + w_off);
                 ss.nsw = reinterpret_cast<int*>(ss.arrive + n);
                 one_launch_done = one_launch;
+                if (ss.stamps && hipMemsetAsync(ss.stamps, 0, sizeof(unsigned long long) * 16 * 2048, st) != hipSuccess) ss.stamps = nullptr;
                 if (cplx)
                     hipLaunchKernelGGL(jacobi_sweep_kernel<true>, dim3((unsigned)n_wg), dim3(NT), SWEEP_LDS_BYTES, st,
                                        static_cast<const RPair*>(d_rp2), max_inner, d_off, ss);
@@ -1743,22 +1748,32 @@
                     hipLaunchKernelGGL(jacobi_sweep_kernel<false>, dim3((unsigned)n_wg), dim3(NT), SWEEP_LDS_BYTES, st,
                                        static_cast<const RPair*>(d_rp2), max_inner, d_off, ss);
                 if (ss.stamps && wgmap.size() <= 2048) {
-                    std::vector<unsigned long long> hs(8 * wgmap.size());
+                    std::vector<unsigned long long> hs(16 * wgmap.size());
                     if (hipMemcpyAsync(hs.data(), rs.stamps, sizeof(unsigned long long) * hs.size(), hipMemcpyDeviceToHost, st) == hipSuccess &&
                         hipStreamSynchronize(st) == hipSuccess) {
                         double acc[6] = {0, 0, 0, 0, 0, 0};
+                        const int cut[7] = {3, 8, 9, 10, 4, 11, 5};
+                        double sub[6] = {0, 0, 0, 0, 0, 0};
+                        int cnts = 0;
                         int cntw = 0;
                         const int mbig = order.front();
                         for (size_t b = 0; b < wgmap.size(); ++b) {
                             if (wl[(size_t)wgmap[b].x].mat != mbig) continue;
-                            for (int k = 0; k < 6; ++k) acc[k] += (double)(hs[8 * b + k + 1] - hs[8 * b + k]) * 0.01;
+                            if (hs[16 * b + 10] == 0 || hs[16 * b + 11] == 0) continue;
+                            for (int k = 0; k < 6; ++k) acc[k] += (double)(hs[16 * b + k + 1] - hs[16 * b + k]) * 0.01;
                             ++cntw;
+                            for (int k = 0; k < 6; ++k) sub[k] += (double)(hs[16 * b + cut[k + 1]] - hs[16 * b + cut[k]]) * 0.01;
+                            ++cnts;
                         }
                         if (cntw)
                             fprintf(stderr, "[jacobi sweep stamps] sweep %d round %d, largest matrix (G=%d, %d workgroups of %zu): wait %.2f load+gram %.2f "
                                             "exch %.2f defl+eig %.2f sort %.2f upd+publish %.2f us\n",
                                     sweep, ss.stamp_round, Gm[(size_t)mbig], cntw, wgmap.size(), acc[0] / cntw, acc[1] / cntw,
                                     acc[2] / cntw, acc[3] / cntw, acc[4] / cntw, acc[5] / cntw);
+                        if (cnts)
+                            fprintf(stderr, "[jacobi sweep stamps]   of defl+eig and sort (%d workgroups): defl+flags %.2f offnorm %.2f setup %.2f "
+                                            "rotations %.2f rank %.2f Qs+zout %.2f us\n",
+                                    cnts, sub[0] / cnts, sub[1] / cnts, sub[2] / cnts, sub[3] / cnts, sub[4] / cnts, sub[5] / cnts);
                     }
                 }
                 did_sweep = true;
diff --git a/cyten_amd/csrc/scaling.hip b/cyten_amd/csrc/scaling.hip
--- a/cyten_amd/csrc/scaling.hip
+++ b/cyten_amd/csrc/scaling.hip
@@ -15,30 +15,42 @@
     int64_t lda;
     int32_t m, n;
     double* out;
+    int32_t parts, pad;
 };
+
+constexpr int kAmaxChunk = 16384;
+
+__device__ __forceinline__ void amax_take(double v, double& mx, bool& bad)
+{
+    bad = bad || !(fabs(v) <= 1.7e308);
+    mx = fmax(mx, fabs(v));
+}
 
 __global__ void __launch_bounds__(256) matrix_amax_kernel(const AmaxDesc* __restrict__ descs)
 {
     __shared__ double red[4];
     const AmaxDesc d = descs[blockIdx.y];
+    if ((int)blockIdx.x >= d.parts) return;
     gcp A = (gcp)d.A;
     double mx = 0.0;
     bool bad = false;
     if (d.lda == d.n) {
         const int64_t tot = (int64_t)d.m * d.n;
-        for (int64_t e = (int64_t)blockIdx.x * 256 + threadIdx.x; e < tot; e += (int64_t)gridDim.x * 256) {
-            const double v = A[e];
-            bad = bad || !(fabs(v) <= 1.7e308);
-            mx = fmax(mx, fabs(v));
+        const int64_t per = (tot + d.parts - 1) / d.parts;
+        const int64_t e0 = (int64_t)blockIdx.x * per, e1 = e0 + per < tot ? e0 + per : tot;
+        int64_t e = e0 + threadIdx.x;
+        for (; e + 7 * 256 < e1; e += 8 * 256) {
+            double v[8];
+#pragma unroll
+            for (int q = 0; q < 8; ++q) v[q] = A[e + q * 256];
+#pragma unroll
+            for (int q = 0; q < 8; ++q) amax_take(v[q], mx, bad);
         }
+        for (; e < e1; e += 256) amax_take(A[e], mx, bad);
     } else {
-        for (int r = blockIdx.x; r < d.m; r += gridDim.x) {
+        for (int r = blockIdx.x; r < d.m; r += d.parts) {
             gcp row = A + (int64_t)r * d.lda;
-            for (int c = threadIdx.x; c < d.n; c += 256) {
-                const double v = row[c];
-                bad = bad || !(fabs(v) <= 1.7e308);
-                mx = fmax(mx, fabs(v));
-            }
+            for (int c = threadIdx.x; c < d.n; c += 256) amax_take(row[c], mx, bad);
         }
     }
     if (bad) mx = __builtin_nan("");
@@ -84,22 +96,30 @@
     const size_t n = mats.size();
     amax.assign(n, 0.0);
     if (n == 0) return CYB_OK;
-    constexpr int kParts = 32;
+    constexpr int kMaxParts = 128;
+    std::vector<AmaxDesc> ds(n);
+    std::vector<size_t> first(n + 1, 0);
+    int max_parts = 1;
+    for (size_t i = 0; i < n; ++i) {
+        const int64_t tot = (int64_t)mats[i].m * (int64_t)mats[i].n;
+        const int parts = (int)std::min<int64_t>(kMaxParts, std::max<int64_t>(1, (tot + kAmaxChunk - 1) / kAmaxChunk));
+        ds[i] = AmaxDesc{mats[i].A, mats[i].lda, (int32_t)mats[i].m, (int32_t)mats[i].n, nullptr, parts, 0};
+        first[i + 1] = first[i] + (size_t)parts;
+        max_parts = std::max(max_parts, parts);
+    }
     void* d_out = nullptr;
-    CYB_TRY(ctx->workspace(sizeof(double) * n * kParts, &d_out, 2));
-    std::vector<AmaxDesc> ds(n);
-    for (size_t i = 0; i < n; ++i)
-        ds[i] = AmaxDesc{mats[i].A, mats[i].lda, (int32_t)mats[i].m, (int32_t)mats[i].n, static_cast<double*>(d_out) + i * kParts};
+    CYB_TRY(ctx->workspace(sizeof(double) * first[n], &d_out, 2));
+    for (size_t i = 0; i < n; ++i) ds[i].out = static_cast<double*>(d_out) + first[i];
     void* d_ds = nullptr;
     CYB_TRY(ctx->upload(ds.data(), sizeof(AmaxDesc) * n, &d_ds));
-    hipLaunchKernelGGL(matrix_amax_kernel, dim3(kParts, (unsigned)n), dim3(256), 0, ctx->stream, static_cast<const AmaxDesc*>(d_ds));
+    hipLaunchKernelGGL(matrix_amax_kernel, dim3((unsigned)max_parts, (unsigned)n), dim3(256), 0, ctx->stream, static_cast<const AmaxDesc*>(d_ds));
     CYB_HIP(hipGetLastError());
-    std::vector<double> parts(n * kParts);
+    std::vector<double> parts(first[n]);
     CYB_TRY(ctx->d2h(parts.data(), d_out, sizeof(double) * parts.size()));
     for (size_t i = 0; i < n; ++i) {
         double r = 0.0;
-        for (int p = 0; p < kParts; ++p) {
-            const double v = parts[i * kParts + p];
+        for (size_t p = first[i]; p < first[i + 1]; ++p) {
+            const double v = parts[p];
             r = (r != r || v != v) ? std::nan("") : std::max(r, v);
         }
         amax[i] = r;
diff --git a/cyten_amd/csrc/svd_jacobi.hip b/cyten_amd/csrc/svd_jacobi.hip
--- a/cyten_amd/csrc/svd_jacobi.hip
+++ b/cyten_amd/csrc/svd_jacobi.hip
@@ -138,38 +138,48 @@
 
 __global__ void __launch_bounds__(256) rank_kernel(const PostDesc* __restrict__ descs)
 {
-    constexpr int CH = 2048;
+    constexpr int CH = 4096;
     __shared__ double keys[CH];
+    __shared__ int part[4][64];
     const PostDesc d = descs[blockIdx.y];
+    if ((int)blockIdx.x * 64 >= d.nv) return;
     gcp sig = (gcp)d.sig;
     const double shift = d.shift ? *(gcp)d.shift : 0.0;
     const int msk = d.cplx ? ~1 : ~0;
-    const int per = (d.nv + (int)gridDim.x * 256 - 1) / ((int)gridDim.x * 256);
-    for (int it = 0; it < per; ++it) {
-        const int j = (it * (int)gridDim.x + (int)blockIdx.x) * 256 + (int)threadIdx.x;
+    const int lane = threadIdx.x & 63, wave = threadIdx.x >> 6;
+    bool staged = false;
+    for (int j0 = (int)blockIdx.x * 64; j0 < d.nv; j0 += (int)gridDim.x * 64) {
+        const int j = j0 + lane;
         const bool mine = j < d.nv;
         const double sj = mine ? sig[j & msk] : 0.0;
         int r = 0;
         for (int k0 = 0; k0 < d.nv; k0 += CH) {
             const int kn = min(CH, d.nv - k0);
-            __syncthreads();
-            for (int k = threadIdx.x; k < kn; k += 256) keys[k] = sig[(k0 + k) & msk];
-            __syncthreads();
-            if (mine) {
-                if (d.mode == 0) {
-                    for (int k = 0; k < kn; ++k) {
-                        const double sk = keys[k];
-                        r += (sk > sj || (sk == sj && k0 + k < j)) ? 1 : 0;
-                    }
-                } else {
-                    for (int k = 0; k < kn; ++k) {
-                        const double sk = keys[k];
-                        r += (sk < sj || (sk == sj && k0 + k < j)) ? 1 : 0;
-                    }
+            if (!staged || d.nv > CH) {
+                __syncthreads();
+                for (int k = threadIdx.x; k < kn; k += 256) keys[k] = sig[(k0 + k) & msk];
+                __syncthreads();
+                staged = true;
+            }
+            const int q = (kn + 3) / 4;
+            const int ka = min(wave * q, kn), kb = min(ka + q, kn);
+            if (d.mode == 0) {
+                for (int k = ka; k < kb; ++k) {
+                    const double sk = keys[k];
+                    r += (sk > sj || (sk == sj && k0 + k < j)) ? 1 : 0;
                 }
-            }
-        }
-        if (mine) {
+            } else {
+                for (int k = ka; k < kb; ++k) {
+                    const double sk = keys[k];
+                    r += (sk < sj || (sk == sj && k0 + k < j)) ? 1 : 0;
+                }
+            }
+        }
+        __syncthreads();
+        part[wave][lane] = r;
+        __syncthreads();
+        if (wave == 0 && mine) {
+            r = part[0][lane] + part[1][lane] + part[2][lane] + part[3][lane];
             d.rank[j] = r;
             d.S[r] = (d.mode == 0) ? sj : sj - shift;
         }
@@ -492,7 +502,7 @@
     CYB_TRY(ctx->upload(post.data(), sizeof(PostDesc) * post.size(), &d_post));
     const PostDesc* dp = static_cast<const PostDesc*>(d_post);
     hipLaunchKernelGGL(row_norm_kernel, dim3(helper_grid_x((size_t)nmat), (unsigned)nmat), dim3(256), 0, st, dp);
-    hipLaunchKernelGGL(rank_kernel, dim3(8, (unsigned)nmat), dim3(256), 0, st, dp);
+    hipLaunchKernelGGL(rank_kernel, dim3(helper_grid_x((size_t)nmat), (unsigned)nmat), dim3(256), 0, st, dp);
     hipLaunchKernelGGL(write_factors_kernel, dim3(helper_grid_x((size_t)nmat), (unsigned)nmat), dim3(256), 0, st, dp);
     if (mode == 0) hipLaunchKernelGGL(complete_null_kernel, dim3((unsigned)nmat), dim3(256), 0, st, dp);
     CYB_HIP(hipGetLastError());
@@ -541,7 +551,8 @@
     const int32_t* rank;
     double* Cq;
     int64_t L;
-    int32_t kp, k;
+    int32_t ld, k;
+    const int32_t* inv;
 };
 __global__ void __launch_bounds__(256) j_to_cq_kernel(const JcqDesc* __restrict__ descs)
 {
@@ -551,7 +562,18 @@
     const int lane = threadIdx.x & 63;
     for (int j = blockIdx.x * 4 + (threadIdx.x >> 6); j < d.k; j += gridDim.x * 4) {
         const int r = d.rank[j];
-        for (int i = lane; i < d.k; i += 64) Cq[(int64_t)r * d.L + i] = J[(int64_t)j * d.kp + i];
+        if (!d.inv) {
+            for (int i = lane; i < d.k; i += 64) Cq[(int64_t)r * d.L + i] = J[(int64_t)j * d.ld + i];
+        } else {
+            const int g = d.inv[j];
+            for (int i = lane; i < d.k; i += 64) {
+                const int h = d.inv[i];
+                double v = i == j ? 1.0 : 0.0;
+                if (g >= 0) v = h >= 0 ? J[(int64_t)g * d.ld + h] : 0.0;
+                Cq[(int64_t)r * d.L + i] = v;
+            }
+        }
+        for (int64_t i = d.k + lane; i < d.L; i += 64) Cq[(int64_t)r * d.L + i] = 0.0;
     }
 }
 
@@ -579,17 +601,6 @@
         } else {
             for (int c = lane; c < d.ncols; c += 64) dst[(int64_t)j * d.ldd + c] = 0.0;
         }
-    }
-}
-__global__ void __launch_bounds__(256) j_scatter_kernel(const RowMoveDesc* __restrict__ descs)
-{
-    const RowMoveDesc d = descs[blockIdx.y];
-    gcp src = (gcp)d.src;
-    gp dst = (gp)d.dst;
-    const int lane = threadIdx.x & 63;
-    for (int g = blockIdx.x * 4 + (threadIdx.x >> 6); g < d.cnt; g += gridDim.x * 4) {
-        const int j = d.idx[g];
-        for (int h = lane; h < d.cnt; h += 64) dst[(int64_t)j * d.ldd + d.idx[h]] = src[(int64_t)g * d.lds + h];
     }
 }
 
@@ -752,15 +763,12 @@
     }
 }
 
-static int launch_row_moves(cyb_ctx_t ctx, const std::vector<RowMoveDesc>& v, bool jscatter = false)
+static int launch_row_moves(cyb_ctx_t ctx, const std::vector<RowMoveDesc>& v)
 {
     if (v.empty()) return CYB_OK;
     void* d = nullptr;
     CYB_TRY(ctx->upload(v.data(), sizeof(RowMoveDesc) * v.size(), &d));
-    if (jscatter)
-        hipLaunchKernelGGL(j_scatter_kernel, dim3(64, (unsigned)v.size()), dim3(256), 0, ctx->stream, static_cast<const RowMoveDesc*>(d));
-    else
-        hipLaunchKernelGGL(row_move_kernel, dim3(helper_grid_x(v.size()), (unsigned)v.size()), dim3(256), 0, ctx->stream, static_cast<const RowMoveDesc*>(d));
+    hipLaunchKernelGGL(row_move_kernel, dim3(helper_grid_x(v.size()), (unsigned)v.size()), dim3(256), 0, ctx->stream, static_cast<const RowMoveDesc*>(d));
     CYB_HIP(hipGetLastError());
     return CYB_OK;
 }
@@ -782,10 +790,13 @@
         size_t ctl;
         int n_fac = -1;
         size_t sigo;
+        size_t ginv;
+        bool j_eye = false;
         size_t dev;
         bool lq = false;
         bool jrec = false;
         int r0 = 0;
+        int rp() const { return std::max(round_up(r0, 64), 64); }
         std::vector<int32_t> good0;
     };
     std::vector<Lay> lay((size_t)nmat);
@@ -827,22 +838,16 @@
             off += al(bytes);
             return o;
         };
-        l.Ac = take(sizeof(double) * (size_t)l.L * l.k);
         l.aux = take(bqr_aux_bytes(l.L, l.k, l.L, l.k));
         l.stop = take(sizeof(double) * (size_t)std::max(1, (l.k + cyb::NBK - 1) / cyb::NBK * cyb::bqr_strip_slots(l.L)));
         l.W = take(sizeof(double) * (size_t)l.kp * l.kp);
-        l.J = take(sizeof(double) * (size_t)l.kp * l.kp);
         l.rank = take(sizeof(int32_t) * (size_t)l.kp);
         l.nnull = take(sizeof(int32_t));
-        l.Cq = take(sizeof(double) * (size_t)l.L * l.k);
-        l.Fc = take(sizeof(double) * (size_t)l.k * l.k);
         l.aux2 = take(bqr_aux_bytes(l.k, l.k, l.k, l.k));
-        l.Cn = take(sizeof(double) * (size_t)l.k * l.k);
         l.Wc = take(sizeof(double) * (size_t)l.kp * l.kp);
         l.Jc = take(sizeof(double) * (size_t)l.kp * l.kp);
         l.Wq = take(sizeof(double) * (size_t)l.kp * l.kp);
         l.aux3 = take(bqr_aux_bytes(l.k, l.k, l.kp, l.k));
-        l.Cq2 = take(sizeof(double) * (size_t)l.k * l.k);
         l.sig2 = take(sizeof(double) * (size_t)l.kp);
         l.sigo = take(sizeof(double) * (size_t)l.kp);
     }
@@ -851,16 +856,34 @@
         lay[(size_t)b].idx = off;
         off += sizeof(int32_t) * (size_t)lay[(size_t)b].k;
     }
+    for (int64_t b = 0; b < nmat; ++b) {
+        lay[(size_t)b].ginv = off;
+        off += sizeof(int32_t) * (size_t)lay[(size_t)b].k;
+    }
     off = al(off);
+    const size_t zero_bytes = off;
+    for (int64_t b = 0; b < nmat; ++b) {
+        Lay& l = lay[(size_t)b];
+        auto take = [&](size_t bytes) {
+            const size_t o = off;
+            off += al(bytes);
+            return o;
+        };
+        l.Ac = take(sizeof(double) * (size_t)l.L * l.k);
+        l.J = take(sizeof(double) * (size_t)l.kp * l.kp);
+        l.Cq = take(sizeof(double) * (size_t)l.L * l.k);
+        l.Fc = take(sizeof(double) * (size_t)l.k * l.k);
+        l.Cn = take(sizeof(double) * (size_t)l.k * l.k);
+        l.Cq2 = take(sizeof(double) * (size_t)l.k * l.k);
+    }
     void* ws = nullptr;
     CYB_TRY(ctx->workspace(off, &ws, 0));
     char* base = static_cast<char*>(ws);
-    CYB_HIP(hipMemsetAsync(ws, 0, off, st));
+    CYB_HIP(hipMemsetAsync(ws, 0, zero_bytes, st));
     auto dp = [&](size_t o) { return reinterpret_cast<double*>(base + o); };
 
     std::vector<BqrMat> qm((size_t)nmat);
     std::vector<XposeDesc> x_in, x_r;
-    std::vector<EyeDesc> eyeJ;
     std::vector<JMat> jm((size_t)nmat);
     for (int64_t b = 0; b < nmat; ++b) {
         const Lay& l = lay[(size_t)b];
@@ -881,7 +904,6 @@
         else
             x_in.push_back(XposeDesc{sd[b].A, q.Ac, sd[b].lda, l.L, l.m, l.n, 0, 0, 1, 0});
         x_r.push_back(XposeDesc{q.Ac, dp(l.W), l.L, l.kp, l.k, l.k, 1, l.k, 0, 0});
-        eyeJ.push_back(EyeDesc{dp(l.J), l.kp, l.kp, l.kp, 0, 0});
         JMat& j = jm[(size_t)b];
         j.W = dp(l.W);
         j.J = dp(l.J);
@@ -897,7 +919,6 @@
     CYB_TRY(xpose_batched(ctx, x_in));
     CYB_TRY(bqr_factor(ctx, qm));
     CYB_TRY(xpose_batched(ctx, x_r));
-    CYB_TRY(eye_cols_batched(ctx, eyeJ));
     std::vector<PostDesc> post((size_t)nmat);
     for (int64_t b = 0; b < nmat; ++b) {
         const Lay& l = lay[(size_t)b];
@@ -933,7 +954,7 @@
     CYB_HIP(hipGetLastError());
     CYB_TRY(ctx->d2h(h_sig.data(), base + sig_begin, sig_bytes));
     {
-        std::vector<int32_t> idx_all;
+        std::vector<int32_t> idx_all, inv_all;
         std::vector<size_t> idx_off((size_t)nmat, 0);
         for (int64_t b = 0; b < nmat; ++b) {
             Lay& l = lay[(size_t)b];
@@ -954,6 +975,9 @@
             idx_off[(size_t)b] = idx_all.size();
             idx_all.insert(idx_all.end(), l.good0.begin(), l.good0.end());
             idx_all.insert(idx_all.end(), nul.begin(), nul.end());
+            const size_t i0 = inv_all.size();
+            inv_all.resize(i0 + (size_t)l.k, -1);
+            for (int g = 0; g < l.r0; ++g) inv_all[i0 + (size_t)l.good0[(size_t)g]] = g;
         }
         static const bool no_lq = getenv("CYB_SVD_NOLQ") != nullptr;
         static const bool lq_always = getenv("CYB_SVD_LQ_ALWAYS") != nullptr;
@@ -988,6 +1012,7 @@
             l.jrec = hi <= jrec_ratio * lo;
         }
         void* d_idx_v = nullptr;
+        idx_all.insert(idx_all.end(), inv_all.begin(), inv_all.end());
         CYB_TRY(ctx->upload(idx_all.data(), sizeof(int32_t) * idx_all.size(), &d_idx_v));
         CYB_HIP(hipMemcpyAsync(base + idx_begin, d_idx_v, sizeof(int32_t) * idx_all.size(), hipMemcpyDeviceToDevice, st));
     }
@@ -1008,9 +1033,13 @@
         for (int64_t b = 0; b < nmat; ++b) {
             Lay& l = lay[(size_t)b];
             l.lq = l.lq && allow_lq;
-            if (l.r0 == l.k && !l.lq) continue;
+            if (l.r0 == l.k && !l.lq) {
+                if (!l.j_eye) eyeJc.push_back(EyeDesc{dp(l.J), l.kp, l.kp, l.kp, 0, 0});
+                l.j_eye = true;
+                continue;
+            }
             const int32_t* didx = reinterpret_cast<const int32_t*>(base + l.idx);
-            const int rp = std::max(round_up(l.r0, 64), 64);
+            const int rp = l.rp();
             gat.push_back(RowMoveDesc{dp(l.W), dp(l.Wc), didx, l.kp, l.kp, l.r0, l.kp, 0, 0});
             if (l.r0 < l.k) zer.push_back(RowMoveDesc{nullptr, dp(l.W), didx + l.r0, 0, l.kp, l.k - l.r0, l.kp, 2, 0});
             const bool jrec = l.lq && l.jrec && allow_lq;
@@ -1142,17 +1171,14 @@
         for (int64_t b = 0; b < nmat; ++b) info[b] = sweeps[(size_t)b];
     if (jst != CYB_OK && jst != CYB_ERR_NOCONV) return jst;
     {
-        std::vector<RowMoveDesc> sw, sj;
+        std::vector<RowMoveDesc> sw;
         for (int64_t b = 0; b < nmat; ++b) {
             const Lay& l = lay[(size_t)b];
             if ((l.r0 == l.k && !l.lq) || l.r0 == 0) continue;
             const int32_t* didx = reinterpret_cast<const int32_t*>(base + l.idx);
-            const int rp = std::max(round_up(l.r0, 64), 64);
             sw.push_back(RowMoveDesc{dp(l.Wc), dp(l.W), didx, l.kp, l.kp, l.r0, l.kp, 1, 0});
-            sj.push_back(RowMoveDesc{dp(l.Jc), dp(l.J), didx, rp, l.kp, l.r0, l.r0, 0, 0});
         }
         CYB_TRY(launch_row_moves(ctx, sw));
-        CYB_TRY(launch_row_moves(ctx, sj, true));
     }
     for (int64_t b = 0; b < nmat; ++b) post[(size_t)b].sig_lq = lay[(size_t)b].lq ? dp(lay[(size_t)b].sigo) : nullptr;
     CYB_TRY(ctx->upload(post.data(), sizeof(PostDesc) * post.size(), &d_post));
@@ -1251,7 +1277,7 @@
     }
     CYB_TRY(ctx->upload(post.data(), sizeof(PostDesc) * post.size(), &d_post));
     dpost = static_cast<const PostDesc*>(d_post);
-    hipLaunchKernelGGL(rank_kernel, dim3(8, (unsigned)nmat), dim3(256), 0, st, dpost);
+    hipLaunchKernelGGL(rank_kernel, dim3(helper_grid_x((size_t)nmat), (unsigned)nmat), dim3(256), 0, st, dpost);
     hipLaunchKernelGGL(write_factors_kernel, dim3(helper_grid_x((size_t)nmat), (unsigned)nmat), dim3(256), 0, st, dpost);
     CYB_HIP(hipGetLastError());
     std::vector<JcqDesc> jc;
@@ -1259,7 +1285,11 @@
     std::vector<XposeDesc> x_out;
     for (int64_t b = 0; b < nmat; ++b) {
         const Lay& l = lay[(size_t)b];
-        jc.push_back(JcqDesc{dp(l.J), reinterpret_cast<const int32_t*>(base + l.rank), dp(l.Cq), l.L, l.kp, l.k});
+        if (l.r0 == l.k && !l.lq)
+            jc.push_back(JcqDesc{dp(l.J), reinterpret_cast<const int32_t*>(base + l.rank), dp(l.Cq), l.L, l.kp, l.k, nullptr});
+        else
+            jc.push_back(JcqDesc{dp(l.Jc), reinterpret_cast<const int32_t*>(base + l.rank), dp(l.Cq), l.L, l.rp(), l.k,
+                                 reinterpret_cast<const int32_t*>(base + l.ginv)});
         tg.push_back(BqrTarget{(int)b, dp(l.Cq), l.L, l.k, l.n_fac >= 0 ? l.n_fac : (l.k + cyb::NBK - 1) / cyb::NBK});
         if (l.tall)
             x_out.push_back(XposeDesc{dp(l.Cq), sd[b].U, l.L, sd[b].ldu, l.m, l.k, 0, 0, 0, 0});
diff --git a/cyten_amd/csrc/truncation.hip b/cyten_amd/csrc/truncation.hip
--- a/cyten_amd/csrc/truncation.hip
+++ b/cyten_amd/csrc/truncation.hip
@@ -54,6 +54,52 @@
     }
     if (total) *total = all;
     return base + inc - v;
+}
+
+constexpr int RCH = 4096;
+__global__ void __launch_bounds__(256) truncate_rank_kernel(const SDesc* __restrict__ descs, int n_sectors, int n, double* __restrict__ s_all,
+                                                            double* __restrict__ skey, int* __restrict__ sidx)
+{
+    __shared__ unsigned long long lk[RCH];
+    __shared__ int part[4][64];
+    const int tid = threadIdx.x, lane = tid & 63, wave = tid >> 6;
+    const int e = (int)blockIdx.x * 64 + lane;
+    double mine = 0.0;
+    if (e < n) {
+        int s = 0;
+        while (s + 1 < n_sectors && e >= descs[s].offset + descs[s].n) ++s;
+        const double v = descs[s].S[e - descs[s].offset];
+        mine = descs[s].w * (v * v);
+        if (wave == 0) s_all[e] = v;
+    }
+    const unsigned long long ke = (unsigned long long)__double_as_longlong(mine);
+    int r = 0;
+    for (int c0 = 0; c0 < n; c0 += RCH) {
+        const int cn = min(RCH, n - c0);
+        __syncthreads();
+        for (int s = 0; s < n_sectors; ++s) {
+            const SDesc d = descs[s];
+            const int lo = max((int)d.offset, c0), hi = min((int)(d.offset + d.n), c0 + cn);
+            for (int f = lo + tid; f < hi; f += 256) {
+                const double v = d.S[f - d.offset];
+                lk[f - c0] = (unsigned long long)__double_as_longlong(d.w * (v * v));
+            }
+        }
+        __syncthreads();
+        const int q = (cn + 3) / 4;
+        const int fa = min(wave * q, cn), fb = min(fa + q, cn);
+        for (int f = fa; f < fb; ++f) {
+            const unsigned long long kf = lk[f];
+            r += (kf < ke || (kf == ke && c0 + f < e)) ? 1 : 0;
+        }
+    }
+    part[wave][lane] = r;
+    __syncthreads();
+    if (wave == 0 && e < n) {
+        r = part[0][lane] + part[1][lane] + part[2][lane] + part[3][lane];
+        skey[r] = mine;
+        sidx[r] = e;
+    }
 }
 
 template <bool BIG>
@@ -74,40 +120,36 @@
     __shared__ double dtot[NT / 64];
     __shared__ int s_cut;
     const int tid = threadIdx.x;
-    for (int s = 0; s < n_sectors; ++s) {
-        const SDesc d = descs[s];
-        for (int64_t e = tid; e < d.n; e += NT) {
-            const double v = d.S[e];
-            s_all[d.offset + e] = v;
-            key[d.offset + e] = d.w * (v * v);
-            idx[d.offset + e] = (int)(d.offset + e);
-        }
-    }
-    for (int e = n + tid; e < n2; e += NT) {
-        key[e] = __builtin_huge_val();
-        idx[e] = e;
-    }
-    __syncthreads();
-    auto cmpx = [&](double* kk, int* ii, int e, int p, bool up) {
-        const double ka = kk[e], kb = kk[p];
-        const int ia = ii[e], ib = ii[p];
-        const bool swap = up ? key_less(kb, ib, ka, ia) : key_less(ka, ia, kb, ib);
-        if (swap) {
-            kk[e] = kb, kk[p] = ka;
-            ii[e] = ib, ii[p] = ia;
-        }
-    };
     if (!BIG) {
-        for (int k = 2; k <= n2; k <<= 1) {
-            for (int j = k >> 1; j > 0; j >>= 1) {
-                for (int t = tid; t < n2 / 2; t += NT) {
-                    const int e = ((t & ~(j - 1)) << 1) | (t & (j - 1));
-                    cmpx(key, idx, e, e + j, (e & k) == 0);
-                }
-                __syncthreads();
-            }
-        }
+        for (int e = tid; e < n; e += NT) {
+            key[e] = gkey[e];
+            idx[e] = gidx[e];
+        }
+        __syncthreads();
     } else {
+        for (int s = 0; s < n_sectors; ++s) {
+            const SDesc d = descs[s];
+            for (int64_t e = tid; e < d.n; e += NT) {
+                const double v = d.S[e];
+                s_all[d.offset + e] = v;
+                key[d.offset + e] = d.w * (v * v);
+                idx[d.offset + e] = (int)(d.offset + e);
+            }
+        }
+        for (int e = n + tid; e < n2; e += NT) {
+            key[e] = __builtin_huge_val();
+            idx[e] = e;
+        }
+        __syncthreads();
+        auto cmpx = [&](double* kk, int* ii, int e, int p, bool up) {
+            const double ka = kk[e], kb = kk[p];
+            const int ia = ii[e], ib = ii[p];
+            const bool swap = up ? key_less(kb, ib, ka, ia) : key_less(ka, ia, kb, ib);
+            if (swap) {
+                kk[e] = kb, kk[p] = ka;
+                ii[e] = ib, ii[p] = ia;
+            }
+        };
         auto chunk_steps = [&](int base, int k, int jmax) {
             for (int e = tid; e < NMAX; e += NT) {
                 lkey[e] = gkey[base + e];
@@ -257,19 +299,23 @@
     if (big) n2 = std::max(n2, 2 * NMAX);
     const size_t off_key = (sizeof(double) * (size_t)n + 255) & ~(size_t)255;
     const size_t off_idx = off_key + sizeof(double) * (size_t)n2, off_good = off_idx + sizeof(int) * (size_t)n2;
-    CYB_TRY(ctx->workspace(big ? off_good + (size_t)n2 : sizeof(double) * (size_t)n, &ws, 2));
+    CYB_TRY(ctx->workspace(big ? off_good + (size_t)n2 : off_good, &ws, 2));
     Opts o{opts->chi_max, opts->chi_min, opts->degeneracy_tol, opts->trunc_cut, opts->svd_min, opts->has_svd_min,
            opts->minimize_error};
     char* w8 = static_cast<char*>(ws);
+    double* d_key = reinterpret_cast<double*>(w8 + off_key);
+    int* d_idx = reinterpret_cast<int*>(w8 + off_idx);
     if (big)
         hipLaunchKernelGGL(truncate_select_kernel<true>, dim3(1), dim3(NT), 0, ctx->stream, static_cast<const SDesc*>(d_descs),
-                           (int)n_sectors, (int)n, n2, o, static_cast<double*>(ws), keep_idx_dev, mask_dev, result_dev,
-                           reinterpret_cast<double*>(w8 + off_key), reinterpret_cast<int*>(w8 + off_idx),
+                           (int)n_sectors, (int)n, n2, o, static_cast<double*>(ws), keep_idx_dev, mask_dev, result_dev, d_key, d_idx,
                            reinterpret_cast<unsigned char*>(w8 + off_good));
-    else
+    else {
+        hipLaunchKernelGGL(truncate_rank_kernel, dim3((unsigned)((n + 63) / 64)), dim3(256), 0, ctx->stream,
+                           static_cast<const SDesc*>(d_descs), (int)n_sectors, (int)n, static_cast<double*>(ws), d_key, d_idx);
         hipLaunchKernelGGL(truncate_select_kernel<false>, dim3(1), dim3(NT), 0, ctx->stream, static_cast<const SDesc*>(d_descs),
-                           (int)n_sectors, (int)n, n2, o, static_cast<double*>(ws), keep_idx_dev, mask_dev, result_dev,
-                           (double*)nullptr, (int*)nullptr, (unsigned char*)nullptr);
+                           (int)n_sectors, (int)n, n2, o, static_cast<double*>(ws), keep_idx_dev, mask_dev, result_dev, d_key, d_idx,
+                           (unsigned char*)nullptr);
+    }
     CYB_HIP(hipGetLastError());
     return CYB_OK;
 }
```

Result: no change. 5503 (median of 5 runs) (+0.6%).
